# rofuyu/exp-trmf-nips16

Hardware: AMD Instinct MI355X
Metric: als_iterations_per_sec (higher is better)
Workload: dtype f32

## Files before the change

exp-trmf-nips16_amd/csrc/full_kernels.hpp:

```cpp
#pragma once

#include "cg_kernels.hpp"
#include "common.hpp"
#include "gram_kernels.hpp"

namespace trmf {

#if !defined(TRMF_UNIT_BODIES)
template <int NT>
__global__ void spmm_rows_kernel(const uint32_t *__restrict__ ptr,
                                                        const uint32_t *__restrict__ idx,
                                                        const real *__restrict__ val,
                                                        const real *__restrict__ X,
                                                        real *__restrict__ out, uint32_t row_begin,
                                                        uint32_t row_end, uint32_t zero_row, uint32_t long_thresh);
template <int NT>
__global__ void spmm_part_kernel(const uint32_t *__restrict__ idx, const real *__restrict__ val, const real *__restrict__ X,
                                 const uint32_t *__restrict__ items, uint32_t item_begin, uint32_t item_end, real *__restrict__ part,
                                 uint32_t zero_row);
#else
template <int NT, bool ITEM>
__device__ __forceinline__ void spmm_body(const uint32_t *__restrict__ ptr,
                                                        const uint32_t *__restrict__ idx,
                                                        const real *__restrict__ val,
                                                        const real *__restrict__ X,
                                                        real *__restrict__ out, uint32_t row_begin,
                                                        uint32_t row_end, uint32_t zero_row, uint32_t long_thresh) {
    constexpr int KP = kTile * NT;
    const int wave = threadIdx.x >> 6, lane = threadIdx.x & 63;
    const int g = lane >> 4, c = lane & 15;
    const uint32_t row = row_begin + blockIdx.x * 4u + (uint32_t)wave;
    if (row >= row_end) return;
    const uint32_t p0 = (uint32_t)__builtin_amdgcn_readfirstlane((int)ptr[ITEM ? 2 * row : row]);
    const uint32_t p1 = (uint32_t)__builtin_amdgcn_readfirstlane((int)ptr[ITEM ? 2 * row + 1 : row + 1]);
    if (!ITEM && p1 - p0 >= long_thresh) return;
    GramState<NT> st;
    st.clear();
    real nowq[NT];
#pragma unroll
    for (int q = 0; q < NT; q++) nowq[q] = 0;
    if (p1 > p0)
        gram_ring<NT, kRingDepth, false, false>(st, idx, val, X, zero_row, 4u, lane, nowq, GramDesc{p0, p1, 0},
                                                SingleRowStream{4u * kRingDepth}, [](int) {});
#pragma unroll
    for (int q = 0; q < NT; q++) {
        real v = st.b[q];
        v += __shfl_xor(v, 16, kWave);
        v += __shfl_xor(v, 32, kWave);
        if (g == 0) out[(size_t)row * KP + kTile * q + c] = v;
    }
}
template <int NT>
__global__ __launch_bounds__(256) void spmm_rows_kernel(const uint32_t *__restrict__ ptr,
                                                        const uint32_t *__restrict__ idx,
                                                        const real *__restrict__ val,
                                                        const real *__restrict__ X,
                                                        real *__restrict__ out, uint32_t row_begin,
                                                        uint32_t row_end, uint32_t zero_row, uint32_t long_thresh) {
    spmm_body<NT, false>(ptr, idx, val, X, out, row_begin, row_end, zero_row, long_thresh);
}
template <int NT>
__global__ __launch_bounds__(256) void spmm_part_kernel(const uint32_t *__restrict__ idx, const real *__restrict__ val,
                                                        const real *__restrict__ X, const uint32_t *__restrict__ items,
                                                        uint32_t item_begin, uint32_t item_end, real *__restrict__ part, uint32_t zero_row) {
    spmm_body<NT, true>(items, idx, val, X, part, item_begin, item_end, zero_row, 0u);
}
#endif

#if !defined(TRMF_UNIT)
__global__ __launch_bounds__(256) void spmm_reduce_kernel(const uint32_t *__restrict__ rows, const uint32_t *__restrict__ first,
                                                          const real *__restrict__ part, real *__restrict__ out, uint32_t begin,
                                                          uint32_t end, int KP) {
    const size_t e = (size_t)blockIdx.x * 256 + threadIdx.x;
    const uint32_t li = begin + (uint32_t)(e / (size_t)KP);
    if (li >= end) return;
    const int col = (int)(e % (size_t)KP);
    real acc = 0;
    for (uint32_t it = first[li]; it < first[li + 1]; it++) acc += part[(size_t)it * KP + col];
    out[(size_t)rows[li] * KP + col] = acc;
}
#endif

#if !defined(TRMF_UNIT_BODIES)
template <int NT>
__global__ void dense_tn_mfma_kernel(const real *__restrict__ A, int K, int M,
                                                            const real *__restrict__ B,
                                                            double *__restrict__ part);
#else
template <int NT>
__global__ __launch_bounds__(256) void dense_tn_mfma_kernel(const real *__restrict__ A, int K, int M,
                                                            const real *__restrict__ B,
                                                            double *__restrict__ part) {
    constexpr int KP = kTile * NT;
    const int wave = threadIdx.x >> 6, lane = threadIdx.x & 63, g = lane >> 4, c = lane & 15;
    const int m0 = (blockIdx.x * 4 + wave) * kTile;
    if (m0 >= M) return;
    const int nchunk = gridDim.y, ch = blockIdx.y;
    const int j0 = (int)((long long)K * ch / nchunk), j1 = (int)((long long)K * (ch + 1) / nchunk);
    typename Mfma16<real>::acc_t acc[NT];
#pragma unroll
    for (int q = 0; q < NT; q++) acc[q] = typename Mfma16<real>::acc_t{0, 0, 0, 0};
    const int mrow = min(m0 + c, M - 1);
    constexpr int U = 4;
    for (int j = j0; j < j1; j += 4 * U) {
        real a[U];
        RealVec<NT> bv[U];
#pragma unroll
        for (int u = 0; u < U; u++) {
            const int jj = j + 4 * u + g;
            const bool valid = jj < j1;
            const size_t jr = (size_t)(valid ? jj : j0);
            a[u] = A[jr * M + mrow];
            bv[u] = *reinterpret_cast<const RealVec<NT> *>(B + jr * KP + NT * c);
            if (!valid) a[u] = 0;
        }
#pragma unroll
        for (int u = 0; u < U; u++)
#pragma unroll
            for (int q = 0; q < NT; q++) acc[q] = Mfma16<real>::mma(a[u], bv[u].v[q], acc[q]);
    }
#pragma unroll
    for (int q = 0; q < NT; q++)
#pragma unroll
        for (int r = 0; r < 4; r++) {
            const int m = m0 + Mfma16<real>::row(lane, r);
            if (m < M) part[((size_t)ch * M + m) * KP + NT * c + q] = (double)acc[q][r];
        }
}
#endif
#if !defined(TRMF_UNIT)
__global__ __launch_bounds__(256) void dense_tn_reduce_kernel(const double *__restrict__ part, int nchunk,
                                                              int M, int KP, int NT, int k,
                                                              real *__restrict__ out) {
    const size_t e = (size_t)blockIdx.x * 4 + (threadIdx.x >> 6);
    const int lane = threadIdx.x & 63;
    if (e >= (size_t)M * KP) return;
    const int m = (int)(e / KP), tp = (int)(e - (size_t)m * KP);
    double acc = 0;
    for (int ch = lane; ch < nchunk; ch += 64) acc += part[((size_t)ch * M + m) * KP + tp];
    acc = wave_butterfly_sum(acc);
    const int t = collog(tp, NT);
    if (lane == 0) out[(size_t)m * KP + t] = (t < k) ? (real)acc : real(0);
}
#endif

#if !defined(TRMF_UNIT)
__global__ __launch_bounds__(256) void dense_tn_reduce_flat_kernel(const double *__restrict__ part, int nchunk,
                                                                   int M, int KP, int NT, int k,
// ... 258 lines not shown
```

exp-trmf-nips16_amd/csrc/gram_kernels.hpp:

```cpp
#pragma once

#include <type_traits>
#include <utility>

#include "common.hpp"

namespace trmf {

template <typename T> struct Mfma16;
template <> struct Mfma16<float> {
    typedef float acc_t __attribute__((ext_vector_type(4)));
    static __device__ __forceinline__ acc_t mma(float a, float b, acc_t c) {
        return __builtin_amdgcn_mfma_f32_16x16x4f32(a, b, c, 0, 0, 0);
    }
    static __device__ __forceinline__ int row(int lane, int r) { return 4 * (lane >> 4) + r; }
};
template <> struct Mfma16<double> {
    typedef double acc_t __attribute__((ext_vector_type(4)));
    static __device__ __forceinline__ acc_t mma(double a, double b, acc_t c) {
        return __builtin_amdgcn_mfma_f64_16x16x4f64(a, b, c, 0, 0, 0);
    }
    static __device__ __forceinline__ int row(int lane, int r) { return (lane >> 4) + 4 * r; }
};

// ... 25 lines not shown
    v += __shfl_xor(v, 16, kWave);
    v += __shfl_xor(v, 32, kWave);
    return v;
}

template <int... Is, typename Fn>
__device__ __forceinline__ void static_for_impl(std::integer_sequence<int, Is...>, Fn &&f) {
    (f(std::integral_constant<int, Is>{}), ...);
}
template <int N, typename Fn> __device__ __forceinline__ void static_for(Fn &&f) {
    static_for_impl(std::make_integer_sequence<int, N>{}, f);
}
struct GramDesc {
    uint32_t e0;
    uint32_t end;
    int row;
};

template <typename T> __device__ __forceinline__ T row16_sum(T v) { return row16_allsum(v); }
#if defined(TRMF_F32)
template <int CTRL> __device__ __forceinline__ float dpp_mov(float v) {
    return __int_as_float(__builtin_amdgcn_update_dpp(0, __float_as_int(v), CTRL, 0xf, 0xf, true));
}
__device__ __forceinline__ float row16_allsum_dpp(float v) {
    v += dpp_mov<0xB1>(v);
    v += dpp_mov<0x4E>(v);
    v += dpp_mov<0x141>(v);
    v += dpp_mov<0x140>(v);
    return v;
}
template <> __device__ __forceinline__ float row16_sum<float>(float v) { return row16_allsum_dpp(v); }
#endif

template <int NT> struct GramState {
    typename Mfma16<real>::acc_t acc[NT * (NT + 1) / 2];
    real b[NT];
    double loss;
    __device__ __forceinline__ void clear() {
#pragma unroll
        for (int t = 0; t < NT * (NT + 1) / 2; t++) acc[t] = typename Mfma16<real>::acc_t{0, 0, 0, 0};
#pragma unroll
        for (int q = 0; q < NT; q++) b[q] = 0;
        loss = 0;
    }
};

template <int N> struct alignas(sizeof(real)) RealVec { real v[N]; };

template <int SRC> __device__ __forceinline__ uint32_t quad_bcast(uint32_t v) {
    return (uint32_t)__builtin_amdgcn_update_dpp(0, (int)v, 0x55 * SRC, 0xf, 0xf, true);
}
template <int SRC> __device__ __forceinline__ float quad_bcast(float v) {
    return __int_as_float(__builtin_amdgcn_update_dpp(0, __float_as_int(v), 0x55 * SRC, 0xf, 0xf, true));
}
template <int SRC> __device__ __forceinline__ double quad_bcast(double v) {
    const long long b = __double_as_longlong(v);
    const int lo = __builtin_amdgcn_update_dpp(0, (int)(b & 0xffffffffLL), 0x55 * SRC, 0xf, 0xf, true);
    const int hi = __builtin_amdgcn_update_dpp(0, (int)(b >> 32), 0x55 * SRC, 0xf, 0xf, true);
    return __longlong_as_double(((long long)hi << 32) | (unsigned int)lo);
}

template <int SRC> __device__ __forceinline__ float quad_inject(float x, float y) {
    return __int_as_float(__builtin_amdgcn_update_dpp(__float_as_int(x), __float_as_int(y), 0x55 * SRC, 0xf, 0x8, false));
}
template <int SRC> __device__ __forceinline__ double quad_inject(double x, double y) {
    const long long xb = __double_as_longlong(x), yb = __double_as_longlong(y);
    const int lo = __builtin_amdgcn_update_dpp((int)(xb & 0xffffffffLL), (int)(yb & 0xffffffffLL), 0x55 * SRC, 0xf, 0x8, false);
    const int hi = __builtin_amdgcn_update_dpp((int)(xb >> 32), (int)(yb >> 32), 0x55 * SRC, 0xf, 0x8, false);
    return __longlong_as_double(((long long)hi << 32) | (unsigned int)lo);
}
template <int NT> __host__ __device__ constexpr bool rhs_pad_ok(int k) { return k <= kTile * NT - 8; }

template <int NT, typename R>
__device__ __forceinline__ void load_factor_slice(R (&dst)[NT], __amdgpu_buffer_rsrc_t rsrc, uint32_t byte_off) {
#pragma unroll
    for (int q = 0; q < NT; q++) {
        if constexpr (sizeof(R) == 4)
            dst[q] = __builtin_bit_cast(R, __builtin_amdgcn_raw_buffer_load_b32(rsrc, byte_off + 4 * q, 0, 0));
        else
            dst[q] = __builtin_bit_cast(R, __builtin_amdgcn_raw_buffer_load_b64(rsrc, byte_off + 8 * q, 0, 0));
    }
}

template <int NT, int D, bool DO_MMA, bool WITH_LOSS, bool RHS_PAD = false, bool TAIL = false, bool ROWEND = false, typename Next, typename RowDone>
__device__ __forceinline__ void gram_ring(GramState<NT> &st, const uint32_t *__restrict__ idx,
                                          const real *__restrict__ val, const real *__restrict__ X,
                                          uint32_t zero_row, uint32_t estride, int lane,
                                          const real (&wq)[NT], GramDesc d0, Next &&next,
                                          RowDone &&row_done) {
    static_assert(D == 4, "one quad lane per group of the iteration");
    constexpr int KP = kTile * NT;
    const uint32_t g = (uint32_t)(lane >> 4), c = (uint32_t)(lane & 15);
    const __amdgpu_buffer_rsrc_t x_rsrc =
        __builtin_amdgcn_make_buffer_rsrc(const_cast<real *>(X), 0, -1 , 0x00020000);
    const uint32_t lane_bytes = (uint32_t)NT * c * (uint32_t)sizeof(real);
    uint32_t jraw; real yraw; bool vraw;
    uint32_t jsel; real ysel;

    const uint32_t lane_e = (c & 3u) * estride + g;
    auto load_entries = [&](const GramDesc &d) {
        const uint32_t e0u = (uint32_t)__builtin_amdgcn_readfirstlane((int)d.e0), endu = (uint32_t)__builtin_amdgcn_readfirstlane((int)d.end);
        uint32_t left;
        asm("s_max_u32 %0, %1, %2\n\ts_sub_u32 %0, %0, %2" : "=&s"(left) : "s"(endu), "s"(e0u) : "scc");
        vraw = lane_e < left;
        const __amdgpu_buffer_rsrc_t ir = __builtin_amdgcn_make_buffer_rsrc(const_cast<uint32_t *>(idx + e0u), 0, (int)(left * 4u), 0x00020000);
        const __amdgpu_buffer_rsrc_t vr = __builtin_amdgcn_make_buffer_rsrc(const_cast<real *>(val + e0u), 0, (int)(left * (uint32_t)sizeof(real)), 0x00020000);
        jraw = __builtin_amdgcn_raw_buffer_load_b32(ir, lane_e * 4u, 0, 0);
        real yv[1];
        load_factor_slice(yv, vr, lane_e * (uint32_t)sizeof(real));
        yraw = yv[0];
    };
    auto promote_entries = [&]() {
        jsel = __umul24(vraw ? jraw : zero_row, (uint32_t)(KP * sizeof(real)));
        ysel = yraw;
    };
    auto load_slices = [&](auto U, real (&x)[D][NT], real (&yx)[D]) {
        constexpr int u = decltype(U)::value;
        if constexpr (!RHS_PAD) yx[u] = quad_bcast<u>(ysel);
        load_factor_slice(x[u], x_rsrc, quad_bcast<u>(jsel) + lane_bytes);
    };

    GramDesc d1 = d0; next(d1);
    GramDesc d2 = d1; next(d2);
    real x[D][NT], yx[D];
    load_entries(d0);
    promote_entries();
    if (TAIL && d1.row < 0) {
        static_for<D>([&](auto U) { load_slices(U, x, yx); });
    } else {
        load_entries(d1);
        __builtin_amdgcn_sched_barrier(0);
        static_for<D>([&](auto U) { load_slices(U, x, yx); });
        __builtin_amdgcn_sched_barrier(0);
    }
    auto consume = [&](auto U, real ycons) {
        constexpr int u = decltype(U)::value;
        real xt[NT];
#pragma unroll
        for (int q = 0; q < NT; q++) xt[q] = x[u][q];
        if constexpr (RHS_PAD) xt[NT - 1] = quad_inject<u>(x[u][NT - 1], ycons);
        else {
#pragma unroll
            for (int q = 0; q < NT; q++) st.b[q] = fma(yx[u], x[u][q], st.b[q]);
        }
        if (DO_MMA) {
            int t = 0;
#pragma unroll
            for (int ti = 0; ti < NT; ti++)
#pragma unroll
                for (int tj = ti; tj < NT; tj++, t++) st.acc[t] = Mfma16<real>::mma(xt[ti], xt[tj], st.acc[t]);
        }
        if (WITH_LOSS) {
            real d = 0;
#pragma unroll
            for (int q = 0; q < NT; q++) d = fma(wq[q], x[u][q], d);
            d = row16_sum(d);
            const real res = yx[u] - d;
            st.loss += (double)res * (double)res;
        }
    };
    while (TAIL ? d1.row >= 0 : d0.row >= 0) {
        const real ycons = ysel;
        promote_entries();
        load_entries(d2);
        const uint32_t left = ROWEND ? (uint32_t)__builtin_amdgcn_readfirstlane((int)(d0.end - d0.e0)) : 0u;
        static_for<D>([&](auto U) {
            constexpr uint32_t u = (uint32_t)decltype(U)::value;
            if (!ROWEND || u == 0 || left > 4u * u) consume(U, ycons);
            __builtin_amdgcn_sched_barrier(0);
            load_slices(U, x, yx);
            __builtin_amdgcn_sched_barrier(0);
        });
        if (d1.row != d0.row) { row_done(d0.row); }
        d0 = d1; d1 = d2; next(d2);
    }
    if constexpr (TAIL) {
        if (d0.row >= 0) {
            const int ngr = (int)((d0.end - d0.e0 + 3u) >> 2);
            const real ycons = ysel;
            static_for<D>([&](auto U) {
                if (decltype(U)::value < ngr) consume(U, ycons);
            });
            row_done(d0.row);
        }
    }
}

struct SingleRowStream {
    uint32_t step;
    __device__ __forceinline__ void operator()(GramDesc &d) const {
        if (d.row < 0) return;
        d.e0 += step;
        if (d.e0 >= d.end) { d.row = -1; d.end = 0; }
    }
};

constexpr int kRingDepth = 4;

struct SplitRows {
    const uint32_t *rows;
    const uint32_t *first;
    const real *slab;
    uint32_t stride;
    uint32_t begin, end;
};
template <int NT> __host__ __device__ constexpr uint32_t split_part_reals(bool with_b) {
    return (uint32_t)(NT * (NT + 1) / 2) * 4u * kWave + (with_b ? (uint32_t)NT * kWave : 0u);
}
#if !defined(TRMF_UNIT)
__global__ __launch_bounds__(256) void split_reduce_kernel(const uint32_t *__restrict__ first, real *__restrict__ slab, uint32_t stride,
                                                           uint32_t begin, uint32_t end, uint32_t blocks_per_row) {
    typedef real gran_t __attribute__((ext_vector_type(16 / sizeof(real))));
    constexpr uint32_t GR = 16 / sizeof(real);
    const uint32_t li = begin + blockIdx.x / blocks_per_row;
    if (li >= end) return;
    const uint32_t i0 = first[li], i1 = first[li + 1];
    const uint32_t gidx = (blockIdx.x % blocks_per_row) * 256u + threadIdx.x;
    if (i1 - i0 < 2u || gidx * GR >= stride) return;
    real *dst = slab + (size_t)i0 * stride + (size_t)gidx * GR;
    gran_t acc = *reinterpret_cast<const gran_t *>(dst);
    const real *p = dst + stride;
    uint32_t it = i0 + 1;
    for (; it + 8 <= i1; it += 8, p += (size_t)8 * stride) {
        gran_t v[8];
#pragma unroll
        for (int u = 0; u < 8; u++) v[u] = *reinterpret_cast<const gran_t *>(p + (size_t)u * stride);
#pragma unroll
        for (int u = 0; u < 8; u++) acc += v[u];
    }
    for (; it < i1; it++, p += stride) acc += *reinterpret_cast<const gran_t *>(p);
    *reinterpret_cast<gran_t *>(dst) = acc;
}
#endif

template <int NT, bool WITH_B>
__device__ __forceinline__ void load_row_sum(GramState<NT> &st, const SplitRows &sp, uint32_t i0, int lane) {
    typedef typename Mfma16<real>::acc_t acc_t;
    constexpr int NTT = NT * (NT + 1) / 2;
    const real *p = sp.slab + (size_t)i0 * sp.stride;
#pragma unroll
    for (int t = 0; t < NTT; t++) st.acc[t] = *reinterpret_cast<const acc_t *>(p + t * 4 * kWave + 4 * lane);
#pragma unroll
    for (int q = 0; q < NT; q++) st.b[q] = WITH_B ? p[NTT * 4 * kWave + q * kWave + lane] : real(0);
    st.loss = 0;
}

#if !defined(TRMF_F32)
__device__ __forceinline__ void wave_lds_sync() {
    __builtin_amdgcn_fence(__ATOMIC_ACQ_REL, "wavefront");
    __builtin_amdgcn_wave_barrier();
}
#endif



#if !defined(TRMF_F32)
constexpr int kMfmaWaves = 2;
constexpr int kRcpNewton = 2;
__device__ __forceinline__ double recip_pivot(double d) {
    double r = __builtin_amdgcn_rcp(d);
#pragma unroll
    for (int i = 0; i < kRcpNewton; i++) { const double e = fma(-d, r, 1.0); r = fma(r, e, r); }
    return r;
}
__host__ __device__ constexpr int upper_tile_index(int ti, int tj, int NT) { return ti * NT - ti * (ti - 1) / 2 + (tj - ti); }

#if !defined(TRMF_UNIT_BODIES)
template <int NT, int KMAX>
__global__ void fsolve_mfma_kernel(const uint32_t *__restrict__ ptr,
                                                                          const uint32_t *__restrict__ idx,
                                                                          const real *__restrict__ val,
                                                                          const real *__restrict__ X,
                                                                          real *__restrict__ F, uint32_t row_begin,
                                                                          uint32_t row_end, int k, real lambda,
                                                                          uint32_t zero_row, uint32_t long_m1);
template <int NT, int KMAX>
__global__ void fsolve_mfma_long_kernel(SplitRows sp, real *__restrict__ F, int k, real lambda);
#else
template <int NT, int KMAX, bool LONG>
__device__ __forceinline__ void fsolve_mfma_body(const uint32_t *__restrict__ ptr,
                                                                          const uint32_t *__restrict__ idx,
                                                                          const real *__restrict__ val,
                                                                          const real *__restrict__ X,
                                                                          real *__restrict__ F, uint32_t row_begin,
                                                                          uint32_t row_end, int k, real lambda,
                                                                          uint32_t zero_row, uint32_t long_m1, const SplitRows &sp) {
    static_assert(sizeof(real) == 8, "the in-accumulator F-solve is the fp64 path");
    constexpr int KP = kTile * NT, NPAN = KMAX / 4;
    constexpr int CP = 10;
    constexpr int FIN = (KP + 1) * CP;
    constexpr int RP = KP + 2;
    constexpr int SCR = (FIN + 8 > kTile * RP) ? FIN + 8 : kTile * RP;
    __shared__ __attribute__((aligned(16))) real scr_s[4][SCR];
    const int wave = threadIdx.x >> 6, lane = threadIdx.x & 63;
    const int g = lane >> 4, c = lane & 15;
    real *ps = scr_s[wave];
    typedef typename Mfma16<real>::acc_t acc_t;
    typedef VecOf<real, 2> pair_t;
    GramState<NT> st;
    uint32_t row;
    if constexpr (LONG) {
        const uint32_t li = sp.begin + blockIdx.x * 4u + (uint32_t)wave;
        if (li >= sp.end) return;
        row = (uint32_t)__builtin_amdgcn_readfirstlane((int)sp.rows[li]);
        load_row_sum<NT, true>(st, sp, (uint32_t)__builtin_amdgcn_readfirstlane((int)sp.first[li]), lane);
    } else {
        row = row_begin + blockIdx.x * 4u + (uint32_t)wave;
        if (row >= row_end) return;
        const uint32_t p0 = (uint32_t)__builtin_amdgcn_readfirstlane((int)ptr[row]);
        const uint32_t p1 = (uint32_t)__builtin_amdgcn_readfirstlane((int)ptr[row + 1]);
        if (p1 - p0 - 1u >= long_m1) return;
        st.clear();
        real nowq[NT];
#pragma unroll
        for (int q = 0; q < NT; q++) nowq[q] = 0;
        gram_ring<NT, kRingDepth, true, false, false, true>(st, idx, val, X, zero_row, 4u, lane, nowq, GramDesc{p0, p1, 0},
                                                            SingleRowStream{4u * kRingDepth}, [](int) {});
    }
    real y = 0, dinv = 1;
#pragma unroll
    for (int q = 0; q < NT; q++) {
        real v = st.b[q];
        v += __shfl_xor(v, 16, kWave);
        v += __shfl_xor(v, 32, kWave);
        if (g == q) y = v;
    }
#pragma unroll
    for (int ti = 0; ti < NT; ti++)
#pragma unroll
        for (int r = 0; r < 4; r++)
            if (c == g + 4 * r) st.acc[upper_tile_index(ti, ti, NT)][r] += (kTile * ti + c < k) ? lambda : real(1);

    static_for<NPAN>([&](auto Pn) {
        constexpr int pn = decltype(Pn)::value, tp = pn >> 2, r0 = pn & 3, j0 = 4 * pn;
#pragma unroll
        for (int tj = tp; tj < NT; tj++) ps[(kTile * tj + c) * CP + g] = st.acc[upper_tile_index(tp, tj, NT)][r0];
        if ((unsigned)(lane - j0) < 4u) ps[KP * CP + (lane - j0)] = y;
        wave_lds_sync();
        const real *pc = ps + j0 * CP;
        const real P00 = pc[0];
        real P01 = pc[CP], P11 = pc[CP + 1];
        real P02 = pc[2 * CP], P12 = pc[2 * CP + 1], P22 = pc[2 * CP + 2];
        real P03 = pc[3 * CP], P13 = pc[3 * CP + 1], P23 = pc[3 * CP + 2], P33 = pc[3 * CP + 3];
        const real i0 = recip_pivot(P00);
        const real l10 = P01 * i0, l20 = P02 * i0, l30 = P03 * i0;
        P11 = fma(-l10, P01, P11); P12 = fma(-l10, P02, P12); P13 = fma(-l10, P03, P13);
        P22 = fma(-l20, P02, P22); P23 = fma(-l20, P03, P23); P33 = fma(-l30, P03, P33);
        const real i1 = recip_pivot(P11);
        const real l21 = P12 * i1, l31 = P13 * i1;
        P22 = fma(-l21, P12, P22); P23 = fma(-l21, P13, P23); P33 = fma(-l31, P13, P33);
        const real i2 = recip_pivot(P22);
        const real l32 = P23 * i2;
        P33 = fma(-l32, P23, P33);
        const real i3 = recip_pivot(P33);
        const bool has_col = KP == kWave || lane < KP;
        const int col = (lane == j0 || !has_col) ? KP : lane;
        real *rec = ps + col * CP;
        const Quad<real> rin = *reinterpret_cast<const Quad<real> *>(rec);
        const real R0 = rin.v[0];
        const real R1 = fma(-l10, R0, rin.v[1]);
        const real R2 = fma(-l21, R1, fma(-l20, R0, rin.v[2]));
        const real R3 = fma(-l32, R2, fma(-l31, R1, fma(-l30, R0, rin.v[3])));
        const real S0 = -(R0 * i0), S1 = -(R1 * i1), S2 = -(R2 * i2), S3 = -(R3 * i3);
        if (has_col) {
            *reinterpret_cast<Quad<real> *>(rec) = Quad<real>{{R0, R1, R2, R3}};
            *reinterpret_cast<Quad<real> *>(rec + 4) = Quad<real>{{S0, S1, S2, S3}};
        }
        if (lane == j0) {
            *reinterpret_cast<Quad<real> *>(ps + FIN) = Quad<real>{{R0, i0, R1, i1}};
            *reinterpret_cast<Quad<real> *>(ps + FIN + 4) = Quad<real>{{R2, i2, R3, i3}};
        }
        wave_lds_sync();
        {
            const Quad<real> f0 = *reinterpret_cast<const Quad<real> *>(ps + FIN), f1 = *reinterpret_cast<const Quad<real> *>(ps + FIN + 4);
            const real upd = fma(S3, f1.v[2], fma(S2, f1.v[0], fma(S1, f0.v[2], fma(S0, f0.v[0], y))));
            const int q = min(max(lane - j0, 0), 3);
            const pair_t mine = *reinterpret_cast<const pair_t *>(ps + FIN + 2 * q);
            const bool in_panel = (unsigned)(lane - j0) < 4u;
            y = in_panel ? mine.v[0] : (lane > j0 + 3 ? upd : y);
            dinv = in_panel ? mine.v[1] : dinv;
        }
#pragma unroll
        for (int tj = tp; tj < NT; tj++) st.acc[upper_tile_index(tp, tj, NT)][r0] = ps[(kTile * tj + c) * CP + g];
        real aop[NT];
#pragma unroll
        for (int tj = tp; tj < NT; tj++) aop[tj] = ps[(kTile * tj + c) * CP + 4 + g];
        if (c <= 4 * r0 + 3) aop[tp] = 0;
        wave_lds_sync();
#pragma unroll
        for (int ti = tp; ti < NT; ti++)
#pragma unroll
            for (int tj = ti; tj < NT; tj++) {
                acc_t &C = st.acc[upper_tile_index(ti, tj, NT)];
                C = Mfma16<real>::mma(aop[ti], st.acc[upper_tile_index(tp, tj, NT)][r0], C);
            }
    });

    static_for<NT>([&](auto Tr) {
        constexpr int tt = NT - 1 - decltype(Tr)::value;
        if constexpr (kTile * tt < KMAX) {
#pragma unroll
            for (int ti = 0; ti <= tt; ti++)
#pragma unroll
                for (int r = 0; r < 4; r++) {
                    real v = st.acc[upper_tile_index(ti, tt, NT)][r];
                    if (ti == tt && g + 4 * r >= c) v = 0;
                    ps[c * RP + kTile * ti + g + 4 * r] = v;
                }
            if constexpr (tt + 1 < NT) {
#pragma unroll
                for (int r = 0; r < 4; r++) ps[c * RP + kTile * (tt + 1) + g + 4 * r] = 0;
            }
            wave_lds_sync();
            static_for<kTile>([&](auto Nr) {
                constexpr int n = kTile - 1 - decltype(Nr)::value, t = kTile * tt + n;
                if constexpr (t < KMAX && t > 0) {
                    const real xt = lane_bcast(y * dinv, t);
                    const real cv = (KP == kWave || lane < KP) ? ps[n * RP + lane] : real(0);
                    y = fma(-cv, xt, y);
                }
            });
            wave_lds_sync();
        }
    });
    if (lane < k) F[(size_t)row * KP + colpos(lane, NT)] = y * dinv;
}
template <int NT, int KMAX>
__global__ __launch_bounds__(256, kMfmaWaves) void fsolve_mfma_kernel(const uint32_t *__restrict__ ptr,
                                                                          const uint32_t *__restrict__ idx,
                                                                          const real *__restrict__ val,
                                                                          const real *__restrict__ X,
                                                                          real *__restrict__ F, uint32_t row_begin,
                                                                          uint32_t row_end, int k, real lambda,
                                                                          uint32_t zero_row, uint32_t long_m1) {
    fsolve_mfma_body<NT, KMAX, false>(ptr, idx, val, X, F, row_begin, row_end, k, lambda, zero_row, long_m1, SplitRows{});
}
template <int NT, int KMAX>
__global__ __launch_bounds__(256, kMfmaWaves) void fsolve_mfma_long_kernel(SplitRows sp, real *__restrict__ F, int k, real lambda) {
    fsolve_mfma_body<NT, KMAX, true>(nullptr, nullptr, nullptr, nullptr, F, 0u, 0u, k, lambda, 0u, 0u, sp);
}
#endif
#endif

#if defined(TRMF_F32)

template <int SRC> __device__ __forceinline__ float row_bcast(float v) {
    return __int_as_float(__builtin_amdgcn_update_dpp(0, __float_as_int(v), 0x150 + SRC, 0xf, 0xf, true));
}

template <int NT> __device__ __forceinline__ constexpr int quad_slab_floats() {
    int n = 0;
    for (int q = 0; q < NT; q++) n += kTile * (kTile * (q + 1) + 4);
    return n;
}
template <int NT> __device__ __forceinline__ constexpr int quad_slab_col_offset(int q) {
    int n = 0;
    for (int i = 0; i < q; i++) n += kTile * (kTile * (i + 1) + 4);
    return n;
}

typedef float quad_f4 __attribute__((ext_vector_type(4)));

template <int NT, int KMAX, bool RHS_IN>
__device__ __forceinline__ void quad_factor_solve(quad_f4 (&a4)[NT][KMAX / 4], float (&bz)[NT], float (&x)[NT], int c) {
    constexpr int NR = KMAX / 4;
    float dinv[NT];
#pragma unroll
    for (int q = 0; q < NT; q++) dinv[q] = 0;
    static_for<KMAX>([&](auto J) {
        constexpr int j = decltype(J)::value, qj = j >> 4, cj = j & 15, Rj = j >> 2, ij = j & 3;
        {
            const float inv = __builtin_amdgcn_rsqf(row_bcast<cj>(a4[qj][Rj][ij]));
            float u[NT], nu[NT];
#pragma unroll
            for (int q = qj; q < NT; q++) {
                u[q] = a4[q][Rj][ij] * inv;
                if (q == qj && c <= cj) u[q] = 0;
                a4[q][Rj][ij] = u[q];
                nu[q] = -u[q];
            }
            if constexpr (!RHS_IN) {
                const float zj = row_bcast<cj>(bz[qj]) * inv;
#pragma unroll
                for (int q = qj; q < NT; q++) bz[q] = fmaf(-u[q], zj, bz[q]);
                if (c == cj) bz[qj] = zj;
            }
            if (c == cj) dinv[qj] = inv;
            static_for<NR>([&](auto Rx) {
                constexpr int R = decltype(Rx)::value, qs = (4 * R) >> 4;
                if constexpr (4 * R + 3 > j) {
#pragma unroll
                    for (int q = qs; q < NT; q++) a4[q][R] = __builtin_amdgcn_mfma_f32_4x4x1f32(nu[qs], u[q], a4[q][R], 2, R & 3, 0);
                }
            });
            __builtin_amdgcn_sched_barrier(0);
        }
    });
#pragma unroll
    for (int q = 0; q < NT; q++) x[q] = 0;
    if constexpr (RHS_IN) {
        if (c == 15) x[NT - 1] = -1.0f;
#pragma unroll
        for (int q = 0; q < NT; q++) bz[q] = 0;
    }
    static_for<KMAX>([&](auto Jr) {
        constexpr int j = KMAX - 1 - decltype(Jr)::value, qj = j >> 4, cj = j & 15, Rj = j >> 2, ij = j & 3;
        {
            float part = 0;
#pragma unroll
            for (int q = qj; q < NT; q++) part = fmaf(a4[q][Rj][ij], x[q], part);
            const float sum = row16_allsum_dpp(part);
            const float xv = (bz[qj] - sum) * dinv[qj];
            if (c == cj) x[qj] = xv;
        }
    });
}

struct QuadStream {
    uint32_t pr[5];
    uint32_t step;
    uint32_t long_m1;
    __device__ __forceinline__ uint32_t row_ptr_at(int i) const {
        return i == 0 ? pr[0] : i == 1 ? pr[1] : i == 2 ? pr[2] : i == 3 ? pr[3] : pr[4];
    }
    __device__ __forceinline__ bool skips(int r) const { return row_ptr_at(r + 1) - row_ptr_at(r) - 1u >= long_m1; }
    __device__ __forceinline__ GramDesc first() const {
        GramDesc d{0, 0, -1};
        for (int r = 0; r < 4; r++)
            if (!skips(r)) { d = GramDesc{row_ptr_at(r), row_ptr_at(r + 1), r}; break; }
        return d;
    }
    __device__ __forceinline__ void operator()(GramDesc &d) const {
        if (d.row < 0) return;
        d.e0 += step;
        if (d.e0 < d.end) return;
        int r = d.row + 1;
        while (r < 4 && skips(r)) r++;
        if (r < 4) d = GramDesc{row_ptr_at(r), row_ptr_at(r + 1), r};
        else d = GramDesc{0, 0, -1};
    }
};

constexpr int kQuadWaves = 3;
constexpr int quad_waves(int NT) { return NT >= 4 ? 2 : kQuadWaves; }
constexpr bool quad_row_end(int NT, int KMAX) { return (NT == 3 && KMAX == 40) || (NT == 4 && KMAX == 56); }
#if !defined(TRMF_UNIT_BODIES)
template <int NT, int KMAX>
__global__ void fsolve_quad_kernel(const uint32_t *__restrict__ ptr,
                                                          const uint32_t *__restrict__ idx,
                                                          const float *__restrict__ val,
                                                          const float *__restrict__ X,
                                                          float *__restrict__ F, uint32_t row_begin,
                                                          uint32_t row_end, int k, float lambda,
                                                          uint32_t zero_row, uint32_t long_m1);
template <int NT, int KMAX>
__global__ void fsolve_quad_long_kernel(SplitRows sp, float *__restrict__ F, int k, float lambda);
#else
template <int NT, int KMAX, bool LONG>
__device__ __forceinline__ void fsolve_quad_body(const uint32_t *__restrict__ ptr,
                                                          const uint32_t *__restrict__ idx,
                                                          const float *__restrict__ val,
                                                          const float *__restrict__ X,
                                                          float *__restrict__ F, uint32_t row_begin,
                                                          uint32_t row_end, int k, float lambda,
                                                          uint32_t zero_row, uint32_t long_m1, const SplitRows &sp) {
    static_assert(sizeof(real) == 4, "quad F-solve is the fp32 path");
    constexpr int KP = kTile * NT;
    constexpr int SLAB = quad_slab_floats<NT>();
    __shared__ __attribute__((aligned(16))) float lds_slab[4][SLAB];
    const int wave = threadIdx.x >> 6, lane = threadIdx.x & 63;
    const int grp = lane >> 4, c = lane & 15;
    const uint32_t row0 = LONG ? sp.begin + (blockIdx.x * 4u + (uint32_t)wave) * 4u : row_begin + (blockIdx.x * 4u + (uint32_t)wave) * 4u;
    if (row0 >= (LONG ? sp.end : row_end)) return;
    float *S = lds_slab[wave];
    typedef float f4 __attribute__((ext_vector_type(4)));

    quad_f4 a4[NT][KMAX / 4];
    float bz[NT];
#pragma unroll
    for (int q = 0; q < NT; q++) {
        bz[q] = 0;
#pragma unroll
        for (int s = 0; s < KMAX; s++) a4[q][s >> 2][s & 3] = (s == kTile * q + c) ? 1.0f : 0.0f;
    }
    bool mine = false;

    QuadStream stream;
    stream.step = 4u * kRingDepth;
    stream.long_m1 = long_m1;
    {
        const uint32_t rr = row0 + (uint32_t)(lane < 5 ? lane : 4);
        const uint32_t lim = LONG ? sp.end : row_end;
        const uint32_t v = (LONG ? sp.first : ptr)[rr < lim ? rr : lim];
#pragma unroll
        for (int i = 0; i < 5; i++) stream.pr[i] = (uint32_t)__builtin_amdgcn_readlane((int)v, i);
    }

    GramState<NT> st;
    st.clear();
    constexpr bool PAD = KMAX <= kTile * NT - 8;
    auto finalize = [&](int sys) {
        if constexpr (!PAD) {
#pragma unroll
            for (int q = 0; q < NT; q++) {
                st.b[q] += __shfl_xor(st.b[q], 16, kWave);
                st.b[q] += __shfl_xor(st.b[q], 32, kWave);
            }
        }
        int t = 0;
#pragma unroll
        for (int ti = 0; ti < NT; ti++)
#pragma unroll
            for (int tj = ti; tj < NT; tj++, t++) {
                f4 v = st.acc[t];
                if (ti == tj) {
#pragma unroll
                    for (int r = 0; r < 4; r++)
                        if (c == 4 * grp + r) v[r] += (kTile * ti + c < k) ? lambda : 1.0f;
                }
                *reinterpret_cast<f4 *>(&S[quad_slab_col_offset<NT>(tj) + c * (kTile * (tj + 1) + 4) + kTile * ti + 4 * grp]) = v;
            }
        __builtin_amdgcn_fence(__ATOMIC_ACQ_REL, "wavefront");
        __builtin_amdgcn_wave_barrier();
        if (grp == sys) {
            mine = true;
#pragma unroll
            for (int q = 0; q < NT; q++) {
                if constexpr (!PAD) bz[q] = st.b[q];
#pragma unroll
                for (int s4 = 0; s4 < KMAX / 4; s4++) {
                    if (4 * s4 <= kTile * q + 15)
                        a4[q][s4] = *reinterpret_cast<const f4 *>(&S[quad_slab_col_offset<NT>(q) + c * (kTile * (q + 1) + 4) + 4 * s4]);
                }
            }
        }
        __builtin_amdgcn_fence(__ATOMIC_ACQ_REL, "wavefront");
        __builtin_amdgcn_wave_barrier();
        st.clear();
    };

    if constexpr (LONG) {
        for (int sys = 0; sys < 4; sys++) {
            if (stream.row_ptr_at(sys + 1) == stream.row_ptr_at(sys)) continue;
            load_row_sum<NT, !PAD>(st, sp, stream.row_ptr_at(sys), lane);
            finalize(sys);
        }
    } else {
        float nowq[NT];
#pragma unroll
        for (int q = 0; q < NT; q++) nowq[q] = 0;
        gram_ring<NT, kRingDepth, true, false, PAD, false, quad_row_end(NT, KMAX)>(st, idx, val, X, zero_row, 4u, lane, nowq, stream.first(), stream,
                                                    finalize);
    }

    float x[NT];
    quad_factor_solve<NT, KMAX, PAD>(a4, bz, x, c);
    if (mine) {
        RealVec<NT> o;
#pragma unroll
        for (int q = 0; q < NT; q++) o.v[q] = (kTile * q + c < k) ? x[q] : 0.0f;
        const uint32_t orow = LONG ? sp.rows[row0 + (uint32_t)grp] : row0 + (uint32_t)grp;
        *reinterpret_cast<RealVec<NT> *>(F + (size_t)orow * KP + NT * c) = o;
    }
}
template <int NT, int KMAX>
__global__ __launch_bounds__(256, quad_waves(NT)) void fsolve_quad_kernel(const uint32_t *__restrict__ ptr,
                                                          const uint32_t *__restrict__ idx,
                                                          const float *__restrict__ val,
                                                          const float *__restrict__ X,
                                                          float *__restrict__ F, uint32_t row_begin,
                                                          uint32_t row_end, int k, float lambda,
                                                          uint32_t zero_row, uint32_t long_m1) {
    fsolve_quad_body<NT, KMAX, false>(ptr, idx, val, X, F, row_begin, row_end, k, lambda, zero_row, long_m1, SplitRows{});
}
template <int NT, int KMAX>
__global__ __launch_bounds__(256, quad_waves(NT) - 1) void fsolve_quad_long_kernel(SplitRows sp, float *__restrict__ F, int k, float lambda) {
    fsolve_quad_body<NT, KMAX, true>(nullptr, nullptr, nullptr, nullptr, F, 0u, 0u, k, lambda, 0u, 0u, sp);
}
#endif

#endif

#if !defined(TRMF_UNIT_BODIES)
template <int NT, bool RHS_PAD, bool PACKED>
__global__ void gram_x_kernel(const uint32_t *__restrict__ ptr,
                                                     const uint32_t *__restrict__ idx,
                                                     const real *__restrict__ val,
                                                     const real *__restrict__ Hf,
                                                     real *__restrict__ G, real *__restrict__ Bv,
                                                     uint32_t row_begin, uint32_t row_end, int k,
                                                     uint32_t zero_row, size_t gs, uint32_t long_thresh, const uint32_t *__restrict__ order);
template <int NT, bool RHS_PAD, bool PACKED>
__global__ void gram_x_long_kernel(SplitRows sp, real *__restrict__ G, real *__restrict__ Bv, int k, size_t gs);
template <int NT, bool RHS_PAD>
__global__ void gram_part_kernel(const uint32_t *__restrict__ idx, const real *__restrict__ val, const real *__restrict__ X,
                                 const uint32_t *__restrict__ items, uint32_t item_begin, uint32_t item_end,
                                 real *__restrict__ slab, uint32_t stride, uint32_t zero_row);
#else
template <int NT, bool RHS_PAD>
__global__ __launch_bounds__(256) void gram_part_kernel(const uint32_t *__restrict__ idx, const real *__restrict__ val,
                                                        const real *__restrict__ X, const uint32_t *__restrict__ items,
                                                        uint32_t item_begin, uint32_t item_end, real *__restrict__ slab,
                                                        uint32_t stride, uint32_t zero_row) {
    typedef typename Mfma16<real>::acc_t acc_t;
    constexpr int NTT = NT * (NT + 1) / 2;
    const int wave = threadIdx.x >> 6, lane = threadIdx.x & 63;
    const uint32_t item = item_begin + blockIdx.x * 4u + (uint32_t)wave;
    if (item >= item_end) return;
    const uint32_t p0 = (uint32_t)__builtin_amdgcn_readfirstlane((int)items[2 * item]);
    const uint32_t p1 = (uint32_t)__builtin_amdgcn_readfirstlane((int)items[2 * item + 1]);
    GramState<NT> st;
    st.clear();
    real nowq[NT];
#pragma unroll
    for (int q = 0; q < NT; q++) nowq[q] = 0;
    if (p1 > p0)
        gram_ring<NT, kRingDepth, true, false, RHS_PAD>(st, idx, val, X, zero_row, 4u, lane, nowq, GramDesc{p0, p1, 0},
                                                        SingleRowStream{4u * kRingDepth}, [](int) {});
    real *p = slab + (size_t)item * stride;
#pragma unroll
    for (int t = 0; t < NTT; t++) *reinterpret_cast<acc_t *>(p + t * 4 * kWave + 4 * lane) = st.acc[t];
    if constexpr (!RHS_PAD) {
#pragma unroll
        for (int q = 0; q < NT; q++) p[NTT * 4 * kWave + q * kWave + lane] = st.b[q];
    }
}

template <int NT, bool RHS_PAD, bool PACKED, bool LONG>
__device__ __forceinline__ void gram_x_body(const uint32_t *__restrict__ ptr,
                                                     const uint32_t *__restrict__ idx,
                                                     const real *__restrict__ val,
                                                     const real *__restrict__ Hf,
                                                     real *__restrict__ G, real *__restrict__ Bv,
                                                     uint32_t row_begin, uint32_t row_end, int k,
                                                     uint32_t zero_row, size_t gs, uint32_t long_thresh, const SplitRows &sp,
                                                     const uint32_t *__restrict__ order) {
    constexpr int KP = kTile * NT;
    const int wave = threadIdx.x >> 6, lane = threadIdx.x & 63;
    const int g = lane >> 4, c = lane & 15;
    GramState<NT> st;
    uint32_t row;
    if constexpr (LONG) {
        const uint32_t li = sp.begin + blockIdx.x * 4u + (uint32_t)wave;
        if (li >= sp.end) return;
        row = (uint32_t)__builtin_amdgcn_readfirstlane((int)sp.rows[li]);
        load_row_sum<NT, !RHS_PAD>(st, sp, (uint32_t)__builtin_amdgcn_readfirstlane((int)sp.first[li]), lane);
    } else {
    row = row_begin + blockIdx.x * (blockDim.x >> 6) + (uint32_t)wave;
    if (row >= row_end) return;
    if (order) row = (uint32_t)__builtin_amdgcn_readfirstlane((int)order[row]);
    const uint32_t p0 = (uint32_t)__builtin_amdgcn_readfirstlane((int)ptr[row]);
    const uint32_t p1 = (uint32_t)__builtin_amdgcn_readfirstlane((int)ptr[row + 1]);
    if (p1 - p0 >= long_thresh) return;

    st.clear();
    real nowq[NT];
#pragma unroll
    for (int q = 0; q < NT; q++) nowq[q] = 0;
    if (p1 > p0)
        gram_ring<NT, kRingDepth, true, false, RHS_PAD>(st, idx, val, Hf, zero_row, 4u, lane, nowq, GramDesc{p0, p1, 0},
                                                        SingleRowStream{4u * kRingDepth}, [](int) {});
    }
    if constexpr (RHS_PAD) {
        if (c == 15) {
#pragma unroll
            for (int ti = 0; ti < NT; ti++) {
                const int t = ti * NT - ti * (ti - 1) / 2 + (NT - 1 - ti);
#pragma unroll
                for (int r = 0; r < 4; r++) {
                    const int tt = kTile * ti + Mfma16<real>::row(lane, r);
                    Bv[(size_t)row * KP + tt] = (tt < k) ? st.acc[t][r] : real(0);
                }
            }
        }
    } else {
#pragma unroll
        for (int q = 0; q < NT; q++) {
            real v = st.b[q];
            v += __shfl_xor(v, 16, kWave);
            v += __shfl_xor(v, 32, kWave);
            if (g == 0) Bv[(size_t)row * KP + kTile * q + c] = (kTile * q + c < k) ? v : real(0);
        }
    }
    real *Grow = G + (size_t)row * gs;
    int t = 0;
#pragma unroll
    for (int ti = 0; ti < NT; ti++)
#pragma unroll
        for (int tj = ti; tj < NT; tj++, t++)
#pragma unroll
            for (int r = 0; r < 4; r++) {
                const int rw = kTile * ti + Mfma16<real>::row(lane, r), cl = kTile * tj + c;
                if (rw < k && cl < k) {
                    const real a = st.acc[t][r];
                    if constexpr (PACKED) {
                        if (rw <= cl) Grow[rw * k - rw * (rw - 1) / 2 + cl - rw] = a;
                    } else {
                        Grow[rw * k + cl] = a;
                        if (ti != tj) Grow[cl * k + rw] = a;
                    }
                }
            }
}
template <int NT, bool RHS_PAD, bool PACKED>
__global__ __launch_bounds__(256) void gram_x_kernel(const uint32_t *__restrict__ ptr,
                                                     const uint32_t *__restrict__ idx,
                                                     const real *__restrict__ val,
                                                     const real *__restrict__ Hf,
                                                     real *__restrict__ G, real *__restrict__ Bv,
                                                     uint32_t row_begin, uint32_t row_end, int k,
                                                     uint32_t zero_row, size_t gs, uint32_t long_thresh, const uint32_t *__restrict__ order) {
    gram_x_body<NT, RHS_PAD, PACKED, false>(ptr, idx, val, Hf, G, Bv, row_begin, row_end, k, zero_row, gs, long_thresh, SplitRows{}, order);
}
template <int NT, bool RHS_PAD, bool PACKED>
__global__ __launch_bounds__(256) void gram_x_long_kernel(SplitRows sp, real *__restrict__ G, real *__restrict__ Bv, int k, size_t gs) {
    gram_x_body<NT, RHS_PAD, PACKED, true>(nullptr, nullptr, nullptr, nullptr, G, Bv, 0u, 0u, k, 0u, gs, 0u, sp, nullptr);
}
#endif

#if !defined(TRMF_UNIT_BODIES)
template <int NT>
__global__ void loss_kernel(const uint32_t *__restrict__ ptr,
                                                   const uint32_t *__restrict__ idx,
                                                   const real *__restrict__ val,
                                                   const real *__restrict__ Hf,
                                                   const real *__restrict__ W,
                                                   double *__restrict__ lossrow,
                                                   uint32_t row_begin, uint32_t row_end,
                                                   uint32_t zero_row);
#else
template <int NT>
__global__ __launch_bounds__(256) void loss_kernel(const uint32_t *__restrict__ ptr,
                                                   const uint32_t *__restrict__ idx,
                                                   const real *__restrict__ val,
                                                   const real *__restrict__ Hf,
                                                   const real *__restrict__ W,
                                                   double *__restrict__ lossrow,
                                                   uint32_t row_begin, uint32_t row_end,
                                                   uint32_t zero_row) {
    constexpr int KP = kTile * NT;
    __shared__ double Sl[4];
    const int wave = threadIdx.x >> 6, lane = threadIdx.x & 63;
    const int c = lane & 15;
    const uint32_t row = row_begin + blockIdx.x;
    if (row >= row_end) return;
    const uint32_t p0 = ptr[row], p1 = ptr[row + 1];
    GramState<NT> st;
    st.clear();
    real wq[NT];
#pragma unroll
    for (int q = 0; q < NT; q++) wq[q] = W[(size_t)row * KP + NT * c + q];
    {
        const uint32_t e0 = (uint32_t)__builtin_amdgcn_readfirstlane((int)(p0 + 4u * (uint32_t)wave));
        const uint32_t e1 = (uint32_t)__builtin_amdgcn_readfirstlane((int)p1);
        GramDesc d0{e0, e1, e0 < e1 ? 0 : -1};
        gram_ring<NT, kRingDepth, false, true>(st, idx, val, Hf, zero_row, 16u, lane, wq, d0,
                                               SingleRowStream{16u * kRingDepth}, [](int) {});
    }
    double l = (c == 0) ? st.loss : 0.0;
    l = wave_allsum(l);
    if (lane == 0) Sl[wave] = l;
    __syncthreads();
    if (threadIdx.x == 0) lossrow[row] = (Sl[0] + Sl[1]) + (Sl[2] + Sl[3]);
}
#endif

}
```

exp-trmf-nips16_amd/csrc/kernel_units.hpp:

```cpp
#pragma once

#if defined(TRMF_UNIT) || defined(TRMF_SINGLE_UNIT)
#define TRMF_UNIT_BODIES 1
#endif
#if !defined(TRMF_UNIT) || TRMF_UNIT == 1
#include "gram_kernels.hpp"
#endif
#if !defined(TRMF_UNIT) || TRMF_UNIT == 2
#include "cg_kernels.hpp"
#endif
#if defined(TRMF_UNIT) && TRMF_UNIT == 4
#include "cg_kernels.hpp"
#include "gram_kernels.hpp"
#include "full_kernels.hpp"
#endif
#if !defined(TRMF_UNIT) || TRMF_UNIT == 5
#include "heldout_kernels.hpp"
#endif
#if !defined(TRMF_UNIT) || TRMF_UNIT == 6
#include "forecast_kernels.hpp"
#endif
#if !defined(TRMF_UNIT) || TRMF_UNIT == 7
#include "online_kernels.hpp"
#endif
#if !defined(TRMF_UNIT) || TRMF_UNIT == 8
#include "uncertainty_kernels.hpp"
#endif
#if !defined(TRMF_UNIT)
#include "cg_persist_args.hpp"
#elif TRMF_UNIT == 3
#include "cg_persist.hpp"
#endif
#if defined(TRMF_SINGLE_UNIT)
#include "cg_persist.hpp"
#endif

namespace trmf {

#define TRMF_HV_SIG (XParams, XState *, HvVecs, TileShard, int, int, const uint32_t *, const real *, const real *, const double *, double *, const PeerTable *, int, int)
#define TRMF_HV_KQS(X, MODE, SHARD, NTH)                           \
    X void hv_tile_kernel<MODE, 8, SHARD, NTH> TRMF_HV_SIG;        \
    X void hv_tile_kernel<MODE, 16, SHARD, NTH> TRMF_HV_SIG;       \
    X void hv_tile_kernel<MODE, 24, SHARD, NTH> TRMF_HV_SIG;       \
    X void hv_tile_kernel<MODE, 32, SHARD, NTH> TRMF_HV_SIG;       \
    X void hv_tile_kernel<MODE, 40, SHARD, NTH> TRMF_HV_SIG;       \
    X void hv_tile_kernel<MODE, 48, SHARD, NTH> TRMF_HV_SIG;       \
    X void hv_tile_kernel<MODE, 56, SHARD, NTH> TRMF_HV_SIG;       \
    X void hv_tile_kernel<MODE, 64, SHARD, NTH> TRMF_HV_SIG;
#define TRMF_UNIT_HV(X, SHARD, NTH)                                                                                   \
    TRMF_HV_KQS(X, HV_GRAD, SHARD, NTH) TRMF_HV_KQS(X, HV_CG_FIRST, SHARD, NTH) TRMF_HV_KQS(X, HV_CG_STEP, SHARD, NTH) TRMF_HV_KQS(X, HV_PLAIN, SHARD, NTH)

#define TRMF_PERSIST_SIG (XParams, XState *, PersistArgs)
#define TRMF_PERSIST_KQS(X, SHARD, NTH)                                  \
    X void cg_persist_kernel<8, SHARD, NTH> TRMF_PERSIST_SIG;            \
    X void cg_persist_kernel<16, SHARD, NTH> TRMF_PERSIST_SIG;           \
    X void cg_persist_kernel<24, SHARD, NTH> TRMF_PERSIST_SIG;           \
    X void cg_persist_kernel<32, SHARD, NTH> TRMF_PERSIST_SIG;           \
    X void cg_persist_kernel<40, SHARD, NTH> TRMF_PERSIST_SIG;           \
    X void cg_persist_kernel<48, SHARD, NTH> TRMF_PERSIST_SIG;           \
    X void cg_persist_kernel<56, SHARD, NTH> TRMF_PERSIST_SIG;           \
    X void cg_persist_kernel<64, SHARD, NTH> TRMF_PERSIST_SIG;
#define TRMF_UNIT_PERSIST(X) TRMF_PERSIST_KQS(X, false, 256) TRMF_PERSIST_KQS(X, true, 256) TRMF_PERSIST_KQS(X, false, 512)

#define TRMF_FSOLVE_SIG (const uint32_t *, const uint32_t *, const real *, const real *, real *, uint32_t, uint32_t, int, real, uint32_t, uint32_t)
#define TRMF_FSOLVE_LONG_SIG (SplitRows, real *, int, real)
#if defined(TRMF_F32)
#define TRMF_FSOLVE_ONE(X, NT, KMAX) X void fsolve_quad_kernel<NT, KMAX> TRMF_FSOLVE_SIG;
#define TRMF_FSOLVE_LONG_ONE(X, NT, KMAX) X void fsolve_quad_long_kernel<NT, KMAX> TRMF_FSOLVE_LONG_SIG;
#else
#define TRMF_FSOLVE_ONE(X, NT, KMAX) X void fsolve_mfma_kernel<NT, KMAX> TRMF_FSOLVE_SIG;
#define TRMF_FSOLVE_LONG_ONE(X, NT, KMAX) X void fsolve_mfma_long_kernel<NT, KMAX> TRMF_FSOLVE_LONG_SIG;
#endif
#define TRMF_GRAMX_SIG (const uint32_t *, const uint32_t *, const real *, const real *, real *, real *, uint32_t, uint32_t, int, uint32_t, size_t, uint32_t, const uint32_t *)
#define TRMF_GRAMX_LONG_SIG (SplitRows, real *, real *, int, size_t)
#define TRMF_GRAM_PART_SIG (const uint32_t *, const real *, const real *, const uint32_t *, uint32_t, uint32_t, real *, uint32_t, uint32_t)
#define TRMF_SPLIT_NT(X, NT)                                               \
    X void gram_part_kernel<NT, true> TRMF_GRAM_PART_SIG;                  \
    X void gram_part_kernel<NT, false> TRMF_GRAM_PART_SIG;                 \
    X void gram_x_long_kernel<NT, true, true> TRMF_GRAMX_LONG_SIG;         \
    X void gram_x_long_kernel<NT, true, false> TRMF_GRAMX_LONG_SIG;        \
    X void gram_x_long_kernel<NT, false, true> TRMF_GRAMX_LONG_SIG;        \
    X void gram_x_long_kernel<NT, false, false> TRMF_GRAMX_LONG_SIG;
#define TRMF_UNIT_SPLIT(X)                                                                                                   \
    TRMF_FSOLVE_LONG_ONE(X, 1, 8) TRMF_FSOLVE_LONG_ONE(X, 1, 16) TRMF_FSOLVE_LONG_ONE(X, 2, 24) TRMF_FSOLVE_LONG_ONE(X, 2, 32) \
    TRMF_FSOLVE_LONG_ONE(X, 3, 40) TRMF_FSOLVE_LONG_ONE(X, 3, 48) TRMF_FSOLVE_LONG_ONE(X, 4, 56) TRMF_FSOLVE_LONG_ONE(X, 4, 64) \
    TRMF_SPLIT_NT(X, 1) TRMF_SPLIT_NT(X, 2) TRMF_SPLIT_NT(X, 3) TRMF_SPLIT_NT(X, 4)
#define TRMF_GRAMX_NT(X, NT)                                     \
    X void gram_x_kernel<NT, true, true> TRMF_GRAMX_SIG;         \
    X void gram_x_kernel<NT, true, false> TRMF_GRAMX_SIG;        \
    X void gram_x_kernel<NT, false, true> TRMF_GRAMX_SIG;        \
    X void gram_x_kernel<NT, false, false> TRMF_GRAMX_SIG;
#define TRMF_LOSS_SIG (const uint32_t *, const uint32_t *, const real *, const real *, const real *, double *, uint32_t, uint32_t, uint32_t)
#define TRMF_UNIT_GRAM(X)                                                                                                    \
    TRMF_FSOLVE_ONE(X, 1, 8) TRMF_FSOLVE_ONE(X, 1, 16) TRMF_FSOLVE_ONE(X, 2, 24) TRMF_FSOLVE_ONE(X, 2, 32)                   \
    TRMF_FSOLVE_ONE(X, 3, 40) TRMF_FSOLVE_ONE(X, 3, 48) TRMF_FSOLVE_ONE(X, 4, 56) TRMF_FSOLVE_ONE(X, 4, 64)                  \
    TRMF_GRAMX_NT(X, 1) TRMF_GRAMX_NT(X, 2) TRMF_GRAMX_NT(X, 3) TRMF_GRAMX_NT(X, 4)                                         \
    X void loss_kernel<1> TRMF_LOSS_SIG; X void loss_kernel<2> TRMF_LOSS_SIG; X void loss_kernel<3> TRMF_LOSS_SIG; X void loss_kernel<4> TRMF_LOSS_SIG;

#define TRMF_APPLY_SHARED_SIG (XParams, const XState *, int, const real *, const real *, const real *, const real *, const real *, int, real *, int, double *, int, int, int)
#define TRMF_FULL_NT(X, NT)                                                                                                              \
    X void spmm_rows_kernel<NT>(const uint32_t *, const uint32_t *, const real *, const real *, real *, uint32_t, uint32_t, uint32_t, uint32_t);  \
    X void spmm_part_kernel<NT>(const uint32_t *, const real *, const real *, const uint32_t *, uint32_t, uint32_t, real *, uint32_t);  \
    X void dense_tn_mfma_kernel<NT>(const real *, int, int, const real *, double *);                                                    \
    X void small_gram_mfma_kernel<NT>(const real *, int, int, double *);                                                                \
    X void chol_wave_kernel<NT>(const real *, real *, int);                                                                             \
    X void apply_shared_mfma_kernel<NT> TRMF_APPLY_SHARED_SIG;
#define TRMF_UNIT_FULL(X) TRMF_FULL_NT(X, 1) TRMF_FULL_NT(X, 2) TRMF_FULL_NT(X, 3) TRMF_FULL_NT(X, 4)

#define TRMF_UNIT_HELDOUT(X)                                                                                                 \
    X void heldout_eval_kernel<0>(HeldoutArgs); X void heldout_eval_kernel<1>(HeldoutArgs); X void heldout_eval_kernel<2>(HeldoutArgs); \
    X void heldout_eval_kernel<3>(HeldoutArgs); X void heldout_eval_kernel<4>(HeldoutArgs);

#define TRMF_UNIT_FORECAST(X)                                                                                                \
    X void forecast_score_kernel<0>(ScoreArgs); X void forecast_score_kernel<1>(ScoreArgs); X void forecast_score_kernel<2>(ScoreArgs); \
    X void forecast_score_kernel<3>(ScoreArgs); X void forecast_score_kernel<4>(ScoreArgs);

#define TRMF_UNIT_ONLINE(X)                                                                                                  \
    X void assim_factor_kernel<1>(AssimFactorArgs); X void assim_factor_kernel<2>(AssimFactorArgs);                          \
    X void assim_factor_kernel<3>(AssimFactorArgs); X void assim_factor_kernel<4>(AssimFactorArgs);

#define TRMF_UNIT_UNCERTAINTY(X)                                                                                             \
    X void noise_resid_kernel<0>(NoiseResidArgs); X void noise_resid_kernel<1>(NoiseResidArgs); X void noise_resid_kernel<2>(NoiseResidArgs); \
    X void noise_resid_kernel<3>(NoiseResidArgs); X void noise_resid_kernel<4>(NoiseResidArgs);                              \
    X void forecast_dist_kernel<0>(DistArgs); X void forecast_dist_kernel<1>(DistArgs); X void forecast_dist_kernel<2>(DistArgs); \
    X void forecast_dist_kernel<3>(DistArgs); X void forecast_dist_kernel<4>(DistArgs);

#define TRMF_DEFINE_KERNEL template __global__

}
```

exp-trmf-nips16_amd/csrc/session.hpp:

```cpp
#pragma once

#include "session_xphase.hpp"

extern "C" char **environ;

namespace trmf {

struct TrmfSessionImpl : SessionXPhase {
    ~TrmfSessionImpl() {
        if (stream) (void)hipStreamSynchronize(stream);
        if (side) (void)hipStreamSynchronize(side);
        if (aux_theta) (void)hipStreamSynchronize(aux_theta);
        for (auto &e : events) {
            hipEvent_t all[] = {e.f0, e.fk0, e.fk1, e.f1, e.xg1, e.x1, e.lv1};
            for (hipEvent_t ev : all) if (ev) (void)hipEventDestroy(ev);
        }
        for (hipEvent_t ev : {gx0, gx1, gx2, fs0, fs1, fs2, ts0, ts1}) if (ev) (void)hipEventDestroy(ev);
        release_p2p();
        for (hipEvent_t ev : {ov_b, ov_c[0], ov_c[1], ov_c[2], ov_c[3], emu_ready, emu_end}) if (ev) (void)hipEventDestroy(ev);
        if (side) (void)hipStreamDestroy(side);
        for (hipEvent_t ev : {theta_fork, theta_done}) if (ev) (void)hipEventDestroy(ev);
        if (cg_note) (void)hipHostFree(cg_note);
        StreamCache::release(aux_theta);
        StreamCache::release(stream);
    }

    int upload_padded(DevBuf<real> &dst, DevBuf<real> &raw, const real *src, size_t rows) {
        if (raw.upload(src, rows * (size_t)k) || dst.alloc((rows + 1) * (size_t)KP, false)) return kFail;
        const size_t N = (rows + 1) * (size_t)KP;
        hipLaunchKernelGGL(factor_pad_kernel, dim3((unsigned)std::min<size_t>(4096, (N + 255) / 256)), dim3(256), 0, stream,
                           raw.p, rows, k, KP, NT, dst.p);
        TRMF_HIP_CHECK(hipGetLastError());
        return 0;
    }
    int download_padded(const DevBuf<real> &src, real *dst, size_t rows) {
        if (rows == 0) return 0;
        DevBuf<real> raw;
        SyncStreamOnExit drain(stream);
        const size_t N = rows * (size_t)k;
        if (raw.alloc(N, false)) return kFail;
        hipLaunchKernelGGL(factor_unpad_kernel, dim3((unsigned)std::min<size_t>(4096, (N + 255) / 256)), dim3(256), 0, stream,
                           src.p, rows, k, KP, NT, raw.p);
        TRMF_HIP_CHECK(hipGetLastError());
        TRMF_HIP_CHECK(hipStreamSynchronize(stream));
        TRMF_HIP_CHECK(hipMemcpy(dst, raw.p, N * sizeof(real), hipMemcpyDeviceToHost));
        return 0;
    }
    struct StagedFactors {
        unsigned char *base = nullptr;
        std::unique_lock<std::mutex> lease;
        std::vector<unsigned char> fallback;
        size_t bW = 0, bH = 0, bL = 0;
        void commit(void *Wout, void *Hout, void *Lout) const {
            HostStager::parallel_copy(Wout, base, bW);
            HostStager::parallel_copy(Hout, base + bW, bH);
            if (bL) std::memcpy(Lout, base + bW + bH, bL);
        }
    };
    int download_staged(StagedFactors &sf) {
        sf.bW = (size_t)T * k * sizeof(real); sf.bH = (size_t)n * k * sizeof(real); sf.bL = (size_t)nlag * k * sizeof(real);
        const size_t total = sf.bW + sf.bH + sf.bL;
        sf.base = HostStager::current().staging(total, sf.lease);
        if (!sf.base) {
            try { sf.fallback.resize(total); } catch (const std::bad_alloc &) { set_error("host staging of the factors: out of memory"); return kFail; }
            sf.base = sf.fallback.data();
        }
        DevBuf<real> rawW, rawH;
        SyncStreamOnExit drain(stream);
        if (rawW.alloc((size_t)T * k, false) || rawH.alloc((size_t)n * k, false)) return kFail;
        auto unpad = [&](const DevBuf<real> &src, size_t rows, real *dst) {
            const size_t N = rows * (size_t)k;
            if (N) hipLaunchKernelGGL(factor_unpad_kernel, dim3((unsigned)std::min<size_t>(4096, (N + 255) / 256)), dim3(256), 0, stream, src.p, rows, k, KP, NT, dst);
        };
        unpad(W, T, rawW.p); unpad(H, n, rawH.p);
        TRMF_HIP_CHECK(hipGetLastError());
        if (sf.bW) TRMF_HIP_CHECK(hipMemcpyAsync(sf.base, rawW.p, sf.bW, hipMemcpyDeviceToHost, stream));
        if (sf.bH) TRMF_HIP_CHECK(hipMemcpyAsync(sf.base + sf.bW, rawH.p, sf.bH, hipMemcpyDeviceToHost, stream));
        if (sf.bL) TRMF_HIP_CHECK(hipMemcpyAsync(sf.base + sf.bW + sf.bH, theta.p, sf.bL, hipMemcpyDeviceToHost, stream));
        TRMF_HIP_CHECK(hipStreamSynchronize(stream));
        if (test_env("TRMF_FAIL_DOWNLOAD")) { set_error("download failure forced by TRMF_FAIL_DOWNLOAD"); return kFail; }
        return 0;
    }
    int upload_ptr32(DevBuf<uint32_t> &dst, const size_t *src, size_t count) {
        if (dst.alloc(count, false)) return kFail;
        return HostStager::current().h2d_narrow(dst.p, (const uint64_t *)src, count, stream);
    }
    int launch_sum_squares(const real *dv, size_t count) {
        if (sumsq_part.alloc(kSumsqBlocks)) return kFail;
        hipLaunchKernelGGL(sumsq_values_kernel, dim3(kSumsqBlocks), dim3(256), 0, stream, dv, count, sumsq_part.p);
        TRMF_HIP_CHECK(hipGetLastError());
        return 0;
    }
    int finish_sum_squares(double *out) {
        std::vector<double> h(kSumsqBlocks);
        TRMF_HIP_CHECK(hipStreamSynchronize(stream));
        TRMF_HIP_CHECK(hipMemcpy(h.data(), sumsq_part.p, kSumsqBlocks * sizeof(double), hipMemcpyDeviceToHost));
        double acc = 0;
        for (double x : h) acc += x;
        *out = acc;
        return 0;
    }
    int device_sum_squares(const real *dv, size_t count, double *out) { return launch_sum_squares(dv, count) || finish_sum_squares(out) ? kFail : 0; }
    size_t footprint_estimate() const {
        const size_t sz = sizeof(real), NVb = (size_t)(T + 1) * KP * sz, NHb = (size_t)(n + 1) * KP * sz;
        size_t b = dense ? 2 * (size_t)T * n * sz + (full ? (size_t)kGemmChunks * std::max(T, n) * KP * sz : 0)
                         : 2 * (size_t)nnz * (4 + sz) + ((size_t)T + n + 2) * 4;
        b += NVb + NHb + (size_t)(T + n) * k * sz;
        b += 11 * NVb + 4 * NVb;
        if (!full) b += (size_t)T * k * k * sz;
        if (full) b += NHb;
        if (generic) b += (size_t)std::min(kGenBlocks, std::max(n, 1)) * k * k * sz;
        b += (size_t)kLogCap * sizeof(DeviceIterLog) + ((size_t)32 << 20);
        return b + b / 16;
    }
    int create(const PyMatrix *Y, const uint32_t *lags, uint32_t lag_size, const PyMatrix *Wm,
               const PyMatrix *Hm, const PyMatrix *LVm) {
        T = (int)Y->rows; n = (int)Y->cols; k = (int)Wm->cols; nnz = Y->nnz;
        KP = padded_rank(k); NT = KP / kTile; KMAX = ((k + 7) / 8) * 8;
        generic = k > kMaxRank;
        nlag = (int)lag_size; midx = nlag ? (int)lags[nlag - 1] : 0;
        has_lag0 = nlag > 0 && lags[0] == 0;
        comm = active_comm();
        if (StreamCache::acquire(&stream)) return kFail;
        FillStreamScope fill(stream);
        dense = Y->type != TRMF_SPARSE;
        DevicePool::current().reserve(footprint_estimate());

        const double tu0 = now_s();
        if (!dense) {
            host_row_ptr.assign(Y->row_ptr, Y->row_ptr + (size_t)T + 1);
            host_col_ptr.assign(Y->col_ptr, Y->col_ptr + (size_t)n + 1);
            if (upload_ptr32(Yc_ptr, Y->col_ptr, (size_t)n + 1)) return kFail;
            if (Yc_idx.upload(Y->row_idx, nnz)) return kFail;
            if (Yc_val.upload((const real *)Y->val, nnz)) return kFail;
            if (upload_ptr32(Yr_ptr, Y->row_ptr, (size_t)T + 1)) return kFail;
            if (Yr_idx.upload(Y->col_idx, nnz)) return kFail;
            if (Yr_val.upload((const real *)Y->val_t, nnz)) return kFail;
            if (launch_sum_squares(Yr_val.p, nnz)) return kFail;
            bytes_uploaded += 2.0 * (double)nnz * (4 + sizeof(real)) + 8.0 * ((double)T + n + 2);
        } else {
            const size_t N = (size_t)T * n;
            if (Yd_tn.alloc(N, false) || Yd_nt.alloc(N, false)) return kFail;
            if (Y->type == TRMF_DENSE_ROWMAJOR) {
                if (HostStager::current().h2d(Yd_tn.p, Y->val, N * sizeof(real), stream)) return kFail;
                launch_transpose(Yd_tn.p, T, n, Yd_nt.p);
            } else {
                if (HostStager::current().h2d(Yd_nt.p, Y->val, N * sizeof(real), stream)) return kFail;
                launch_transpose(Yd_nt.p, n, T, Yd_tn.p);
            }
            if (launch_sum_squares(Yd_tn.p, N)) return kFail;
            bytes_uploaded += (double)N * sizeof(real);
        }
        if (lag_set.upload(lags, nlag)) return kFail;
        {
            const std::vector<uint32_t> steps = ar_lag_steps(lags, nlag);
            nsteps = (int)steps.size();
            if (lag_steps.upload(steps.data(), steps.size())) return kFail;
        }
        if (upload_padded(W, raw_W, (const real *)Wm->val, T)) return kFail;
        if (upload_padded(H, raw_H, (const real *)Hm->val, n)) return kFail;
        if (theta.upload((const real *)LVm->val, (size_t)nlag * k)) return kFail;
        bytes_uploaded += ((double)T + n + nlag) * k * sizeof(real);
        t_upload_s = now_s() - tu0;

        if (xstate.alloc(1) || log.alloc(kLogCap)) return kFail;
        if (full && (Bf.alloc((size_t)n * KP) || GSf.alloc((size_t)k * k) || Uf.alloc((size_t)k * k) || GSx.alloc((size_t)k * k + kHvGramPad) ||
                     sgram_part.alloc((size_t)kSmallGramBlocks * k * k)))
            return kFail;
        if (comm->world > 1 && count_ranks_per_device()) return kFail;
        if (alloc_time_scratch()) return kFail;

        events.resize(kEventRing);
        for (auto &e : events) {
            hipEvent_t *all[] = {&e.f0, &e.fk0, &e.fk1, &e.f1, &e.xg1, &e.x1, &e.lv1};
            for (hipEvent_t *ev : all) { *ev = nullptr; TRMF_HIP_CHECK(hipEventCreate(ev)); }
        }
        for (hipEvent_t *ev : {&gx0, &gx1, &gx2, &fs0, &fs1, &fs2, &ts0, &ts1}) TRMF_HIP_CHECK(hipEventCreate(ev));
        if (gramx_times.alloc((size_t)8 * comm->world)) return kFail;
        if (comm->world == 1) { gramx_mode = kGramxShard; fs_mode = kShardOn; }
        if (const char *e = test_env("TRMF_GRAMX")) gramx_mode = (e[0] == 'r') ? kGramxReplicate : kGramxShard;
        if (const char *e = test_env("TRMF_FSHARD")) fs_mode = (e[0] == 'r') ? kShardOff : kShardOn;
        if (const char *e = test_env("TRMF_THETA_SOLVE")) theta_force_lds = std::string(e) == "lds";
        if (finish_sum_squares(&ysq_acc)) return kFail;
        set_trYTY();
        raw_W.release(); raw_H.release(); sumsq_part.release();
        if (comm->world > 1) {
            std::vector<uint64_t> off(comm->world + 1);
            for (int r = 0; r <= comm->world; r++) off[r] = (uint64_t)r * 2 * sizeof(double);
            if (comm->allgatherv(gramx_times.p, off.data(), stream)) return kFail;
            TRMF_HIP_CHECK(hipStreamSynchronize(stream));
        }
        if (nlag > 0 && theta_overlap_pays() && !test_env("TRMF_NO_OVERLAP")) (void)ensure_aux();
        created = true;
        return autotune();
    }

    int alloc_time_scratch() {
        const size_t NV = (size_t)T * KP;
        if (full && dense && gemm_part.alloc((size_t)kGemmChunks * (size_t)std::max(T, n) * KP)) return kFail;
        if (Bv.alloc(NV) || g.alloc(NV) || s.alloc(NV) || r.alloc(NV) ||
            d0.alloc(NV) || d1.alloc(NV) || Hd.alloc(NV) || r1.alloc(NV) || Hd1.alloc(NV) || w_new.alloc(NV) ||
            lossrow.alloc(T))
            return kFail;
        const int nchunk = std::max(1, (T - midx + kThetaChunk - 1) / kThetaChunk);
        const int npairs = nlag * (nlag + 1) / 2 + nlag;
        if (theta_part.alloc((size_t)k * nchunk * std::max(npairs, 1))) return kFail;
        if (nlag && allow_dyn_lds(theta_gram_kernel, theta_gram_lds(), "Theta Gram (max lag too large)")) return kFail;
        if (nlag && theta_solve_lds() > kLdsMax) {
            if (theta_scratch.alloc((size_t)k * ((size_t)nlag * nlag + nlag), false)) return kFail;
        } else if (nlag && allow_dyn_lds(theta_solve_kernel, theta_solve_lds(), "Theta solve (too many lags)")) return kFail;
        if (generic) {
            if (gen_scratch.alloc((size_t)std::min(kGenBlocks, std::max(n, 1)) * k * k, false)) return kFail;
            if (allow_dyn_lds(gram_generic_kernel<true>, gram_generic_lds(k), "generic F-solve") ||
                allow_dyn_lds(gram_generic_kernel<false>, gram_generic_lds(k), "generic Gram build")) return kFail;
        }

        nbe = (int)std::min<size_t>(kMaxPartials, (NV + 255) / 256);
        rpb = std::max(1, 256 / k);
        nba = std::min(kMaxPartials, (T + rpb - 1) / rpb);
        if (full && !generic) {
            const int blocks = ((T + kApplyTile - 1) / kApplyTile + 3) / 4, passes = (blocks + 511) / 512;
// ... 75 lines not shown
        fbounds.resize(comm->world + 1); xbounds.resize(comm->world + 1); fcut.clear();
        if (!dense) {
            partition_by_nnz<uint64_t>((uint64_t)n, host_col_ptr.data(), comm->world, fbounds.data());
            partition_by_nnz<uint64_t>((uint64_t)T, host_row_ptr.data(), comm->world, xbounds.data());
        } else {
            for (int r = 0; r <= comm->world; r++) {
                fbounds[r] = (uint64_t)n * r / comm->world;
                xbounds[r] = (uint64_t)T * r / comm->world;
            }
        }
        if (decide_cg_shard()) return kFail;
        init_x_forms();
        return setup_split_rows();
    }
    int setup_split_rows() {
        longF.clear(); longX.clear();
        part_slab.release(); part_stride = 0;
        if (dense || generic) return 0;
        hipDeviceProp_t prop;
        int dev = 0;
        TRMF_HIP_CHECK(hipGetDevice(&dev));
        TRMF_HIP_CHECK(hipGetDeviceProperties(&prop, dev));
        const int waves = std::max(1, prop.multiProcessorCount) * 12;
        if (build_long_rows(longF, host_col_ptr, (size_t)n, (sizeof(real) == 4 && !full) ? 512u : 2048u, waves) ||
            build_long_rows(longX, host_row_ptr, (size_t)T, 2048u, waves, true)) return kFail;
        const uint32_t items = std::max(longF.nitems, longX.nitems);
        if (!items) return 0;
        if (full) {
            part_stride = (uint32_t)KP;
            return part_slab.alloc((size_t)items * part_stride, false);
        }
        if (!with_nt(NT, [&](auto N) { part_stride = split_part_reals<decltype(N)::value>(true); })) return unsupported_rank();
        return part_slab.alloc((size_t)items * part_stride, false);
    }
    int set_series_transform(const real *a, const real *b) {
        if (!dense) { set_error("set_series_transform: needs a dense Y (missing == 0)"); return kFail; }
        FillStreamScope fill(stream);
        TRMF_HIP_CHECK(hipStreamSynchronize(stream));
        if (Yraw.n != (size_t)T * n) {
            if (has_transform) { set_error("set_series_transform: raw matrix lost"); return kFail; }
            if (Yraw.alloc((size_t)T * n, false)) return kFail;
            TRMF_HIP_CHECK(hipMemcpyAsync(Yraw.p, Yd_tn.p, (size_t)T * n * sizeof(real), hipMemcpyDeviceToDevice, stream));
        }
        std::vector<real> one((size_t)n, real(1)), zero((size_t)n, real(0));
        if (tr_a.upload(a ? a : one.data(), n) || tr_b.upload(b ? b : zero.data(), n)) return kFail;
        has_transform = true;
        return apply_series_transform();
    }
    int apply_series_transform() {
        const int nb = 1024;
        if (tr_part.alloc(nb)) return kFail;
        hipLaunchKernelGGL(affine_columns_kernel, dim3(nb), dim3(256), 0, stream, Yraw.p, (size_t)T, n, tr_a.p, tr_b.p, Yd_tn.p, tr_part.p);
        launch_transpose(Yd_tn.p, T, n, Yd_nt.p);
        TRMF_HIP_CHECK(hipGetLastError());
        std::vector<double> part(nb);
        TRMF_HIP_CHECK(hipStreamSynchronize(stream));
        TRMF_HIP_CHECK(hipMemcpy(part.data(), tr_part.p, nb * sizeof(double), hipMemcpyDeviceToHost));
        ysq_acc = 0;
        for (double v : part) ysq_acc += v;
        set_trYTY();
        return 0;
    }

    int append_rows(const PyMatrix *Yn) {
        const int Tn = (int)Yn->rows, T0 = T;
        if ((int)Yn->cols != n) { set_error("append_rows: column count differs from the session's"); return kFail; }
        if ((Yn->type != TRMF_SPARSE) != dense) { set_error("append_rows: storage class (sparse/dense) differs from the session's"); return kFail; }
        if ((uint64_t)(T0 + Tn + 1) >= (1ull << 24) || (uint64_t)(T0 + Tn + 1) * KP * sizeof(real) > 0xffffffffull ||
            nnz + Yn->nnz >= (1ull << 32)) { set_error("append_rows: problem would exceed 32-bit device indices"); return kFail; }
        if (Tn <= 0) return 0;
        FillStreamScope fill(stream);
        TRMF_HIP_CHECK(hipStreamSynchronize(stream));
        const int T1 = T0 + Tn;
        {
            const int Tsave = T; const uint64_t nzsave = nnz;
            T = T1; nnz = dense ? (uint64_t)T1 * n : nnz + Yn->nnz;
            const size_t fp = footprint_estimate();
            T = Tsave; nnz = nzsave;
            DevicePool::current().reserve(fp);
        }
        std::vector<uint64_t> new_row_ptr, new_col_ptr;
        uint64_t new_nnz = nnz;
        double new_ysq = ysq_acc;
        DevBuf<uint32_t> ptr2, idx2, cptr2, cidx2; DevBuf<real> val2, cval2, tn2, nt2, raw2, W2;
        SyncStreamOnExit drain(stream);
        if (!dense) {
            const uint64_t nz0 = nnz, nzn = Yn->nnz, nz1 = nz0 + nzn;
            new_row_ptr = host_row_ptr;
            for (int i = 1; i <= Tn; i++) new_row_ptr.push_back(nz0 + Yn->row_ptr[i]);
            if (upload_ptr32(ptr2, (const size_t *)new_row_ptr.data(), (size_t)T1 + 1) || idx2.alloc(nz1, false) || val2.alloc(nz1, false)) return kFail;
            TRMF_HIP_CHECK(hipMemcpyAsync(idx2.p, Yr_idx.p, nz0 * sizeof(uint32_t), hipMemcpyDeviceToDevice, stream));
            TRMF_HIP_CHECK(hipMemcpyAsync(val2.p, Yr_val.p, nz0 * sizeof(real), hipMemcpyDeviceToDevice, stream));
            if (nzn) {
                TRMF_HIP_CHECK(hipMemcpyAsync(idx2.p + nz0, Yn->col_idx, nzn * sizeof(uint32_t), hipMemcpyHostToDevice, stream));
                TRMF_HIP_CHECK(hipMemcpyAsync(val2.p + nz0, Yn->val_t, nzn * sizeof(real), hipMemcpyHostToDevice, stream));
            }
            new_col_ptr = host_col_ptr;
            std::vector<uint32_t> np32((size_t)n + 1);
            for (int j = 0; j <= n; j++) { new_col_ptr[j] += Yn->col_ptr[j]; np32[j] = (uint32_t)new_col_ptr[j]; }
            DevBuf<uint32_t> wptr, widx; DevBuf<real> wval;
            SyncStreamOnExit drain_block(stream);
            if (cptr2.upload(np32.data(), np32.size()) || cidx2.alloc(nz1, false) || cval2.alloc(nz1, false) ||
                upload_ptr32(wptr, Yn->col_ptr, (size_t)n + 1) || widx.upload(Yn->row_idx, nzn) || wval.upload((const real *)Yn->val, nzn))
                return kFail;
            hipLaunchKernelGGL(csc_append_kernel, dim3((n + 3) / 4), dim3(256), 0, stream, Yc_ptr.p, Yc_idx.p, Yc_val.p, wptr.p, widx.p,
                               wval.p, cptr2.p, cidx2.p, cval2.p, n, (uint32_t)T0);
            TRMF_HIP_CHECK(hipGetLastError());
            TRMF_HIP_CHECK(hipStreamSynchronize(stream));
            new_nnz = nz1;
            if (device_sum_squares(val2.p, new_nnz, &new_ysq)) return kFail;
        } else {
            std::vector<real> blk;
            (void)dense_rows_to_rowmajor(Yn, blk);
            if (tn2.alloc((size_t)T1 * n, false) || nt2.alloc((size_t)T1 * n, false)) return kFail;
            TRMF_HIP_CHECK(hipMemcpyAsync(tn2.p, Yd_tn.p, (size_t)T0 * n * sizeof(real), hipMemcpyDeviceToDevice, stream));
            TRMF_HIP_CHECK(hipMemcpyAsync(tn2.p + (size_t)T0 * n, blk.data(), blk.size() * sizeof(real), hipMemcpyHostToDevice, stream));
            if (has_transform) {
                if (raw2.alloc((size_t)T1 * n, false)) return kFail;
                TRMF_HIP_CHECK(hipMemcpyAsync(raw2.p, Yraw.p, (size_t)T0 * n * sizeof(real), hipMemcpyDeviceToDevice, stream));
                TRMF_HIP_CHECK(hipMemcpyAsync(raw2.p + (size_t)T0 * n, blk.data(), blk.size() * sizeof(real), hipMemcpyHostToDevice, stream));
            }
            launch_transpose(tn2.p, T1, n, nt2.p);
            TRMF_HIP_CHECK(hipGetLastError());
            TRMF_HIP_CHECK(hipStreamSynchronize(stream));
            new_nnz = (uint64_t)T1 * n;
            if (device_sum_squares(tn2.p, new_nnz, &new_ysq)) return kFail;
        }
        {
            if (W2.alloc((size_t)(T1 + 1) * KP)) return kFail;
            TRMF_HIP_CHECK(hipMemcpyAsync(W2.p, W.p, (size_t)T0 * KP * sizeof(real), hipMemcpyDeviceToDevice, stream));
            if (k <= kMaxRank) {
                hipLaunchKernelGGL(latent_forecast_kernel, dim3(1), dim3(64), 0, stream, W2.p, T0, T1, KP, NT, k, lag_set.p, nlag, theta.p);
                TRMF_HIP_CHECK(hipGetLastError());
            } else if (launch_rollout(W.p, T0, Tn, W2.p + (size_t)T0 * KP, nullptr)) return kFail;
            TRMF_HIP_CHECK(hipStreamSynchronize(stream));
        }
        if (!dense) {
            Yr_ptr.swap(ptr2); Yr_idx.swap(idx2); Yr_val.swap(val2);
            Yc_ptr.swap(cptr2); Yc_idx.swap(cidx2); Yc_val.swap(cval2);
            host_row_ptr.swap(new_row_ptr); host_col_ptr.swap(new_col_ptr);
        } else {
            Yd_tn.swap(tn2); Yd_nt.swap(nt2);
            if (has_transform) Yraw.swap(raw2);
        }
        W.swap(W2);
        nnz = new_nnz; ysq_acc = new_ysq;
        T = T1;
        if (dense && has_transform && apply_series_transform()) return kFail;
        set_trYTY();
        iter = 0;
        if (gramx_mode != kGramxReplicate && comm->world > 1 && !test_env("TRMF_GRAMX")) { gramx_mode = kGramxMeasure; gramx_calls = 0; }
        if (alloc_time_scratch()) return kFail;
        TRMF_HIP_CHECK(hipDeviceSynchronize());
        return autotune();
    }
    bool decisions_pending() const {
        if (comm->world <= 1 || full) return false;
        if (fs_mode == kShardMeasure && period_H > 0) return true;
        if (period_W <= 0) return false;
        if (x_form < 0) return true;
        const bool rep_gram = tile_TI > 0 ? x_form == kXRep : (!uts && !cg_shard);
        return rep_gram && !cg_shard && gramx_mode == kGramxMeasure;
    }
    struct TunedDecisions {
        int fs_mode, gramx_mode, x_form, tuned_iters;
        float x_ms[kXForms]; double x_ms_all[kXForms];
        std::vector<int> x_cands;
        std::string persist_note;
    };
    static std::map<std::string, TunedDecisions> &decision_cache() { static std::map<std::string, TunedDecisions> c; return c; }
    static std::mutex &decision_mu() { static std::mutex m; return m; }
    std::string decision_key() const {
        std::string key = std::to_string(T) + "," + std::to_string(n) + "," + std::to_string(k) + "," + std::to_string(nnz) + "," + std::to_string(nlag) + "," +
                          std::to_string(midx) + "," + std::to_string(sizeof(real)) + "," + std::to_string(full) + std::to_string(dense) + "," + std::to_string(comm->id) + "," +
                          std::to_string(comm->world) + "," + std::to_string(period_W > 0) + std::to_string(period_H > 0);
        for (char **e = ::environ; e && *e; e++) if (!strncmp(*e, "TRMF_", 5)) { key += ";"; key += *e; }
        return key;
    }
    int autotune() {
        tuned_iters = 0; decisions_from_cache = false;
        if (const char *e = getenv("TRMF_AUTOTUNE")) if (atoi(e) == 0) return 0;
        if (!decisions_pending()) return 0;
        const std::string key = decision_key();
        {
            std::lock_guard<std::mutex> lk(decision_mu());
            auto it = decision_cache().find(key);
            if (it != decision_cache().end() && it->second.x_cands == x_cands) {
                const TunedDecisions &d = it->second;
                fs_mode = d.fs_mode; gramx_mode = d.gramx_mode; x_form = d.x_form; persist_note = d.persist_note;
                for (int f = 0; f < kXForms; f++) { x_ms[f] = d.x_ms[f]; x_ms_all[f] = d.x_ms_all[f]; }
                x_calls = 2 * (int)x_cands.size();
                decisions_from_cache = true;
                if (!decisions_pending()) {
                    if (verbose && comm->rank == 0) fprintf(stderr, ">> %s\n", describe().c_str());
                    return 0;
                }
                decisions_from_cache = false;
            }
        }
        DevBuf<real> W0, H0, T0;
        SyncStreamOnExit drain(stream);
        const size_t nw = (size_t)(T + 1) * KP, nh = (size_t)(n + 1) * KP, nt = (size_t)nlag * k;
        if (W0.alloc(nw, false) || H0.alloc(nh, false) || T0.alloc(nt, false)) return kFail;
        TRMF_HIP_CHECK(hipMemcpyAsync(W0.p, W.p, nw * sizeof(real), hipMemcpyDeviceToDevice, stream));
        TRMF_HIP_CHECK(hipMemcpyAsync(H0.p, H.p, nh * sizeof(real), hipMemcpyDeviceToDevice, stream));
        if (nt) TRMF_HIP_CHECK(hipMemcpyAsync(T0.p, theta.p, nt * sizeof(real), hipMemcpyDeviceToDevice, stream));
        const int v = verbose, it0 = iter;
        const bool ln = log_norms;
        verbose = 0; log_norms = false;
        int rc = 0;
        for (; tuned_iters < kAutotuneMax && decisions_pending() && rc == 0; tuned_iters++) rc = run(1);
        verbose = v; log_norms = ln; iter = it0;
        if (rc) return kFail;
        TRMF_HIP_CHECK(hipMemcpyAsync(W.p, W0.p, nw * sizeof(real), hipMemcpyDeviceToDevice, stream));
        TRMF_HIP_CHECK(hipMemcpyAsync(H.p, H0.p, nh * sizeof(real), hipMemcpyDeviceToDevice, stream));
        if (nt) TRMF_HIP_CHECK(hipMemcpyAsync(theta.p, T0.p, nt * sizeof(real), hipMemcpyDeviceToDevice, stream));
        TRMF_HIP_CHECK(hipStreamSynchronize(stream));
        if (sync()) return kFail;
        if (!decisions_pending()) {
            TunedDecisions d{fs_mode, gramx_mode, x_form, tuned_iters, {}, {}, x_cands, persist_note};
            for (int f = 0; f < kXForms; f++) { d.x_ms[f] = x_ms[f]; d.x_ms_all[f] = x_ms_all[f]; }
            std::lock_guard<std::mutex> lk(decision_mu());
// ... 192 lines not shown
            TRMF_HIP_CHECK(hipMemcpy(hp.data(), persist_prof.p, hp.size() * sizeof(long long), hipMemcpyDeviceToHost));
            for (int sel = 0; sel < 2; sel++) {
                const long long t0 = hp[(size_t)sel * kProfIters * kProfSlots];
                for (int i = 0; i < kProfIters; i++) {
                    const long long *r = hp.data() + ((size_t)sel * kProfIters + i) * kProfSlots;
                    if (!r[0] && !r[3]) continue;
                    fprintf(stderr, "PERSIST_PROF tile %s row %2d:", sel ? "mid" : "0  ", i);
                    for (int q = 0; q < kProfSlots; q++) fprintf(stderr, " %8.2f", r[q] ? (r[q] - t0) * 0.01 : 0.0);
                    fprintf(stderr, "  us\n");
                }
            }
            {
                const long long *q = hp.data() + (size_t)2 * kProfIters * kProfSlots;
                long long base = 0;
                for (int t = 0; t < nbt; t++) if (q[2 * t] && (!base || q[2 * t] < base)) base = q[2 * t];
                fprintf(stderr, "PERSIST_TILES");
                for (int t = 0; t < nbt; t++) fprintf(stderr, " %.2f/%.2f", (q[2 * t] - base) * 0.01, (q[2 * t + 1] - base) * 0.01);
                fprintf(stderr, "\n");
            }
        }
#endif
        if (persist_state == 1 && comm->world == 1) {
            XState hx;
            TRMF_HIP_CHECK(hipMemcpy(&hx, xstate.p, sizeof hx, hipMemcpyDeviceToHost));
            if (hx.p2p_error && recover) return persist_recover(hx);
            if (hx.p2p_error) { set_error("persistent CG kernel: an exchange between workgroups timed out"); return kFail; }
            if (recover && snap_iter >= 0 && snap_iter != iter && take_snapshot()) return kFail;
        } else if (persist_state == 1 || (persist_shard_state == 1 && x_form == kXTsPersist)) {
            XState hx;
            TRMF_HIP_CHECK(hipMemcpy(&hx, xstate.p, sizeof hx, hipMemcpyDeviceToHost));
            if (hx.p2p_error) { set_error("persistent CG kernel: an exchange between workgroups timed out (is another process using the GPU? TRMF_PERSIST=0 selects the launch-per-step path)"); return kFail; }
        }
        if (p2p.on) {
            XState hx;
            TRMF_HIP_CHECK(hipMemcpy(&hx, xstate.p, sizeof hx, hipMemcpyDeviceToHost));
            if (hx.p2p_error) {
                char msg[256];
                snprintf(msg, sizeof msg, "time-sharded CG: a peer-to-peer exchange timed out (TRMF_CG=p2p): rank %d, message %lld, launch %lld, "
                         "peer %lld: expected epoch %lld, flag %lld", comm->rank, hx.p2p_diag[0] / 1000000, hx.p2p_diag[0] / 1000 % 1000 - 1,
                         hx.p2p_diag[0] % 1000, hx.p2p_diag[1], hx.p2p_diag[2]);
                set_error(msg);
                if (test_env("TRMF_P2P_DEBUG")) {
                    std::vector<double> hp((size_t)P_NSLOTS * xp.pstride);
                    TRMF_HIP_CHECK(hipMemcpy(hp.data(), pbase(), hp.size() * sizeof(double), hipMemcpyDeviceToHost));
                    fprintf(stderr, "[p2p debug] rank %d: %s\n  stop_it %d cg_iter %d rho %.17g %.17g %.17g gnorm %.17g cgtol %.9g\n", comm->rank, msg,
                            hx.stop_it, hx.cg_iter, hx.rho_hist[0], hx.rho_hist[1], hx.rho_hist[2], hx.gnorm, (double)hx.cgtol);
                    for (int a = 0; a < P_NSLOTS; a++) {
                        double t = 0; int nz = 0;
                        for (int q = 0; q < xp.pstride; q++) { t += hp[(size_t)a * xp.pstride + q]; nz += hp[(size_t)a * xp.pstride + q] != 0; }
                        fprintf(stderr, "  partial array %2d: sum %.17g (%d nonzero)\n", a, t, nz);
                    }
                }
                return kFail;
            }
        }
        return 0;
    }

    int stats(TrmfIterStats *out, int cap) {
        if (sync()) return kFail;
        const int avail = std::min(iter, std::min(kLogCap, kEventRing));
        const int cnt = std::min(cap, avail);
        for (int q = 0; q < cnt; q++) {
            const int it0 = iter - cnt + q;
            DeviceIterLog hl;
            TRMF_HIP_CHECK(hipMemcpy(&hl, log.p + (it0 % kLogCap), sizeof hl, hipMemcpyDeviceToHost));
            PhaseEvents &ev = events[it0 % kEventRing];
            TrmfIterStats &o = out[q];
            o.normF = hl.normF; o.normX = hl.normX; o.normLV = hl.normLV;
            o.f = hl.x.f; o.fnew = hl.x.fnew; o.actred = hl.x.actred; o.prered = hl.x.prered;
            o.gnorm = hl.x.gnorm; o.cg_rnorm = hl.x.cg_rnorm; o.cg_iter = hl.x.cg_iter; o.accepted = hl.x.accepted; o.delta = hl.x.delta;
            o.cg_rnorm_direct = hl.x.rho_direct >= 0 ? std::sqrt(hl.x.rho_direct) : -1.0;
            o.ms_F = o.ms_X = o.ms_LV = o.ms_F_kernel = o.ms_X_gram = -1;
            if (ev_valid.size() != (size_t)kEventRing || !ev_valid[it0 % kEventRing]) continue;
            (void)hipEventElapsedTime(&o.ms_X_gram, ev.f1, ev.xg1);
            (void)hipEventElapsedTime(&o.ms_F, ev.f0, ev.f1);
            (void)hipEventElapsedTime(&o.ms_F_kernel, ev.fk0, ev.fk1);
            (void)hipEventElapsedTime(&o.ms_X, ev.f1, ev.x1);
            (void)hipEventElapsedTime(&o.ms_LV, ev.x1, ev.lv1);
        }
        return cnt;
    }

    double objective() {
        if (full) return NAN;
        XState *st = xstate.p;
        if (loss(W.p, true)) return NAN;
        hipLaunchKernelGGL(reduce_rows_kernel, dim3(1), dim3(256), 0, stream, lossrow.p, T, &st->loss1);
        const double l = host_double(&st->loss1);
        {
            ArVecs av{};
            av.v = W.p;
            hipLaunchKernelGGL((ar_tile_kernel<AR_PLAIN>), dim3((T + ar_TI - 1) / ar_TI, KP / kArCols), dim3(kArThreads),
                               ar_tile_lds_bytes(ar_TI, midx, nlag), stream, xp, st, av, 0, 0, 0, lag_set.p, lag_steps.p, nsteps,
                               theta.p, arbase.p, pbase(), ar_TI, 0);
        }
        hipLaunchKernelGGL(reduce_rows_kernel, dim3(1), dim3(256), 0, stream, P(P_AR), nbar, &st->gs);
        const double ar = host_double(&st->gs);
        hipLaunchKernelGGL(reduce_rows_kernel, dim3(1), dim3(256), 0, stream, P(P_VV), nbar, &st->gs);
        const double w2 = host_double(&st->gs);
        log_norm(H.p, (size_t)n * KP, &st->gs);
        const double h2 = host_double(&st->gs);
        return 0.5 * l + 0.5 * lambdaI * (w2 + h2) + 0.5 * lambdaAR * ar;
    }

    int set_heldout(const PyMatrix *Yt, const std::vector<uint32_t> &rows) {
        ho_set = false; ho_m = 0;
        ho_row.release(); ho_col.release(); ho_val.release(); ho_pred.release(); ho_part.release(); ho_sums.release();
        if (!Yt) return 0;
        FillStreamScope fill(stream);
        const uint64_t m = Yt->nnz;
        if (ho_row.upload(rows.data(), m) || ho_col.upload(Yt->col_idx, m) || ho_val.upload((const real *)Yt->val_t, m)) return kFail;
        ho_nb = (int)std::max<uint64_t>(1, std::min<uint64_t>(kHoMaxBlocks, (m + 255) / 256));
        ho_chunk = ((m + ho_nb - 1) / ho_nb + kHoStep - 1) / kHoStep * kHoStep;
        if (ho_chunk == 0) ho_chunk = kHoStep;
        ho_nb = (int)std::max<uint64_t>(1, (m + ho_chunk - 1) / ho_chunk);
        if (ho_part.alloc((size_t)kHoSums * ho_nb, false) || ho_sums.alloc(kHoSums, false)) return kFail;
        TRMF_HIP_CHECK(hipStreamSynchronize(stream));
        ho_m = m; ho_set = true;
        return 0;
    }
    int eval_heldout(TrmfHeldoutSums *out, real *pred) {
        if (!ho_set) { set_error("eval_heldout: no held-out set (trmf_session_set_heldout)"); return kFail; }
        double h[kHoSums] = {0, 0, 0, 0, 0, 0};
        if (ho_m > 0) {
            FillStreamScope fill(stream);
            if (pred && ho_pred.alloc(ho_m, false)) return kFail;
            HeldoutArgs a{ho_row.p, ho_col.p, ho_val.p, W.p, H.p, pred ? ho_pred.p : nullptr, ho_part.p, ho_m, ho_chunk, KP, NT};
            if (!with_nt0(generic ? 0 : NT, [&](auto N) { hipLaunchKernelGGL(heldout_eval_kernel<decltype(N)::value>, dim3(ho_nb), dim3(256), 0, stream, a); }))
                return unsupported_rank();
            hipLaunchKernelGGL(heldout_reduce_kernel, dim3(1), dim3(256), 0, stream, ho_part.p, ho_nb, ho_sums.p);
            TRMF_HIP_CHECK(hipGetLastError());
            TRMF_HIP_CHECK(hipMemcpyAsync(h, ho_sums.p, sizeof h, hipMemcpyDeviceToHost, stream));
            if (pred) TRMF_HIP_CHECK(hipMemcpyAsync(pred, ho_pred.p, ho_m * sizeof(real), hipMemcpyDeviceToHost, stream));
            TRMF_HIP_CHECK(hipStreamSynchronize(stream));
        }
        out->count = (uint64_t)h[0]; out->count_nonzero = (uint64_t)h[1];
        out->sq_err = h[2]; out->abs_err = h[3]; out->abs_truth = h[4]; out->rel_err = h[5];
        return 0;
    }
    int launch_rollout(const real *Wsrc, int T0, int steps, real *roll, real *flat) {
        RolloutArgs a{Wsrc, roll, flat, lag_set.p, theta.p, T0, steps, KP, NT, k, nlag, 0};
        const size_t lds = rollout_lds_bytes(nlag, midx);
        if (midx > 0 && midx <= T0 && lds <= kLdsMax && !test_env("TRMF_FORECAST_GLOBAL")) {
            if (allow_dyn_lds(forecast_rollout_kernel, lds, "forecast roll-out")) return kFail;
            a.reach = midx;
        }
        hipLaunchKernelGGL(forecast_rollout_kernel, dim3((k + 63) / 64), dim3(64), a.reach ? lds : 0, stream, a);
        TRMF_HIP_CHECK(hipGetLastError());
        return 0;
    }
    int forecast(int steps, bool clip, double threshold, const PyMatrix *truth, real *Ynew, real *Wnew) {
        FillStreamScope fill(stream);
        const size_t NY = (size_t)steps * n, NW = (size_t)steps * k, NT6 = (size_t)n * kFcSums;
        const bool score = truth != nullptr;
        DevBuf<real> roll, flat, tru, yd;
        std::vector<real> blk;
        SyncStreamOnExit drain(stream);
        if (roll.alloc((size_t)steps * KP) || (Wnew && flat.alloc(NW, false)) || (Ynew && yd.alloc(NY, false))) return kFail;
        if (score) {
            const real *src = (const real *)truth->val;
            if (truth->type != TRMF_DENSE_ROWMAJOR) { (void)dense_rows_to_rowmajor(truth, blk); src = blk.data(); }
            if (tru.upload(src, NY)) return kFail;
            if (fc_table[0].n != NT6 || fc_table[1].n != NT6 || fc_prev[0].n != (size_t)n || fc_prev[1].n != (size_t)n) {
                if (fc_table[0].alloc(NT6) || fc_table[1].alloc(NT6) || fc_prev[0].alloc(n) || fc_prev[1].alloc(n)) return kFail;
                fc_cur = 0; fc_rows = 0;
// ... 329 lines not shown
```

exp-trmf-nips16_amd/csrc/session_fphase.hpp:

```cpp
#pragma once

#include "session_transport.hpp"

namespace trmf {

struct SessionFPhase : SessionTransport {
    template <int NT_, bool PAD_> void launch_gram_part(const LongRows &L, uint32_t lo, uint32_t hi, const uint32_t *idx, const real *val,
                                                        const real *X, uint32_t zero_row) {
        const uint32_t i0 = L.first[lo], i1 = L.first[hi];
        if (i1 <= i0) return;
        hipLaunchKernelGGL((gram_part_kernel<NT_, PAD_>), dim3((i1 - i0 + 3) / 4), dim3(256), 0, stream, idx, val, X, L.d_items.p, i0, i1,
                           part_slab.p, part_stride, zero_row);
        if (i1 - i0 > hi - lo) {
            const uint32_t bpr = (uint32_t)((part_stride * sizeof(real) / 16 + 255) / 256);
            hipLaunchKernelGGL(split_reduce_kernel, dim3(bpr * (hi - lo)), dim3(256), 0, stream, L.d_first.p, part_slab.p, part_stride, lo, hi, bpr);
        }
    }
    template <int NT_, int KMAX_> int launch_fsolve_mfma(uint32_t rb, uint32_t re) {
        const uint32_t rows = re - rb;
        if (rows == 0) return 0;
#if !defined(TRMF_F32)
        if (longF.any()) {
            uint32_t lo, hi;
            longF.range(rb, re, lo, hi);
            if (hi > lo) {
                launch_gram_part<NT_, false>(longF, lo, hi, Yc_idx.p, Yc_val.p, W.p, (uint32_t)T);
                hipLaunchKernelGGL((fsolve_mfma_long_kernel<NT_, KMAX_>), dim3((hi - lo + 3) / 4), dim3(256), 0, stream, split_view(longF, lo, hi), H.p, k, (real)lambdaI);
            }
        }
        hipLaunchKernelGGL((fsolve_mfma_kernel<NT_, KMAX_>), dim3((rows + 3) / 4), dim3(256), 0, stream,
                           Yc_ptr.p, Yc_idx.p, Yc_val.p, W.p, H.p, rb, re, k, (real)lambdaI, (uint32_t)T, longF.thresh - 1u);
#endif
        return 0;
    }
    template <int NT_, int KMAX_> int launch_fsolve_quad(uint32_t rb, uint32_t re) {
        const uint32_t rows = re - rb;
        if (rows == 0) return 0;
#if defined(TRMF_F32)
        if (longF.any()) {
            uint32_t lo, hi;
            longF.range(rb, re, lo, hi);
            if (hi > lo) {
                launch_gram_part<NT_, (KMAX_ <= kTile * NT_ - 8)>(longF, lo, hi, Yc_idx.p, Yc_val.p, W.p, (uint32_t)T);
                hipLaunchKernelGGL((fsolve_quad_long_kernel<NT_, KMAX_>), dim3((hi - lo + 15) / 16), dim3(256), 0, stream, split_view(longF, lo, hi), H.p, k, (real)lambdaI);
            }
        }
        if (longF.any()) { uint32_t lo, hi; longF.range(rb, re, lo, hi); if (hi - lo == rows) return 0; }
        const dim3 grid((rows + 15) / 16), block(256);
        hipLaunchKernelGGL((fsolve_quad_kernel<NT_, KMAX_>), grid, block, 0, stream, Yc_ptr.p,
                           Yc_idx.p, Yc_val.p, W.p, H.p, rb, re, k, (real)lambdaI, (uint32_t)T, longF.thresh - 1u);
#endif
        return 0;
    }
    int launch_fsolve_rows(uint32_t rb, uint32_t re) {
        if (generic) {
            if (re > rb)
                hipLaunchKernelGGL(gram_generic_kernel<true>, dim3(std::min<uint32_t>(kGenBlocks, re - rb)), dim3(256), gram_generic_lds(k), stream,
                                   Yc_ptr.p, Yc_idx.p, Yc_val.p, W.p, rb, re, k, KP, NT, (real)lambdaI, gen_scratch.p, (size_t)0, H.p);
            return 0;
        }
        return with_kq(KMAX, [&](auto KM) {
            constexpr int KMAX_ = decltype(KM)::value, NT_ = (KMAX_ + kTile - 1) / kTile;
            if (sizeof(real) == 4) launch_fsolve_quad<NT_, KMAX_>(rb, re);
            else launch_fsolve_mfma<NT_, KMAX_>(rb, re);
        }) ? 0 : unsupported_rank();
    }
    int overlap_chunks() {
        if (comm->world <= 1 || full || host_col_ptr.empty()) return 0;
        if (const char *e = test_env("TRMF_FOVERLAP")) { const int c = atoi(e); return c <= 0 ? 0 : std::max(2, std::min(kMaxChunks, c)); }
        uint64_t rows = 0;
        for (int r = 0; r < comm->world; r++) rows = std::max<uint64_t>(rows, fbounds[r + 1] - fbounds[r]);
        uint64_t thresh = kOverlapBytes;
        if (const char *e = test_env("TRMF_FOVERLAP_BYTES")) thresh = std::max<uint64_t>(1, strtoull(e, nullptr, 10));
        const uint64_t bytes = rows * KP * sizeof(real);
        return bytes >= thresh ? (int)std::max<uint64_t>(2, std::min<uint64_t>(kMaxChunks, bytes / thresh)) : 0;
    }
    int fsolve(PhaseEvents &ev) {
        if (fs_mode == kShardMeasure && fs_calls == 2) {
            const int m = decide_shard(fs0, fs1, fs2, "F-solve");
            if (m < 0) return kFail;
            fs_mode = m;
        }
        const bool replicate = fs_mode == kShardOff, measure = fs_mode == kShardMeasure && fs_calls == 1;
        const uint32_t rb = replicate ? 0u : (uint32_t)fbounds[comm->rank];
        const uint32_t re = replicate ? (uint32_t)n : (uint32_t)fbounds[comm->rank + 1];
        const int C = fs_mode == kShardOn ? overlap_chunks() : 0;
        if (C >= 2) {
            const int W_ = comm->world;
            if (!side) {
                TRMF_HIP_CHECK(hipStreamCreateWithFlags(&side, hipStreamNonBlocking));
                TRMF_HIP_CHECK(hipEventCreateWithFlags(&ov_b, hipEventDisableTiming));
                for (hipEvent_t &e : ov_c) TRMF_HIP_CHECK(hipEventCreateWithFlags(&e, hipEventDisableTiming));
            }
            if (fchunks != C || fcut.size() != (size_t)W_ * (C + 1)) {
                fchunks = C; fcut.resize((size_t)W_ * (C + 1));
                for (int r = 0; r < W_; r++) {
                    const uint64_t n0 = host_col_ptr[fbounds[r]], n1 = host_col_ptr[fbounds[r + 1]];
                    fcut[(size_t)r * (C + 1)] = fbounds[r]; fcut[(size_t)r * (C + 1) + C] = fbounds[r + 1];
                    for (int c = 1; c < C; c++)
                        fcut[(size_t)r * (C + 1) + c] = (uint64_t)(std::lower_bound(host_col_ptr.begin() + fbounds[r], host_col_ptr.begin() + fbounds[r + 1],
                                                                                   n0 + (n1 - n0) * c / C) - host_col_ptr.begin());
                }
            }
            const uint64_t rowbytes = (uint64_t)KP * sizeof(real);
            const uint64_t *mine = fcut.data() + (size_t)comm->rank * (C + 1);
            TRMF_EVREC(ev.fk0, stream);
            for (int c = 0; c < C; c++) {
                if (launch_fsolve_rows((uint32_t)mine[c], (uint32_t)mine[c + 1])) return kFail;
                if (c + 1 < C) TRMF_HIP_CHECK(hipEventRecord(ov_c[c], stream));
            }
            TRMF_EVREC(ev.fk1, stream);
            TRMF_HIP_CHECK(hipGetLastError());
            fs_calls++;
            std::vector<uint64_t> gb(W_), ge(W_);
            for (int c = 0; c < C; c++) {
                for (int r = 0; r < W_; r++) { gb[r] = fcut[(size_t)r * (C + 1) + c] * rowbytes; ge[r] = fcut[(size_t)r * (C + 1) + c + 1] * rowbytes; }
                if (c + 1 < C) {
                    TRMF_HIP_CHECK(hipStreamWaitEvent(side, ov_c[c], 0));
                    if (comm->allgatherv_ranges(H.p, gb.data(), ge.data(), side)) return kFail;
                } else {
                    TRMF_HIP_CHECK(hipEventRecord(ov_b, side));
                    if (comm->allgatherv_ranges(H.p, gb.data(), ge.data(), stream)) return kFail;
                    TRMF_HIP_CHECK(hipStreamWaitEvent(stream, ov_b, 0));
                }
            }
            return 0;
        }
        if (measure) TRMF_HIP_CHECK(hipEventRecord(fs0, stream));
        TRMF_EVREC(ev.fk0, stream);
        if (launch_fsolve_rows(rb, re)) return kFail;
        TRMF_EVREC(ev.fk1, stream);
        TRMF_HIP_CHECK(hipGetLastError());
        fs_calls++;
        if (replicate) return 0;
        if (measure) TRMF_HIP_CHECK(hipEventRecord(fs1, stream));
        if (gather_rows(H.p, fbounds, (size_t)KP * sizeof(real))) return kFail;
        if (measure) TRMF_HIP_CHECK(hipEventRecord(fs2, stream));
        return 0;
    }

    template <int NT_> void launch_spmm(const LongRows &L, const uint32_t *ptr, const uint32_t *idx, const real *val, const real *X,
                                        real *out, uint32_t rb, uint32_t re, uint32_t zero_row) {
        if (re <= rb) return;
        if (L.any()) {
            uint32_t lo, hi;
            L.range(rb, re, lo, hi);
            const uint32_t i0 = L.first[lo], i1 = L.first[hi];
            if (i1 > i0) {
                hipLaunchKernelGGL((spmm_part_kernel<NT_>), dim3((i1 - i0 + 3) / 4), dim3(256), 0, stream, idx, val, X, L.d_items.p, i0, i1, part_slab.p, zero_row);
                hipLaunchKernelGGL(spmm_reduce_kernel, dim3((unsigned)(((size_t)(hi - lo) * KP + 255) / 256)), dim3(256), 0, stream, L.d_rows.p, L.d_first.p,
                                   part_slab.p, out, lo, hi, KP);
            }
        }
        hipLaunchKernelGGL((spmm_rows_kernel<NT_>), dim3((re - rb + 3) / 4), dim3(256), 0, stream, ptr, idx, val, X, out, rb, re, zero_row, L.thresh);
    }
    template <int NT_> void launch_dense_tn(const real *A, int K, int M, const real *B, real *out) {
        const int xb = (M + 63) / 64;
        const long long cap = (long long)kGemmChunks * std::max(n, T) / std::max(M, 1);
        const int nchunk = (int)std::max<long long>(1, std::min<long long>({cap, (long long)std::max(1, K / 64), (1024 + xb - 1) / xb}));
        hipLaunchKernelGGL((dense_tn_mfma_kernel<NT_>), dim3(xb, nchunk), dim3(256), 0, stream, A, K, M, B, gemm_part.p);
        if (nchunk <= 16)
            hipLaunchKernelGGL(dense_tn_reduce_flat_kernel, dim3((unsigned)(((size_t)M * KP + 255) / 256)), dim3(256), 0, stream,
                               gemm_part.p, nchunk, M, KP, NT, k, out);
        else
            hipLaunchKernelGGL(dense_tn_reduce_kernel, dim3((unsigned)(((size_t)M * KP + 3) / 4)), dim3(256), 0, stream,
                               gemm_part.p, nchunk, M, KP, NT, k, out);
    }
    int y_times_factor(bool transposed, const real *X, real *out, uint32_t rb, uint32_t re) {
        if (generic) {
            if (!dense) {
                if (re > rb)
                    hipLaunchKernelGGL(spmm_generic_kernel, dim3(std::min<uint32_t>(4096, re - rb)), dim3(256), 0, stream, transposed ? Yc_ptr.p : Yr_ptr.p,
                                       transposed ? Yc_idx.p : Yr_idx.p, transposed ? Yc_val.p : Yr_val.p, X, out, rb, re, k, KP, NT);
            } else {
                const int K = transposed ? T : n, M = transposed ? n : T;
                hipLaunchKernelGGL(dense_tn_generic_kernel, dim3(std::min(4096, std::max(1, M))), dim3(256), 0, stream, transposed ? Yd_tn.p : Yd_nt.p, K, M, X, out, k, KP, NT);
            }
            TRMF_HIP_CHECK(hipGetLastError());
            return 0;
        }
        if (!dense) {
            const uint32_t *ptr = transposed ? Yc_ptr.p : Yr_ptr.p, *idx = transposed ? Yc_idx.p : Yr_idx.p;
            const real *val = transposed ? Yc_val.p : Yr_val.p;
            const uint32_t zr = (uint32_t)(transposed ? T : n);
            if (!with_nt(NT, [&](auto N) { launch_spmm<decltype(N)::value>(transposed ? longF : longX, ptr, idx, val, X, out, rb, re, zr); })) return unsupported_rank();
        } else {
            const real *A = transposed ? Yd_tn.p : Yd_nt.p;
            const int K = transposed ? T : n, M = transposed ? n : T;
            if (!with_nt(NT, [&](auto N) { launch_dense_tn<decltype(N)::value>(A, K, M, X, out); })) return unsupported_rank();
        }
        TRMF_HIP_CHECK(hipGetLastError());
        return 0;
    }
    int small_gram(const real *A, int rows, real lambda, real *GS, hipStream_t stream) {
        if (generic) {
            hipLaunchKernelGGL(small_gram_generic_kernel, dim3(k), dim3(256), 0, stream, A, rows, k, KP, NT, lambda, GS);
            return 0;
        }
        const int nb = std::max(1, std::min(kSmallGramBlocks / 4, rows / 256));
        if (!with_nt(NT, [&](auto N) {
                hipLaunchKernelGGL((small_gram_mfma_kernel<decltype(N)::value>), dim3(nb), dim3(256), 0, stream, A, rows, k, sgram_part.p);
            })) return unsupported_rank();
        hipLaunchKernelGGL(small_gram_reduce_kernel, dim3((k * k + 3) / 4), dim3(256), 0, stream, sgram_part.p, nb * 4, k, lambda, GS);
        return 0;
    }
    int fsolve_full(PhaseEvents &ev) {
        const uint32_t rb = (uint32_t)fbounds[comm->rank], re = (uint32_t)fbounds[comm->rank + 1];
        TRMF_EVREC(ev.fk0, stream);
        hipStream_t gs = stream;
        if (y_times_factor(true, W.p, Bf.p, dense ? 0u : rb, dense ? (uint32_t)n : re)) return kFail;
        if (small_gram(W.p, T, (real)lambdaI, GSf.p, gs)) return kFail;
        if (re > rb && generic) {
            hipLaunchKernelGGL(chol_generic_kernel, dim3(1), dim3(256), 0, stream, GSf.p, Uf.p, k);
            const int nrows = (int)(re - rb);
            hipLaunchKernelGGL(solve_rows_generic_kernel, dim3(std::min(2048, nrows)), dim3(256), (size_t)k * sizeof(real), stream, Uf.p, Bf.p + (size_t)rb * KP,
                               H.p + (size_t)rb * KP, nrows, k, KP, NT);
        } else if (re > rb) {
            const size_t ulds = (size_t)k * k * sizeof(real);
            if (!with_nt(NT, [&](auto N) { hipLaunchKernelGGL(chol_wave_kernel<decltype(N)::value>, dim3(1), dim3(64), 0, gs, GSf.p, Uf.p, k); })) return unsupported_rank();
            const int nrows = (int)(re - rb), nblk = std::max(1, std::min(2048, (nrows + 3) / 4));
            hipLaunchKernelGGL(solve_rows_kernel, dim3(nblk), dim3(256), ulds, stream, Uf.p, Bf.p + (size_t)rb * KP,
                               H.p + (size_t)rb * KP, nrows, k, KP, NT);
        }
        TRMF_EVREC(ev.fk1, stream);
        TRMF_HIP_CHECK(hipGetLastError());
        return gather_rows(H.p, fbounds, (size_t)KP * sizeof(real));
    }

    double fsolve_bytes() const {
        return fs_mode == kShardOff ? bytes_for_rows(0, (uint64_t)n) : bytes_for_rows(fbounds[comm->rank], fbounds[comm->rank + 1]);
    }
    double bytes_for_rows(uint64_t rb, uint64_t re) const {
        const double sz = sizeof(real);
        const double nz = host_col_ptr.empty() ? 0.0 : (double)(host_col_ptr[re] - host_col_ptr[rb]);
        const double rows = (double)(re - rb);
        return nz * (4.0 + sz + k * sz) + (rows + 1) * 8.0 + rows * k * sz;
    }
};

}
```

exp-trmf-nips16_amd/csrc/session_state.hpp:

```cpp
#pragma once

#include <algorithm>
#include <chrono>
#include <cmath>
#include <cstring>
#include <map>
#include <memory>
#include <mutex>
#include <type_traits>
#include <vector>

#include "../../include/trmf_abi.h"
#include "comm.hpp"
#include "dev_buf.hpp"
#include "full_kernels.hpp"
#include "generic_kernels.hpp"
#include "resident_kernels.hpp"
#include "theta_kernels.hpp"

namespace trmf {

std::shared_ptr<Comm> active_comm();

template <int... Vs, class F> bool dispatch_int(int v, F &&f) {
    return ((v == Vs ? (f(std::integral_constant<int, Vs>{}), true) : false) || ...);
}
template <class F> bool with_nt(int nt, F &&f) { return dispatch_int<1, 2, 3, 4>(nt, f); }
template <class F> bool with_nt0(int nt, F &&f) { return dispatch_int<0, 1, 2, 3, 4>(nt, f); }
template <class F> bool with_kq(int kq, F &&f) { return dispatch_int<8, 16, 24, 32, 40, 48, 56, 64>(kq, f); }

struct SessionState {
    int T = 0, n = 0, k = 0, KP = 0, NT = 0, KMAX = 0, nlag = 0, midx = 0;
    uint64_t nnz = 0;
    double lambdaI = 0, lambdaAR = 0, lambdaLag = 0;
    int period_W = 1, period_H = 1, period_Lag = 2, verbose = 0;
    bool log_norms = true;
    int max_cg_iter = 20;
    int max_cg() const { return (int)std::min<long long>(max_cg_iter, (long long)T * k); }
    bool cg_direct = test_env("TRMF_CG_DIRECT") != nullptr && atoi(test_env("TRMF_CG_DIRECT")) != 0;
    double eps_cg = 0.1;
    int iter = 0;
    std::shared_ptr<Comm> comm;
    std::vector<uint64_t> fbounds, xbounds;
    hipStream_t stream = nullptr;
    DevBuf<uint32_t> Yc_ptr, Yc_idx, Yr_ptr, Yr_idx, lag_set, lag_steps;
    int nsteps = 0;
    bool has_lag0 = false;
    DevBuf<real> Yc_val, Yr_val, W, H, theta, G, Bv, g, s, r, r1, d0, d1, Hd, Hd1, w_new;
    DevBuf<double> lossrow, partials, theta_part;
    bool full = false, dense = false;
    DevBuf<real> Yd_tn, Yd_nt;
    DevBuf<real> Bf, GSf, GSx, Uf;
    DevBuf<double> gemm_part, sgram_part;
    double trYTY = 0;
    static constexpr int kGemmChunks = 32, kSmallGramBlocks = 256;
    DevBuf<XState> xstate;
    DevBuf<DeviceIterLog> log;
    static constexpr int kLogCap = 4096;
    std::vector<PhaseEvents> events;
    static constexpr int kEventRing = 64;
    int nbe = 1, nba = 1, rpb = 1;
    bool generic = false;
    DevBuf<real> gen_scratch, theta_scratch;
    bool gpacked = false;
    int tile_TI = 0, nbt = 1;
    int tile_nth = 256;
    DevBuf<double> xmsg_own[3];
    double *xm[3] = {nullptr, nullptr, nullptr};
    TileShard tsh{}, tsh_rank{};
    struct P2p {
        bool on = false;
        bool loopback = false;
        void *arena = nullptr;
        size_t bytes = 0;
        std::vector<void *> peer;
        unsigned long long epoch[3] = {0, 0, 0};
        double *msg[3] = {nullptr, nullptr, nullptr};
        size_t ext_off = 0, ext_bytes = 0;
        size_t ext_ll_bytes = 0;
        std::string note;
    } p2p;
    bool p2p_use = false;
    DevBuf<PeerTable> peer_table;
    std::vector<uint64_t> tbounds;
    bool ts_possible = false;
    enum { kXRep = 0, kXTsComm = 1, kXTsP2p = 2, kXTsPersist = 3, kXForms = 4 };
    int x_form = kXRep;
    std::vector<int> x_cands;
    int x_calls = 0, cg_pred = 4;
    float x_ms[kXForms] = {0, 0, 0, 0};
    double x_ms_all[kXForms] = {0, 0, 0, 0};
    hipEvent_t ts0 = nullptr, ts1 = nullptr;
    int ar_TI = 64, nbar = 1;
    DevBuf<real> arbase;
    XParams xp{};
    static bool test_knobs() { static const bool on = getenv("TRMF_TEST") != nullptr; return on; }
    static int unsupported_rank() { set_error("unsupported rank"); return kFail; }
    static const char *test_env(const char *name) {
        if (test_knobs()) return getenv(name);
        if (getenv(name)) {
            static std::mutex mu; static std::map<std::string, bool> told;
            std::lock_guard<std::mutex> lk(mu);
            if (!told[name]) { told[name] = true; fprintf(stderr, "[trmf] %s is a test knob: ignored unless TRMF_TEST is set\n", name); }
        }
        return nullptr;
    }

    double *pbase_override = nullptr;
    static constexpr int kSumsqBlocks = 1024;
    DevBuf<double> sumsq_part;

    std::vector<uint64_t> host_row_ptr, host_col_ptr;
    double ysq_acc = 0;

    double t_upload_s = 0;
    double bytes_uploaded = 0;
    DevBuf<real> raw_W, raw_H;
    static double now_s() { return std::chrono::duration<double>(std::chrono::steady_clock::now().time_since_epoch()).count(); }
    bool created = false;

    static double sum_squares(const real *v, uint64_t count) {
        double acc = 0;
        for (uint64_t e = 0; e < count; e++) acc += (double)v[e] * (double)v[e];
        return acc;
    }
    static double dense_rows_to_rowmajor(const PyMatrix *Y, std::vector<real> &tn) {
        const size_t R = Y->rows, C = Y->cols;
        const real *v = (const real *)Y->val;
        tn.resize(R * C);
        if (Y->type == TRMF_DENSE_ROWMAJOR) std::memcpy(tn.data(), v, R * C * sizeof(real));
// ... 199 lines not shown
```

exp-trmf-nips16_amd/csrc/session_xphase.hpp:

```cpp
#pragma once

#include "session_fphase.hpp"

namespace trmf {

struct SessionXPhase : SessionFPhase {
    int setup_tile_messages() {
        tsh = TileShard{};
        tsh.rank = 0; tsh.world = 1; tsh.tile0 = 0; tsh.ntiles = nbt; tsh.nbt = nbt; tsh.tpr = std::max(nbt, 1);
        tsh.row_b = 0; tsh.row_e = T; tsh.slot_dbl = (unsigned)nbt * kRecDoubles; tsh.edge_off_dbl = tsh.slot_dbl;
        tsh_rank = tsh;
        ts_possible = false;
        tbounds.assign(comm->world + 1, (uint64_t)T);
        tbounds[0] = 0;
        size_t doubles = (size_t)std::max(nbt, 1) * kRecDoubles;
        const int W_ = comm->world;
        if (tile_TI > 0 && W_ > 1 && !full) {
            const int tpr = (nbt + W_ - 1) / W_;
            const long long last_rows = (long long)T - (long long)(W_ - 1) * tpr * tile_TI;
            if ((long long)(W_ - 1) * tpr < nbt && (long long)tpr * tile_TI >= midx && last_rows >= std::max(midx, 1)) {
                ts_possible = true;
                const size_t edge_bytes = (size_t)2 * kEdgeVecs * midx * KP * sizeof(real);
                tsh_rank.rank = comm->rank; tsh_rank.world = W_; tsh_rank.tpr = tpr;
                tsh_rank.tile0 = comm->rank * tpr; tsh_rank.ntiles = std::min(nbt, (comm->rank + 1) * tpr) - tsh_rank.tile0;
                tsh_rank.row_b = tsh_rank.tile0 * tile_TI; tsh_rank.row_e = std::min(T, (tsh_rank.tile0 + tsh_rank.ntiles) * tile_TI);
                tsh_rank.edge_off_dbl = (unsigned)tpr * kRecDoubles;
                tsh_rank.slot_dbl = tsh_rank.edge_off_dbl + (unsigned)((edge_bytes + 15) / 16 * 2);
                for (int r = 1; r < W_; r++) tbounds[r] = (uint64_t)std::min<long long>(T, (long long)r * tpr * tile_TI);
                doubles = std::max(doubles, (size_t)W_ * tsh_rank.slot_dbl);
            }
        }
        release_p2p();
        for (int m = 0; m < 3; m++) { if (xmsg_own[m].alloc(doubles)) return kFail; xm[m] = xmsg_own[m].p; }
        const char *e = getenv("TRMF_CG");
        const bool ptables = nbt <= kPersistMaxTiles;
        if (ts_possible && ((e && e[0] == 'p') || (!e && !getenv("TRMF_NO_P2P"))) &&
            setup_p2p(doubles, e != nullptr, ptables ? (size_t)2 * nbt * kLLWords * 8 : 0, ptables ? (size_t)2 * T * KP * 2 * sizeof(real) : 0)) return kFail;
        return 0;
    }
    void init_x_forms() {
        x_cands.clear(); x_calls = 0; x_form = kXRep;
        for (int f = 0; f < kXForms; f++) { x_ms[f] = 0; x_ms_all[f] = 0; }
        const char *e = getenv("TRMF_CG");
        const bool fused_ts = tile_TI > 0 && ts_possible;
        if (!fused_ts && !uts) return;
        if (fused_ts && e && e[0] == 'p' && e[1] == 'e') {
            if (!persist_usable_shard()) { x_form = kXTsP2p; persist_note = "TRMF_CG=persist: tiles not co-resident / tables missing, peer-to-peer launches instead"; return; }
            x_form = kXTsPersist; return;
        }
        if (e && e[0] == 'p') { x_form = kXTsP2p; return; }
        if (e && e[0] == 't') { x_form = kXTsComm; return; }
        if (fused_ts && e && e[0] == 'r') { x_form = kXRep; return; }
        if (fused_ts) x_cands.push_back(kXRep);
        x_cands.push_back(kXTsComm);
        if (p2p.on) x_cands.push_back(kXTsP2p);
        const char *at = getenv("TRMF_AUTOTUNE");
        if (fused_ts && p2p.on && !(at && atoi(at) == 0) && persist_usable_shard()) {
            if (max_ranks_per_device == 1) x_cands.push_back(kXTsPersist);
            else persist_note = std::to_string(max_ranks_per_device) + " ranks share one device: the persistent-kernel form is not tried";
        }
        x_form = x_cands.size() == 1 ? x_cands[0] : -1;
    }
    static const char *x_form_name(int f) {
        return f == kXRep ? "replicated" : f == kXTsComm ? "time-sharded (communicator)" : f == kXTsP2p ? "time-sharded (peer to peer)"
             : f == kXTsPersist ? "time-sharded (one persistent kernel per rank, peer to peer)" : "measuring";
    }

    template <int NT_> void launch_gram_x(uint32_t rb, uint32_t re) {
        if (re <= rb) return;
        const uint32_t wpb = longX.skewed ? 1u : 4u;
        const dim3 grid((re - rb + wpb - 1) / wpb), block(64 * wpb), lblock(256);
        uint32_t lo = 0, hi = 0;
        if (longX.any()) longX.range(rb, re, lo, hi);
        const dim3 lgrid((hi - lo + 3) / 4);
        const uint32_t *xorder = (longX.skewed && longX.d_order.p && rb == 0 && re == (uint32_t)T) ? longX.d_order.p : nullptr;
        auto launch = [&](auto Pad, auto Packed) {
            constexpr bool PAD = decltype(Pad)::value, PACKED = decltype(Packed)::value;
            if (hi > lo) {
                launch_gram_part<NT_, PAD>(longX, lo, hi, Yr_idx.p, Yr_val.p, H.p, (uint32_t)n);
                hipLaunchKernelGGL((gram_x_long_kernel<NT_, PAD, PACKED>), lgrid, lblock, 0, stream, split_view(longX, lo, hi), G.p, Bv.p, k, xp.gstride);
            }
            hipLaunchKernelGGL((gram_x_kernel<NT_, PAD, PACKED>), grid, block, 0, stream, Yr_ptr.p, Yr_idx.p, Yr_val.p, H.p, G.p, Bv.p,
                               rb, re, k, (uint32_t)n, xp.gstride, longX.thresh, xorder);
        };
        if (rhs_pad_ok<NT_>(k)) {
            if (gpacked) launch(std::true_type{}, std::true_type{}); else launch(std::true_type{}, std::false_type{});
        } else {
            if (gpacked) launch(std::false_type{}, std::true_type{}); else launch(std::false_type{}, std::false_type{});
        }
    }
    int launch_gram_x_rows(uint32_t rb, uint32_t re) {
        if (generic) {
            if (re > rb)
                hipLaunchKernelGGL(gram_generic_kernel<false>, dim3(std::min<uint32_t>(4096, re - rb)), dim3(256), gram_generic_lds(k), stream,
                                   Yr_ptr.p, Yr_idx.p, Yr_val.p, H.p, rb, re, k, KP, NT, real(0), G.p, xp.gstride, Bv.p);
            return 0;
        }
        return with_nt(NT, [&](auto N) { launch_gram_x<decltype(N)::value>(rb, re); }) ? 0 : unsupported_rank();
    }
    int gram_x(bool timeshard = false) {
        if (timeshard || uts) {
            const uint32_t rb = (uint32_t)(uts ? ush.row_b : tsh_rank.row_b), re = (uint32_t)(uts ? ush.row_e : tsh_rank.row_e);
            if (launch_gram_x_rows(rb, re)) return kFail;
            TRMF_HIP_CHECK(hipGetLastError());
            return 0;
        }
        if (!cg_shard && gramx_mode == kGramxMeasure && gramx_calls == 2 && gramx_decide()) return kFail;
        const bool replicate = gramx_mode == kGramxReplicate && !cg_shard;
        const bool measure = gramx_mode == kGramxMeasure && !cg_shard && gramx_calls == 1;
        const uint32_t rb = replicate ? 0u : (uint32_t)xbounds[comm->rank];
        const uint32_t re = replicate ? (uint32_t)T : (uint32_t)xbounds[comm->rank + 1];
        if (measure) TRMF_HIP_CHECK(hipEventRecord(gx0, stream));
        if (launch_gram_x_rows(rb, re)) return kFail;
        TRMF_HIP_CHECK(hipGetLastError());
        gramx_calls++;
        if (replicate) return 0;
        if (cg_shard) return 0;
        if (measure) TRMF_HIP_CHECK(hipEventRecord(gx1, stream));
        if (gather_rows(G.p, xbounds, xp.gstride * sizeof(real))) return kFail;
        if (gather_rows(Bv.p, xbounds, (size_t)KP * sizeof(real))) return kFail;
        if (measure) TRMF_HIP_CHECK(hipEventRecord(gx2, stream));
        return 0;
    }
    int gramx_decide() {
        const int m = decide_shard(gx0, gx1, gx2, "X-side Gram build");
        if (m < 0) return kFail;
        gramx_mode = m == kShardOff ? kGramxReplicate : kGramxShard;
        return 0;
    }
    int loss(const real *Wv, bool all_rows) {
        const uint32_t rb = all_rows ? 0u : (uint32_t)xbounds[comm->rank];
        const uint32_t re = all_rows ? (uint32_t)T : (uint32_t)xbounds[comm->rank + 1];
        if (generic) {
            if (re > rb) hipLaunchKernelGGL(loss_generic_kernel, dim3(re - rb), dim3(256), 0, stream, Yr_ptr.p, Yr_idx.p, Yr_val.p, H.p, Wv, lossrow.p, rb, re, KP);
        } else if (!with_nt(NT, [&](auto N) {
                       if (re > rb)
                           hipLaunchKernelGGL((loss_kernel<decltype(N)::value>), dim3(re - rb), dim3(256), 0, stream, Yr_ptr.p, Yr_idx.p,
                                              Yr_val.p, H.p, Wv, lossrow.p, rb, re, (uint32_t)n);
                   })) return unsupported_rank();
        TRMF_HIP_CHECK(hipGetLastError());
        return all_rows ? 0 : gather_rows(lossrow.p, xbounds, sizeof(double));
    }
    int xprepare_full() {
        const uint32_t rb = (uint32_t)xbounds[comm->rank], re = (uint32_t)xbounds[comm->rank + 1];
        if (y_times_factor(false, H.p, Bv.p, dense ? 0u : rb, dense ? (uint32_t)T : re)) return kFail;
        if (!dense && gather_rows(Bv.p, xbounds, (size_t)KP * sizeof(real))) return kFail;
        return small_gram(H.p, n, real(0), GSx.p, stream);
    }

    template <class F> void with_tile_form(bool shard, F &&f) const {
        if (shard) f(std::true_type{}, std::integral_constant<int, 256>{});
        else if (tile_nth == 512) f(std::false_type{}, std::integral_constant<int, 512>{});
        else f(std::false_type{}, std::integral_constant<int, 256>{});
    }
    template <int MODE> int launch_hv_tile(bool shard, const HvVecs &a, int it, int last, const double *rec_in, double *rec_out) {
        const size_t lds = hv_tile_lds_bytes(tile_TI, midx, KP, nlag, k);
        const TileShard &sh = shard ? tsh_rank : tsh;
        const PeerTable *pt = (shard && p2p_use) ? peer_table.p : nullptr;
        const int mi = rec_out == xm[0] ? 0 : rec_out == xm[1] ? 1 : 2;
        bool ok = false;
        with_tile_form(shard, [&](auto Shard, auto Nth) {
            constexpr bool SHARD = decltype(Shard)::value;
            constexpr int NTH = decltype(Nth)::value;
            ok = with_kq(hv_kq(k), [&](auto Kq) {
                hipLaunchKernelGGL((hv_tile_kernel<MODE, decltype(Kq)::value, SHARD, NTH>), dim3(sh.ntiles), dim3(NTH), lds, stream, xp, xstate.p, a, sh,
                                   it, last, lag_set.p, theta.p, Gmat(), rec_in, rec_out, pt, mi, tile_TI);
            });
        });
        return ok ? 0 : unsupported_rank();
    }
    int first_stop_check(bool follow, int maxcg) const { return follow ? std::min(maxcg, std::max(1, cg_pred)) : maxcg; }
    int follow_stop(int it, int maxcg, int &upto) {
        if (it == maxcg) cg_pred = maxcg;
        if (it != upto || it == maxcg) return 0;
        int stop = kCgRunning;
        TRMF_HIP_CHECK(hipMemcpyAsync(&stop, &xstate.p->stop_it, sizeof(int), hipMemcpyDeviceToHost, stream));
        TRMF_HIP_CHECK(hipStreamSynchronize(stream));
        if (stop != kCgRunning) { cg_pred = stop; return 1; }
        upto = std::min(maxcg, upto + 2);
        return 0;
    }
    int xsolve_fused(bool shard, int maxcg, XState *log_x, double *log_n) {
        real *dbuf[2] = {d0.p, d1.p}, *rbuf[2] = {r.p, r1.p}, *hbuf[2] = {Hd.p, Hd1.p};
        double *mg = xm[2], *mc[2] = {xm[0], xm[1]};
        HvVecs a{};
        a.v = W.p; a.out = g.p; a.Bv = Bv.p;
        if (launch_hv_tile<HV_GRAD>(shard, a, 0, 0, nullptr, mg)) return kFail;
        if (shard && exchange(2, -1, 1, g.p, nullptr, nullptr)) return kFail;
        a = HvVecs{};
        a.v = g.p; a.s = s.p; a.d_out = dbuf[0]; a.r_out = rbuf[0]; a.out = hbuf[0];
        if (launch_hv_tile<HV_CG_FIRST>(shard, a, 0, 0, mg, mc[0])) return kFail;
        if (shard && exchange(0, 0, 3, dbuf[0], rbuf[0], hbuf[0])) return kFail;
        const bool follow = shard && !p2p_use;
        int upto = first_stop_check(follow, maxcg);
        for (int it = 1; it <= maxcg; it++) {
            a.v = dbuf[(it - 1) & 1]; a.r_in = rbuf[(it - 1) & 1]; a.hd_in = hbuf[(it - 1) & 1];
            a.d_out = dbuf[it & 1]; a.r_out = rbuf[it & 1]; a.out = hbuf[it & 1];
            if (launch_hv_tile<HV_CG_STEP>(shard, a, it, it == maxcg ? 1 : 0, mc[(it - 1) & 1], mc[it & 1])) return kFail;
            if (!shard) continue;
            if (exchange(it & 1, it, 3, dbuf[it & 1], rbuf[it & 1], hbuf[it & 1])) return kFail;
            if (!follow) continue;
            if (const int fs = follow_stop(it, maxcg, upto)) { if (fs == kFail) return kFail; break; }
        }
        const TileShard &sh = shard ? tsh_rank : tsh;
        const PeerTable *pt = (shard && p2p_use) ? peer_table.p : nullptr;
        with_tile_form(shard, [&](auto Shard, auto Nth) {
            constexpr int NTH = decltype(Nth)::value;
            hipLaunchKernelGGL((cg_close_kernel<decltype(Shard)::value, NTH>), dim3(sh.ntiles), dim3(NTH), 0, stream, xp, xstate.p, sh, tile_TI, mc[0],
                               mc[1], dbuf[0], dbuf[1], rbuf[0], rbuf[1], hbuf[0], hbuf[1], s.p, g.p, W.p, w_new.p, mg, pt);
        });
        if (shard && exchange(2, -1, cg_direct ? 1 : 0, cg_direct ? s.p : nullptr, nullptr, nullptr)) return kFail;
        if (cg_direct) {
            a = HvVecs{};
            a.v = s.p; a.out = hbuf[0];
            if (launch_hv_tile<HV_PLAIN>(shard, a, 0, 0, nullptr, mg)) return kFail;
            if (shard && exchange(2, -1, 0, nullptr, nullptr, nullptr)) return kFail;
        }
        const int nb = (int)std::min<size_t>(kMaxPartials, ((size_t)(sh.row_e - sh.row_b) * KP + 255) / 256);
        with_tile_form(shard, [&](auto, auto Nth) {
            constexpr int NTH = decltype(Nth)::value;
            hipLaunchKernelGGL(accept_tile_kernel<NTH>, dim3(std::max(nb, 1)), dim3(NTH), 0, stream, xp, xstate.p, mg, sh, shard ? 1 : 0, w_new.p, W.p,
// ... 394 lines not shown
```

exp-trmf-nips16_amd/csrc/trmf_abi.hip:

```cpp
#include "../../include/trmf_abi.h"

#include <memory>
#include <mutex>
#include <random>

#include "session_group.hpp"

namespace trmf {

static std::string g_last_error = "";
static std::mutex g_err_mu;
static thread_local std::string tl_last_error;
void set_error(const std::string &msg) {
    tl_last_error = msg;
    std::lock_guard<std::mutex> lk(g_err_mu);
    g_last_error = msg;
}

static int g_device = 0;
static std::mutex g_prof_mu;
static TrmfTrainProfile g_last_profile;
static bool g_have_profile = false;
static std::shared_ptr<Comm> g_self = std::make_shared<SelfComm>();
static std::shared_ptr<Comm> g_comm;
// ... 266 lines not shown
                                 const PyMatrix *W, const PyMatrix *H, const PyMatrix *lag_val,
                                 double lambdaI, double lambdaAR, double lambdaLag, int32_t period_W,
                                 int32_t period_H, int32_t period_Lag, int32_t missing, int32_t verbose) {
    DeviceGuard guard;
    return reinterpret_cast<TrmfSession *>(make_session(Y, lag_set, lag_size, W, H, lag_val, lambdaI, lambdaAR,
                                                        lambdaLag, period_W, period_H, period_Lag, missing, verbose));
}
#define HND(s) reinterpret_cast<SessionHandle *>(s)

int32_t trmf_session_run(TrmfSession *s, int32_t iters) {
    if (!s) return kFail;
    DeviceGuard guard;
    return guard.ok ? HND(s)->all([&](TrmfSessionImpl *t) { return t->run(iters); }) : kFail;
}
int32_t trmf_session_log_norms(TrmfSession *s, int32_t on) {
    if (!s) return kFail;
    return HND(s)->all([&](TrmfSessionImpl *t) { t->log_norms = on != 0; return 0; });
}
int32_t trmf_session_set_timing(TrmfSession *s, int32_t period) {
    if (!s || period < 0) return kFail;
    return HND(s)->all([&](TrmfSessionImpl *t) { t->ev_period = period; return 0; });
}
int32_t trmf_session_sync(TrmfSession *s) {
    if (!s) return kFail;
    DeviceGuard guard;
    return guard.ok ? HND(s)->all([&](TrmfSessionImpl *t) { return t->sync(); }) : kFail;
}
int32_t trmf_session_mark(TrmfSession *s) {
    if (!s) return kFail;
    DeviceGuard guard;
    return guard.ok ? HND(s)->all([&](TrmfSessionImpl *t) { return t->mark(); }) : kFail;
}
int32_t trmf_session_rewind(TrmfSession *s) {
    if (!s) return kFail;
    DeviceGuard guard;
    return guard.ok ? HND(s)->all([&](TrmfSessionImpl *t) { return t->rewind(); }) : kFail;
}
int32_t trmf_session_append_rows(TrmfSession *s, const PyMatrix *Ynew) {
    if (!s || !Ynew) { set_error("null session or block"); return kFail; }
    DeviceGuard guard;
    return guard.ok ? HND(s)->all([&](TrmfSessionImpl *t) { return t->append_rows(Ynew); }) : kFail;
}
int32_t trmf_session_rows(TrmfSession *s) { return s ? HND(s)->first()->T : kFail; }
int32_t trmf_session_set_series_transform(TrmfSession *s, const void *a, const void *b) {
    if (!s) { set_error("null session"); return kFail; }
    DeviceGuard guard;
    return guard.ok ? HND(s)->all([&](TrmfSessionImpl *t) { return t->set_series_transform((const real *)a, (const real *)b); }) : kFail;
}

int32_t trmf_session_download(TrmfSession *s, PyMatrix *W, PyMatrix *H, PyMatrix *lag_val) {
    if (!s) return kFail;
    DeviceGuard guard;
    if (!guard.ok) return kFail;
    if (HND(s)->all([&](TrmfSessionImpl *t) { return t->sync(); })) return kFail;
    return HND(s)->rank0([&](TrmfSessionImpl *t) -> int {
        if (W && (W->rows != (uint64_t)t->T || W->cols != (uint64_t)t->k || W->type != TRMF_DENSE_ROWMAJOR)) { set_error("W shape/layout mismatch"); return kFail; }
        if (H && (H->rows != (uint64_t)t->n || H->cols != (uint64_t)t->k || H->type != TRMF_DENSE_ROWMAJOR)) { set_error("H shape/layout mismatch"); return kFail; }
        if (lag_val && (lag_val->rows != (uint64_t)t->nlag || lag_val->cols != (uint64_t)t->k || lag_val->type != TRMF_DENSE_COLMAJOR)) { set_error("lag_val shape/layout mismatch"); return kFail; }
        if (W && t->download_padded(t->W, (real *)W->val, t->T)) return kFail;
        if (H && t->download_padded(t->H, (real *)H->val, t->n)) return kFail;
        if (lag_val && t->nlag)
            TRMF_HIP_CHECK(hipMemcpy(lag_val->val, t->theta.p, sizeof(real) * (size_t)t->nlag * t->k, hipMemcpyDeviceToHost));
        return 0;
    });
}

int32_t trmf_session_stats(TrmfSession *s, TrmfIterStats *out, int32_t cap) {
    if (!(s && out && cap > 0)) return 0;
    DeviceGuard guard;
    if (!guard.ok) return 0;
    if (HND(s)->group && HND(s)->all([&](TrmfSessionImpl *t) { return t->sync(); })) return 0;
    int cnt = 0;
    (void)HND(s)->rank0([&](TrmfSessionImpl *t) { cnt = t->stats(out, cap); return cnt < 0 ? kFail : 0; });
    return cnt < 0 ? 0 : cnt;
}
double trmf_session_objective(TrmfSession *s) {
    if (!s) return NAN;
    DeviceGuard guard;
    if (!guard.ok) return NAN;
    double J = NAN;
    (void)HND(s)->all([&](TrmfSessionImpl *t) { const double v = t->objective(); if (t->comm->rank == 0) J = v; return 0; });
    return J;
}
double trmf_session_fsolve_bytes(TrmfSession *s) { return s ? HND(s)->first()->fsolve_bytes() : 0.0; }
int32_t trmf_session_describe(TrmfSession *s, char *buf, int32_t cap) {
    if (!s) return kFail;
    std::string d = HND(s)->first()->describe();
    if (HND(s)->group) d += "; ranks are threads of this process (TRMF_DEVICES), communicator: " + HND(s)->group->comm_kind;
    if (buf && cap > 0) { std::strncpy(buf, d.c_str(), (size_t)cap - 1); buf[cap - 1] = 0; }
    return (int32_t)d.size();
}
void trmf_session_destroy(TrmfSession *s) {
    if (!s) return;
    DeviceGuard guard;
    delete HND(s);
}

int32_t trmf_session_set_heldout(TrmfSession *s, const PyMatrix *Yt) {
    if (!s) { set_error("null session"); return kFail; }
    const TrmfSessionImpl *f = HND(s)->first();
    std::vector<uint32_t> rows;
    if (Yt) {
        if (Yt->type != TRMF_SPARSE) { set_error("set_heldout: Ytest must be a sparse PyMatrix"); return kFail; }
        if (Yt->cols != (uint64_t)f->n) { set_error("set_heldout: Ytest has " + std::to_string(Yt->cols) + " columns, the session " + std::to_string(f->n)); return kFail; }
        if (Yt->rows > (uint64_t)f->T) { set_error("set_heldout: Ytest has more rows than the session's W (" + std::to_string(f->T) + ")"); return kFail; }
        if (Yt->nnz >= (1ull << 32)) { set_error("set_heldout: Ytest exceeds 32-bit entry indices"); return kFail; }
        if (!Yt->row_ptr || (Yt->nnz && (!Yt->col_idx || !Yt->val_t))) { set_error("set_heldout: Ytest lacks its CSR arrays"); return kFail; }
        if (Yt->row_ptr[0] != 0 || Yt->row_ptr[Yt->rows] != Yt->nnz) { set_error("set_heldout: Ytest row pointers do not span its entries"); return kFail; }
        rows.resize(Yt->nnz);
        for (uint64_t i = 0; i < Yt->rows; i++) {
            const size_t p0 = Yt->row_ptr[i], p1 = Yt->row_ptr[i + 1];
            if (p1 < p0 || p1 > Yt->nnz) { set_error("set_heldout: Ytest row pointers are not ascending"); return kFail; }
            for (size_t e = p0; e < p1; e++) rows[e] = (uint32_t)i;
        }
        for (uint64_t e = 0; e < Yt->nnz; e++)
            if (Yt->col_idx[e] >= (uint32_t)f->n) { set_error("set_heldout: Ytest column index " + std::to_string(Yt->col_idx[e]) + " out of range"); return kFail; }
    }
    DeviceGuard guard;
    return guard.ok ? HND(s)->all([&](TrmfSessionImpl *t) { return t->set_heldout(Yt, rows); }) : kFail;
}
int32_t trmf_session_eval_heldout(TrmfSession *s, TrmfHeldoutSums *out, void *pred) {
    if (!s || !out) { set_error("null session or output"); return kFail; }
    const TrmfSessionImpl *f = HND(s)->first();
    if (!f->ho_set) { set_error("eval_heldout: no held-out set (trmf_session_set_heldout)"); return kFail; }
    if (f->has_transform) { set_error("eval_heldout: the session trains on a series transform; held-out truths would be in another scale"); return kFail; }
    DeviceGuard guard;
    if (!guard.ok) return kFail;
    if (HND(s)->all([&](TrmfSessionImpl *t) { return t->sync(); })) return kFail;
    TrmfHeldoutSums sums{};
    const int rc = HND(s)->rank0([&](TrmfSessionImpl *t) { return t->eval_heldout(&sums, (real *)pred); });
    if (rc == 0) *out = sums;
    return rc;
}
static int check_forecast_args(const TrmfSessionImpl *f, const std::string &what, int32_t steps, int32_t clip, double threshold, const PyMatrix *truth) {
    if (steps < 1) { set_error(what + ": steps must be at least 1"); return kFail; }
    if ((uint64_t)f->T + (uint64_t)steps + 1 >= (1ull << 24) || (uint64_t)steps * (uint64_t)f->n >= (1ull << 32)) {
        set_error(what + ": the window would exceed 32-bit device indices"); return kFail;
    }
    if (clip && !std::isfinite(threshold)) { set_error(what + ": the threshold must be finite"); return kFail; }
    if (truth) {
        if (truth->type != TRMF_DENSE_ROWMAJOR && truth->type != TRMF_DENSE_COLMAJOR) { set_error(what + ": the truth must be a dense PyMatrix"); return kFail; }
        if (truth->rows != (uint64_t)steps || truth->cols != (uint64_t)f->n) {
            set_error(what + ": the truth is " + std::to_string(truth->rows) + " x " + std::to_string(truth->cols) + ", the forecast " + std::to_string(steps) +
                      " x " + std::to_string(f->n));
            return kFail;
        }
        if (!truth->val) { set_error(what + ": the truth lacks its values"); return kFail; }
    }
    return 0;
}
int32_t trmf_session_forecast(TrmfSession *s, int32_t steps, int32_t clip, double threshold, const PyMatrix *truth, void *Ynew, void *Wnew) {
    if (!s) { set_error("null session"); return kFail; }
    if (check_forecast_args(HND(s)->first(), "forecast", steps, clip, threshold, truth)) return kFail;
    DeviceGuard guard;
    if (!guard.ok) return kFail;
    if (HND(s)->all([&](TrmfSessionImpl *t) { return t->sync(); })) return kFail;
    return HND(s)->rank0([&](TrmfSessionImpl *t) { return t->forecast(steps, clip != 0, threshold, truth, (real *)Ynew, (real *)Wnew); });
}
int32_t trmf_session_forecast_scores(TrmfSession *s, uint64_t *rows_scored, TrmfSeriesSums *per_series) {
    if (!s) { set_error("null session"); return kFail; }
    static_assert(sizeof(TrmfSeriesSums) == kFcSums * sizeof(double), "the resident table is an array of TrmfSeriesSums");
    DeviceGuard guard;
    if (!guard.ok) return kFail;
    return HND(s)->rank0([&](TrmfSessionImpl *t) { return t->forecast_scores(rows_scored, reinterpret_cast<double *>(per_series)); });
}
int32_t trmf_session_forecast_reset(TrmfSession *s) {
// ... 180 lines not shown
```

exp-trmf-nips16_amd/trmf/session.py:

```python
import ctypes
from ctypes import POINTER, byref, c_char_p, c_double, c_float, c_int32, c_uint32, c_uint64, c_void_p

import numpy as np
import scipy.sparse as smat

from ._corelib import get_clib
from .rf_util import PyMatrix


class TrmfIterStats(ctypes.Structure):
    _fields_ = [('normF', c_double), ('normX', c_double), ('normLV', c_double),
                ('f', c_double), ('fnew', c_double), ('actred', c_double), ('prered', c_double),
                ('gnorm', c_double), ('cg_rnorm', c_double),
                ('cg_iter', c_int32), ('accepted', c_int32),
                ('ms_F', c_float), ('ms_X', c_float), ('ms_LV', c_float), ('ms_F_kernel', c_float),
                ('delta', c_double), ('cg_rnorm_direct', c_double), ('ms_X_gram', c_float), ('reserved_', c_float)]

    def as_dict(self):
        return {name: getattr(self, name) for name, _ in self._fields_}


class TrmfHeldoutSums(ctypes.Structure):
    _fields_ = [('count', c_uint64), ('count_nonzero', c_uint64), ('sq_err', c_double), ('abs_err', c_double),
                ('abs_truth', c_double), ('rel_err', c_double)]

    def as_dict(self):
        return {name: getattr(self, name) for name, _ in self._fields_}


class TrmfSeriesSums(ctypes.Structure):
    _fields_ = [('abs_err', c_double), ('sq_err', c_double), ('abs_truth', c_double), ('abs_dtruth', c_double),
                ('rel_err', c_double), ('count_nonzero', c_double)]

    def as_dict(self):
        return {name: getattr(self, name) for name, _ in self._fields_}


class TrmfAssimilateSums(ctypes.Structure):
    _fields_ = [('rows', c_uint64), ('entries', c_uint64), ('sq_err_before', c_double), ('sq_err_after', c_double)]

    def as_dict(self):
        return {name: getattr(self, name) for name, _ in self._fields_}


class TrmfNoiseStats(ctypes.Structure):
    _fields_ = [('pooled_sigma2', c_double), ('sigma2_min', c_double), ('sigma2_max', c_double), ('series_pooled', c_uint64),
                ('q_min', c_double), ('q_max', c_double)]

    def as_dict(self):
        return {name: getattr(self, name) for name, _ in self._fields_}


class TrmfIntervalSums(ctypes.Structure):
    _fields_ = [('cells', c_double), ('covered', c_double), ('sd_sum', c_double), ('abs_truth', c_double), ('z2_sum', c_double),
                ('nll_sum', c_double), ('crps_sum', c_double)]

    def as_dict(self):
        return {name: getattr(self, name) for name, _ in self._fields_}


class TrmfTrainProfile(ctypes.Structure):
    _fields_ = [('total_s', c_double), ('setup_s', c_double), ('upload_s', c_double), ('compute_s', c_double),
                ('download_s', c_double), ('teardown_s', c_double), ('bytes_h2d', c_double), ('bytes_d2h', c_double),
                ('iters', c_int32), ('device_mallocs', c_int32), ('pool_reused', c_int32), ('failed', c_int32)]

    def as_dict(self):
        return {name: getattr(self, name) for name, _ in self._fields_}


ALLGATHERV_FN = ctypes.CFUNCTYPE(c_int32, c_void_p, POINTER(c_uint64), c_int32, c_void_p)
_prototyped = set()


def bind(lib):
    if id(lib) in _prototyped:
        return lib
    P = POINTER(PyMatrix)
    lib.trmf_sizeof_real.restype = c_int32
    lib.trmf_device_count.restype = c_int32
    lib.trmf_set_device.argtypes = [c_int32]; lib.trmf_set_device.restype = c_int32
    lib.trmf_last_error.restype = c_char_p
    lib.trmf_device_free_bytes.restype = ctypes.c_int64
    lib.trmf_last_train_profile.argtypes = [POINTER(TrmfTrainProfile)]; lib.trmf_last_train_profile.restype = c_int32
    lib.trmf_release_cached.restype = c_int32
    lib.trmf_session_create.argtypes = [P, POINTER(c_uint32), c_uint32, P, P, P, c_double, c_double, c_double,
                                        c_int32, c_int32, c_int32, c_int32, c_int32]
    lib.trmf_session_create.restype = c_void_p
    lib.trmf_session_run.argtypes = [c_void_p, c_int32]; lib.trmf_session_run.restype = c_int32
    lib.trmf_session_log_norms.argtypes = [c_void_p, c_int32]; lib.trmf_session_log_norms.restype = c_int32
    lib.trmf_session_set_timing.argtypes = [c_void_p, c_int32]; lib.trmf_session_set_timing.restype = c_int32
    lib.trmf_session_sync.argtypes = [c_void_p]; lib.trmf_session_sync.restype = c_int32
    if hasattr(lib, 'trmf_session_mark'):
        lib.trmf_session_mark.argtypes = [c_void_p]; lib.trmf_session_mark.restype = c_int32
        lib.trmf_session_rewind.argtypes = [c_void_p]; lib.trmf_session_rewind.restype = c_int32
    lib.trmf_session_append_rows.argtypes = [c_void_p, P]; lib.trmf_session_append_rows.restype = c_int32
    lib.trmf_session_rows.argtypes = [c_void_p]; lib.trmf_session_rows.restype = c_int32
    lib.trmf_session_set_series_transform.argtypes = [c_void_p, c_void_p, c_void_p]
    lib.trmf_session_set_series_transform.restype = c_int32
    lib.trmf_session_download.argtypes = [c_void_p, P, P, P]; lib.trmf_session_download.restype = c_int32
    lib.trmf_session_stats.argtypes = [c_void_p, POINTER(TrmfIterStats), c_int32]
    lib.trmf_session_stats.restype = c_int32
    lib.trmf_session_objective.argtypes = [c_void_p]; lib.trmf_session_objective.restype = c_double
    lib.trmf_session_fsolve_bytes.argtypes = [c_void_p]; lib.trmf_session_fsolve_bytes.restype = c_double
    lib.trmf_session_describe.argtypes = [c_void_p, ctypes.c_char_p, c_int32]; lib.trmf_session_describe.restype = c_int32
    lib.trmf_session_destroy.argtypes = [c_void_p]; lib.trmf_session_destroy.restype = None
    if hasattr(lib, 'trmf_session_set_heldout'):
        lib.trmf_session_set_heldout.argtypes = [c_void_p, P]; lib.trmf_session_set_heldout.restype = c_int32
        lib.trmf_session_eval_heldout.argtypes = [c_void_p, POINTER(TrmfHeldoutSums), c_void_p]
        lib.trmf_session_eval_heldout.restype = c_int32
        lib.trmf_session_set_lambdas.argtypes = [c_void_p, c_double, c_double, c_double]
        lib.trmf_session_set_lambdas.restype = c_int32
    if hasattr(lib, 'trmf_session_forecast'):
        lib.trmf_session_forecast.argtypes = [c_void_p, c_int32, c_int32, c_double, P, c_void_p, c_void_p]
        lib.trmf_session_forecast.restype = c_int32
        lib.trmf_session_forecast_scores.argtypes = [c_void_p, POINTER(c_uint64), c_void_p]
        lib.trmf_session_forecast_scores.restype = c_int32
        lib.trmf_session_forecast_reset.argtypes = [c_void_p]; lib.trmf_session_forecast_reset.restype = c_int32
    if hasattr(lib, 'trmf_session_set_lag_penalty'):
        lib.trmf_session_set_lag_penalty.argtypes = [c_void_p, c_double, c_int32]; lib.trmf_session_set_lag_penalty.restype = c_int32
        lib.trmf_session_solve_lags.argtypes = [c_void_p]; lib.trmf_session_solve_lags.restype = c_int32
        lib.trmf_session_lag_stats.argtypes = [c_void_p, c_void_p, POINTER(c_int32), POINTER(c_int32)]
        lib.trmf_session_lag_stats.restype = c_int32
    if hasattr(lib, 'trmf_session_assimilate'):
        lib.trmf_session_assimilate.argtypes = [c_void_p, c_int32, POINTER(TrmfAssimilateSums), c_void_p]
        lib.trmf_session_assimilate.restype = c_int32
    if hasattr(lib, 'trmf_session_fit_noise'):
        lib.trmf_session_fit_noise.argtypes = [c_void_p, POINTER(TrmfNoiseStats)]; lib.trmf_session_fit_noise.restype = c_int32
        lib.trmf_session_noise.argtypes = [c_void_p, c_void_p, c_void_p]; lib.trmf_session_noise.restype = c_int32
        lib.trmf_session_set_noise.argtypes = [c_void_p, c_void_p, c_void_p]; lib.trmf_session_set_noise.restype = c_int32
        lib.trmf_session_forecast_dist.argtypes = [c_void_p, c_int32, c_int32, c_double, c_double, P, c_void_p, c_void_p, c_void_p]
        lib.trmf_session_forecast_dist.restype = c_int32
        lib.trmf_session_interval_scores.argtypes = [c_void_p, POINTER(c_uint64), c_void_p]
        lib.trmf_session_interval_scores.restype = c_int32
        lib.trmf_session_interval_reset.argtypes = [c_void_p]; lib.trmf_session_interval_reset.restype = c_int32
    lib.trmf_dist_get_unique_id.argtypes = [c_void_p]; lib.trmf_dist_get_unique_id.restype = c_int32
    lib.trmf_dist_init.argtypes = [c_int32, c_int32, c_void_p]; lib.trmf_dist_init.restype = c_int32
    lib.trmf_dist_init_callback.argtypes = [c_int32, c_int32, ALLGATHERV_FN, c_void_p]
    lib.trmf_dist_init_callback.restype = c_int32
    lib.trmf_dist_init_solo.argtypes = [c_int32, c_int32]; lib.trmf_dist_init_solo.restype = c_int32
    lib.trmf_dist_rank.restype = c_int32
    lib.trmf_dist_world.restype = c_int32
    lib.trmf_dist_finalize.restype = None
    lib.trmf_partition_by_nnz.argtypes = [c_uint64, POINTER(c_uint64), c_int32, POINTER(c_uint64)]
    lib.trmf_partition_by_nnz.restype = c_int32
    _prototyped.add(id(lib))
    return lib


def lib_for(dtype):
    return bind(get_clib().lib_for(dtype))


def train_profile(dtype):
    prof = TrmfTrainProfile()
    return prof.as_dict() if lib_for(dtype).trmf_last_train_profile(byref(prof)) == 0 else None


def check_lag_penalty(lambdaLagL1, lag_refit=False):
    try:
        l1 = float(lambdaLagL1)
    except (TypeError, ValueError):
        raise TypeError('lambdaLagL1 must be a number, not {!r}'.format(lambdaLagL1))
    if not np.isfinite(l1) or l1 < 0:
        raise ValueError('lambdaLagL1 must be finite and not negative, not {!r}'.format(lambdaLagL1))
    return l1, bool(lag_refit)


class Session(object):

    def __init__(self, Y, model, lambdaI=0.1, lambdaAR=0.1, lambdaLag=0.1,
                 period_W=1, period_H=1, period_Lag=2, missing=True, verbose=0, log_norms=True, timing=1,
                 lambdaLagL1=0.0, lag_refit=False):
        lambdaLagL1, lag_refit = check_lag_penalty(lambdaLagL1, lag_refit)
        self.handle = None
        self.model = model
        self.lib = lib_for(model.W.dtype)
        self.pyY = Y if isinstance(Y, PyMatrix) else PyMatrix(Y, dtype=model.W.dtype)
        self.handle = self.lib.trmf_session_create(
            byref(self.pyY), model.lag_set.ctypes.data_as(POINTER(c_uint32)), len(model.lag_set),
            byref(model.pyW), byref(model.pyH), byref(model.pylag_val),
            lambdaI, lambdaAR, lambdaLag, period_W, period_H, period_Lag, int(missing), verbose)
        if not self.handle:
            raise RuntimeError('trmf_session_create failed: ' + self.lib.trmf_last_error().decode())
        if not log_norms:
            self.lib.trmf_session_log_norms(self.handle, 0)
        if timing != 1:
# ... 152 lines not shown
        table = np.zeros((self.model.n, len(TrmfSeriesSums._fields_)), dtype=np.float64)
        self._check(self.lib.trmf_session_forecast_scores(self.handle, byref(rows), table.ctypes.data), 'trmf_session_forecast_scores')
        return int(rows.value), table

    def forecast_scores(self):
        from .metrics import Metrics
        return Metrics.from_series_sums(*self.forecast_series_sums())

    def reset_forecast_scores(self):
        self._check(self.lib.trmf_session_forecast_reset(self.handle), 'trmf_session_forecast_reset')
        return self

    def fit_noise(self):
        stats = TrmfNoiseStats()
        self._check(self.lib.trmf_session_fit_noise(self.handle, byref(stats)), 'trmf_session_fit_noise')
        return stats.as_dict()

    def noise(self):
        sigma2, q = np.zeros(self.model.n, dtype=np.float64), np.zeros(self.model.k, dtype=np.float64)
        self._check(self.lib.trmf_session_noise(self.handle, sigma2.ctypes.data, q.ctypes.data), 'trmf_session_noise')
        return sigma2, q

    def set_noise(self, sigma2, q):
        sigma2 = np.ascontiguousarray(sigma2, dtype=np.float64).ravel()
        q = np.ascontiguousarray(q, dtype=np.float64).ravel()
        if sigma2.shape != (self.model.n,) or q.shape != (self.model.k,):
            raise ValueError('set_noise: sigma2 must have n = {} values and q k = {}'.format(self.model.n, self.model.k))
        self._check(self.lib.trmf_session_set_noise(self.handle, sigma2.ctypes.data, q.ctypes.data), 'trmf_session_set_noise')
        return self

    def forecast_dist(self, steps, level=0.9, threshold=None, truth=None, return_latent=False):
        from .uncertainty import z_of_level
        dt = np.dtype(self.model.W.dtype)
        n, k = self.model.n, self.model.k
        steps = int(steps)
        zq = z_of_level(level)
        pyT = self._truth_matrix(truth, 'forecast_dist')
        Ynew = np.empty((max(steps, 0), n), dtype=dt)
        Ysd = np.empty((max(steps, 0), n), dtype=dt)
        Wnew = np.empty((max(steps, 0), k), dtype=dt) if return_latent else None
        self._check(self.lib.trmf_session_forecast_dist(
            self.handle, steps, int(threshold is not None), float(threshold) if threshold is not None else 0.0, zq,
            byref(pyT) if pyT is not None else None, Ynew.ctypes.data, Ysd.ctypes.data,
            Wnew.ctypes.data if Wnew is not None else None), 'trmf_session_forecast_dist')
        return (Ynew, Ysd, Wnew) if return_latent else (Ynew, Ysd)

    def forecast_interval(self, steps, level=0.9, threshold=None, truth=None):
        from .uncertainty import z_of_level
        Ynew, Ysd = self.forecast_dist(steps, level=level, threshold=threshold, truth=truth)
        half = Ysd * Ynew.dtype.type(z_of_level(level))
        lo, hi = Ynew - half, Ynew + half
        if threshold is not None:
            np.maximum(lo, Ynew.dtype.type(threshold), out=lo)
        return Ynew, lo, hi

    def interval_series_sums(self):
        rows = c_uint64(0)
        table = np.zeros((self.model.n, len(TrmfIntervalSums._fields_)), dtype=np.float64)
        self._check(self.lib.trmf_session_interval_scores(self.handle, byref(rows), table.ctypes.data), 'trmf_session_interval_scores')
        return int(rows.value), table

    def interval_scores(self, level=0.9):
        from .uncertainty import IntervalMetrics
        return IntervalMetrics.from_series_sums(self.interval_series_sums()[1], level)

    def reset_interval_scores(self):
        self._check(self.lib.trmf_session_interval_reset(self.handle), 'trmf_session_interval_reset')
        return self

    def download(self):
        m = self.model
        self._check(self.lib.trmf_session_download(self.handle, byref(m.pyW), byref(m.pyH), byref(m.pylag_val)),
                    'trmf_session_download')
        return m

    def stats(self, last=64):
        buf = (TrmfIterStats * last)()
        cnt = self._check(self.lib.trmf_session_stats(self.handle, buf, last), 'trmf_session_stats')
        return [buf[i].as_dict() for i in range(cnt)]

    def objective(self):
        return self.lib.trmf_session_objective(self.handle)

    def fsolve_bytes(self):
        return self.lib.trmf_session_fsolve_bytes(self.handle)

    def describe(self):
        buf = ctypes.create_string_buffer(1024)
        self._check(self.lib.trmf_session_describe(self.handle, buf, len(buf)), 'trmf_session_describe')
        return buf.value.decode()

    def close(self):
        if getattr(self, 'handle', None):
            self.lib.trmf_session_destroy(self.handle)
            self.handle = None

    __del__ = close

    def __enter__(self):
        return self

    def __exit__(self, *exc):
        self.close()


def partition_by_nnz(ptr, world, dtype=np.float32):
    ptr = np.ascontiguousarray(ptr, dtype=np.uint64)
    bounds = np.zeros(world + 1, dtype=np.uint64)
    lib = lib_for(dtype)
    rc = lib.trmf_partition_by_nnz(len(ptr) - 1, ptr.ctypes.data_as(POINTER(c_uint64)), world,
                                   bounds.ctypes.data_as(POINTER(c_uint64)))
    if rc != 0:
        raise RuntimeError(lib.trmf_last_error().decode())
    return bounds
```

include/trmf_abi.h:

```cpp
#ifndef TRMF_ABI_H
#define TRMF_ABI_H

#include <stddef.h>
#include <stdint.h>

#if defined(__GNUC__) || defined(__clang__)
#define TRMF_API __attribute__((visibility("default")))
#else
#define TRMF_API
#endif

#ifdef __cplusplus
extern "C" {
#endif


enum {
    TRMF_DENSE_ROWMAJOR = 1,
    TRMF_DENSE_COLMAJOR = 2,
    TRMF_SPARSE = 3,
    TRMF_EYE = 4
};

typedef struct {
    uint64_t rows, cols, nnz;
    size_t *row_ptr;
    size_t *col_ptr;
    uint32_t *row_idx;
    uint32_t *col_idx;
    void *val;
    void *val_t;
    int32_t type;
} PyMatrix;

TRMF_API void c_trmf_train(const PyMatrix *pyY, uint32_t *py_lag_set, uint32_t py_lag_size,
                  PyMatrix *pyW, PyMatrix *pyH, PyMatrix *pylag_val, int warm_start,
                  double lambdaI, double lambdaAR, double lambdaLag,
                  int32_t max_iter, int32_t period_W, int32_t period_H, int32_t period_Lag,
                  int32_t threads, int32_t missing, int32_t verbose);


typedef struct {
    double total_s, setup_s, upload_s, compute_s, download_s, teardown_s;
    double bytes_h2d, bytes_d2h;
    int32_t iters, device_mallocs, pool_reused, failed;
} TrmfTrainProfile;
TRMF_API int32_t trmf_last_train_profile(TrmfTrainProfile *out);
TRMF_API int32_t trmf_release_cached(void);

TRMF_API int32_t trmf_sizeof_real(void);
TRMF_API int32_t trmf_device_count(void);
TRMF_API int32_t trmf_set_device(int32_t device);
TRMF_API int64_t trmf_device_free_bytes(void);
TRMF_API const char *trmf_last_error(void);

typedef struct {
    double normF, normX, normLV;
    double f, fnew, actred, prered;
    double gnorm, cg_rnorm;
    int32_t cg_iter, accepted;
    float ms_F, ms_X, ms_LV;
    float ms_F_kernel;
    double delta;
    double cg_rnorm_direct;
    float ms_X_gram;
    float reserved_;
} TrmfIterStats;

typedef struct TrmfSession TrmfSession;

TRMF_API TrmfSession *trmf_session_create(const PyMatrix *Y, const uint32_t *lag_set, uint32_t lag_size,
                                 const PyMatrix *W, const PyMatrix *H, const PyMatrix *lag_val,
                                 double lambdaI, double lambdaAR, double lambdaLag,
                                 int32_t period_W, int32_t period_H, int32_t period_Lag,
                                 int32_t missing, int32_t verbose);
TRMF_API int32_t trmf_session_run(TrmfSession *s, int32_t iters);
TRMF_API int32_t trmf_session_log_norms(TrmfSession *s, int32_t on);
TRMF_API int32_t trmf_session_set_timing(TrmfSession *s, int32_t period);
TRMF_API int32_t trmf_session_append_rows(TrmfSession *s, const PyMatrix *Ynew);
TRMF_API int32_t trmf_session_set_series_transform(TrmfSession *s, const void *a , const void *b );
TRMF_API int32_t trmf_session_mark(TrmfSession *s);
TRMF_API int32_t trmf_session_rewind(TrmfSession *s);
TRMF_API int32_t trmf_session_rows(TrmfSession *s);
TRMF_API int32_t trmf_session_sync(TrmfSession *s);
TRMF_API int32_t trmf_session_download(TrmfSession *s, PyMatrix *W, PyMatrix *H, PyMatrix *lag_val);
TRMF_API int32_t trmf_session_stats(TrmfSession *s, TrmfIterStats *out, int32_t cap);
TRMF_API double trmf_session_objective(TrmfSession *s);
TRMF_API double trmf_session_fsolve_bytes(TrmfSession *s);
TRMF_API int32_t trmf_session_describe(TrmfSession *s, char *buf, int32_t cap);
TRMF_API void trmf_session_destroy(TrmfSession *s);

typedef struct {
    uint64_t count, count_nonzero;
    double sq_err, abs_err, abs_truth, rel_err;
} TrmfHeldoutSums;
TRMF_API int32_t trmf_session_set_heldout(TrmfSession *s, const PyMatrix *Ytest);
TRMF_API int32_t trmf_session_eval_heldout(TrmfSession *s, TrmfHeldoutSums *out, void *pred);
TRMF_API int32_t trmf_session_set_lambdas(TrmfSession *s, double lambdaI, double lambdaAR, double lambdaLag);

TRMF_API int32_t trmf_session_set_lag_penalty(TrmfSession *s, double lambdaLagL1, int32_t refit);
TRMF_API int32_t trmf_session_solve_lags(TrmfSession *s);
TRMF_API int32_t trmf_session_lag_stats(TrmfSession *s, int32_t *per_dim , int32_t *capped, int32_t *refit_skipped);

typedef struct {
    double abs_err, sq_err, abs_truth, abs_dtruth, rel_err, count_nonzero;
} TrmfSeriesSums;
TRMF_API int32_t trmf_session_forecast(TrmfSession *s, int32_t steps, int32_t clip, double threshold, const PyMatrix *truth,
                                       void *Ynew, void *Wnew);
TRMF_API int32_t trmf_session_forecast_scores(TrmfSession *s, uint64_t *rows_scored, TrmfSeriesSums *per_series);
TRMF_API int32_t trmf_session_forecast_reset(TrmfSession *s);

typedef struct {
    uint64_t rows, entries;
    double sq_err_before, sq_err_after;
} TrmfAssimilateSums;
TRMF_API int32_t trmf_session_assimilate(TrmfSession *s, int32_t first_row, TrmfAssimilateSums *out ,
                                         void *Wnew );

typedef struct {
    double pooled_sigma2;
    double sigma2_min, sigma2_max;
    uint64_t series_pooled;
    double q_min, q_max;
} TrmfNoiseStats;
TRMF_API int32_t trmf_session_fit_noise(TrmfSession *s, TrmfNoiseStats *out );
TRMF_API int32_t trmf_session_noise(TrmfSession *s, double *sigma2 , double *q );
TRMF_API int32_t trmf_session_set_noise(TrmfSession *s, const double *sigma2 , const double *q );
typedef struct {
    double cells, covered, sd_sum, abs_truth, z2_sum, nll_sum, crps_sum;
} TrmfIntervalSums;
TRMF_API int32_t trmf_session_forecast_dist(TrmfSession *s, int32_t steps, int32_t clip, double threshold, double zq,
                                            const PyMatrix *truth, void *Ynew, void *Ysd, void *Wnew);
TRMF_API int32_t trmf_session_interval_scores(TrmfSession *s, uint64_t *rows_scored, TrmfIntervalSums *per_series);
TRMF_API int32_t trmf_session_interval_reset(TrmfSession *s);

#define TRMF_UNIQUE_ID_BYTES 128
TRMF_API int32_t trmf_dist_get_unique_id(void *out_id );
TRMF_API int32_t trmf_dist_init(int32_t rank, int32_t world, const void *id );
typedef int32_t (*trmf_allgatherv_fn)(void *buf, const uint64_t *offsets, int32_t world,
                                      void *ctx);
TRMF_API int32_t trmf_dist_init_callback(int32_t rank, int32_t world, trmf_allgatherv_fn allgatherv,
                                void *ctx);
TRMF_API int32_t trmf_dist_init_solo(int32_t rank, int32_t world);
TRMF_API int32_t trmf_dist_rank(void);
TRMF_API int32_t trmf_dist_world(void);
TRMF_API void trmf_dist_finalize(void);
TRMF_API int32_t trmf_partition_by_nnz(uint64_t nrows, const size_t *ptr, int32_t world,
                              uint64_t *bounds );

#ifdef __cplusplus
}
#endif
#endif
```

Measured before the change: 1245.

## Pack sparse entries into interleaved index/value records with pre-scaled offsets

The sparse matrix's separate index and value arrays are replaced by an array-of-structs record per nonzero. Each record holds a byte offset already multiplied by the row pitch plus the value. The gram, fsolve, spmm and loss kernels now load each entry with a single wider buffer load instead of two, and no longer do the per-entry umul24 scaling. This costs extra device memory for the record arrays and a one-time conversion kernel. A gram_x download entry point is also added for debugging or inspection.

```diff
diff --git a/exp-trmf-nips16_amd/csrc/full_kernels.hpp b/exp-trmf-nips16_amd/csrc/full_kernels.hpp
--- a/exp-trmf-nips16_amd/csrc/full_kernels.hpp
+++ b/exp-trmf-nips16_amd/csrc/full_kernels.hpp
@@ -9,20 +9,18 @@
 #if !defined(TRMF_UNIT_BODIES)
 template <int NT>
 __global__ void spmm_rows_kernel(const uint32_t *__restrict__ ptr,
-                                                        const uint32_t *__restrict__ idx,
-                                                        const real *__restrict__ val,
+                                                        const uint32_t *__restrict__ rec,
                                                         const real *__restrict__ X,
                                                         real *__restrict__ out, uint32_t row_begin,
                                                         uint32_t row_end, uint32_t zero_row, uint32_t long_thresh);
 template <int NT>
-__global__ void spmm_part_kernel(const uint32_t *__restrict__ idx, const real *__restrict__ val, const real *__restrict__ X,
+__global__ void spmm_part_kernel(const uint32_t *__restrict__ rec, const real *__restrict__ X,
                                  const uint32_t *__restrict__ items, uint32_t item_begin, uint32_t item_end, real *__restrict__ part,
                                  uint32_t zero_row);
 #else
 template <int NT, bool ITEM>
 __device__ __forceinline__ void spmm_body(const uint32_t *__restrict__ ptr,
-                                                        const uint32_t *__restrict__ idx,
-                                                        const real *__restrict__ val,
+                                                        const uint32_t *__restrict__ rec,
                                                         const real *__restrict__ X,
                                                         real *__restrict__ out, uint32_t row_begin,
                                                         uint32_t row_end, uint32_t zero_row, uint32_t long_thresh) {
@@ -40,7 +38,7 @@
 #pragma unroll
     for (int q = 0; q < NT; q++) nowq[q] = 0;
     if (p1 > p0)
-        gram_ring<NT, kRingDepth, false, false>(st, idx, val, X, zero_row, 4u, lane, nowq, GramDesc{p0, p1, 0},
+        gram_ring<NT, kRingDepth, false, false>(st, rec, X, zero_row, 4u, lane, nowq, GramDesc{p0, p1, 0},
                                                 SingleRowStream{4u * kRingDepth}, [](int) {});
 #pragma unroll
     for (int q = 0; q < NT; q++) {
@@ -52,18 +50,17 @@
 }
 template <int NT>
 __global__ __launch_bounds__(256) void spmm_rows_kernel(const uint32_t *__restrict__ ptr,
-                                                        const uint32_t *__restrict__ idx,
-                                                        const real *__restrict__ val,
+                                                        const uint32_t *__restrict__ rec,
                                                         const real *__restrict__ X,
                                                         real *__restrict__ out, uint32_t row_begin,
                                                         uint32_t row_end, uint32_t zero_row, uint32_t long_thresh) {
-    spmm_body<NT, false>(ptr, idx, val, X, out, row_begin, row_end, zero_row, long_thresh);
-}
-template <int NT>
-__global__ __launch_bounds__(256) void spmm_part_kernel(const uint32_t *__restrict__ idx, const real *__restrict__ val,
+    spmm_body<NT, false>(ptr, rec, X, out, row_begin, row_end, zero_row, long_thresh);
+}
+template <int NT>
+__global__ __launch_bounds__(256) void spmm_part_kernel(const uint32_t *__restrict__ rec,
                                                         const real *__restrict__ X, const uint32_t *__restrict__ items,
                                                         uint32_t item_begin, uint32_t item_end, real *__restrict__ part, uint32_t zero_row) {
-    spmm_body<NT, true>(items, idx, val, X, part, item_begin, item_end, zero_row, 0u);
+    spmm_body<NT, true>(items, rec, X, part, item_begin, item_end, zero_row, 0u);
 }
 #endif
 
diff --git a/exp-trmf-nips16_amd/csrc/gram_kernels.hpp b/exp-trmf-nips16_amd/csrc/gram_kernels.hpp
--- a/exp-trmf-nips16_amd/csrc/gram_kernels.hpp
+++ b/exp-trmf-nips16_amd/csrc/gram_kernels.hpp
@@ -131,9 +131,36 @@
     }
 }
 
+constexpr uint32_t kEntryWords = 1u + (uint32_t)(sizeof(real) / 4u);
+constexpr uint32_t kEntryBytes = 4u * kEntryWords;
+typedef uint32_t EntryWords2 __attribute__((ext_vector_type(2)));
+typedef uint32_t EntryWords3 __attribute__((ext_vector_type(3)));
+__device__ __forceinline__ void load_entry_record(__amdgpu_buffer_rsrc_t rsrc, uint32_t byte_off, uint32_t &off, float &y) {
+    const EntryWords2 w = __builtin_amdgcn_raw_buffer_load_b64(rsrc, byte_off, 0, 0);
+    const uint32_t ybits = w.y;
+    off = w.x; y = __builtin_bit_cast(float, ybits);
+}
+__device__ __forceinline__ void load_entry_record(__amdgpu_buffer_rsrc_t rsrc, uint32_t byte_off, uint32_t &off, double &y) {
+    const EntryWords3 w = __builtin_amdgcn_raw_buffer_load_b96(rsrc, byte_off, 0, 0);
+    const uint32_t lo = w.y, hi = w.z;
+    off = w.x; y = __builtin_bit_cast(double, ((unsigned long long)hi << 32) | lo);
+}
+__device__ __forceinline__ void store_entry_record(uint32_t *r, uint32_t off, float y) { r[0] = off; r[1] = __builtin_bit_cast(uint32_t, y); }
+__device__ __forceinline__ void store_entry_record(uint32_t *r, uint32_t off, double y) {
+    const unsigned long long b = __builtin_bit_cast(unsigned long long, y);
+    r[0] = off; r[1] = (uint32_t)b; r[2] = (uint32_t)(b >> 32);
+}
+#if !defined(TRMF_UNIT)
+__global__ __launch_bounds__(256) void entry_records_kernel(const uint32_t *__restrict__ idx, const real *__restrict__ val,
+                                                            uint32_t *__restrict__ rec, size_t count, uint32_t pitch_bytes) {
+    for (size_t e = (size_t)blockIdx.x * 256 + threadIdx.x; e < count; e += (size_t)gridDim.x * 256) {
+        store_entry_record(rec + e * kEntryWords, idx[e] * pitch_bytes, val[e]);
+    }
+}
+#endif
+
 template <int NT, int D, bool DO_MMA, bool WITH_LOSS, bool RHS_PAD = false, bool TAIL = false, bool ROWEND = false, typename Next, typename RowDone>
-__device__ __forceinline__ void gram_ring(GramState<NT> &st, const uint32_t *__restrict__ idx,
-                                          const real *__restrict__ val, const real *__restrict__ X,
+__device__ __forceinline__ void gram_ring(GramState<NT> &st, const uint32_t *__restrict__ rec, const real *__restrict__ X,
                                           uint32_t zero_row, uint32_t estride, int lane,
                                           const real (&wq)[NT], GramDesc d0, Next &&next,
                                           RowDone &&row_done) {
@@ -145,6 +172,7 @@
     const uint32_t lane_bytes = (uint32_t)NT * c * (uint32_t)sizeof(real);
     uint32_t jraw; real yraw; bool vraw;
     uint32_t jsel; real ysel;
+    const uint32_t zero_off = zero_row * (uint32_t)(KP * sizeof(real));
 
     const uint32_t lane_e = (c & 3u) * estride + g;
     auto load_entries = [&](const GramDesc &d) {
@@ -152,15 +180,12 @@
         uint32_t left;
         asm("s_max_u32 %0, %1, %2\n\ts_sub_u32 %0, %0, %2" : "=&s"(left) : "s"(endu), "s"(e0u) : "scc");
         vraw = lane_e < left;
-        const __amdgpu_buffer_rsrc_t ir = __builtin_amdgcn_make_buffer_rsrc(const_cast<uint32_t *>(idx + e0u), 0, (int)(left * 4u), 0x00020000);
-        const __amdgpu_buffer_rsrc_t vr = __builtin_amdgcn_make_buffer_rsrc(const_cast<real *>(val + e0u), 0, (int)(left * (uint32_t)sizeof(real)), 0x00020000);
-        jraw = __builtin_amdgcn_raw_buffer_load_b32(ir, lane_e * 4u, 0, 0);
-        real yv[1];
-        load_factor_slice(yv, vr, lane_e * (uint32_t)sizeof(real));
-        yraw = yv[0];
+        const __amdgpu_buffer_rsrc_t er = __builtin_amdgcn_make_buffer_rsrc(const_cast<uint32_t *>(rec + (size_t)e0u * kEntryWords), 0,
+                                                                            (int)(left * kEntryBytes), 0x00020000);
+        load_entry_record(er, lane_e * kEntryBytes, jraw, yraw);
     };
     auto promote_entries = [&]() {
-        jsel = __umul24(vraw ? jraw : zero_row, (uint32_t)(KP * sizeof(real)));
+        jsel = vraw ? jraw : zero_off;
         ysel = yraw;
     };
     auto load_slices = [&](auto U, real (&x)[D][NT], real (&yx)[D]) {
@@ -317,8 +342,7 @@
 #if !defined(TRMF_UNIT_BODIES)
 template <int NT, int KMAX>
 __global__ void fsolve_mfma_kernel(const uint32_t *__restrict__ ptr,
-                                                                          const uint32_t *__restrict__ idx,
-                                                                          const real *__restrict__ val,
+                                                                          const uint32_t *__restrict__ rec,
                                                                           const real *__restrict__ X,
                                                                           real *__restrict__ F, uint32_t row_begin,
                                                                           uint32_t row_end, int k, real lambda,
@@ -328,8 +352,7 @@
 #else
 template <int NT, int KMAX, bool LONG>
 __device__ __forceinline__ void fsolve_mfma_body(const uint32_t *__restrict__ ptr,
-                                                                          const uint32_t *__restrict__ idx,
-                                                                          const real *__restrict__ val,
+                                                                          const uint32_t *__restrict__ rec,
                                                                           const real *__restrict__ X,
                                                                           real *__restrict__ F, uint32_t row_begin,
                                                                           uint32_t row_end, int k, real lambda,
@@ -363,7 +386,7 @@
         real nowq[NT];
 #pragma unroll
         for (int q = 0; q < NT; q++) nowq[q] = 0;
-        gram_ring<NT, kRingDepth, true, false, false, true>(st, idx, val, X, zero_row, 4u, lane, nowq, GramDesc{p0, p1, 0},
+        gram_ring<NT, kRingDepth, true, false, false, true>(st, rec, X, zero_row, 4u, lane, nowq, GramDesc{p0, p1, 0},
                                                             SingleRowStream{4u * kRingDepth}, [](int) {});
     }
     real y = 0, dinv = 1;
@@ -476,17 +499,16 @@
 }
 template <int NT, int KMAX>
 __global__ __launch_bounds__(256, kMfmaWaves) void fsolve_mfma_kernel(const uint32_t *__restrict__ ptr,
-                                                                          const uint32_t *__restrict__ idx,
-                                                                          const real *__restrict__ val,
+                                                                          const uint32_t *__restrict__ rec,
                                                                           const real *__restrict__ X,
                                                                           real *__restrict__ F, uint32_t row_begin,
                                                                           uint32_t row_end, int k, real lambda,
                                                                           uint32_t zero_row, uint32_t long_m1) {
-    fsolve_mfma_body<NT, KMAX, false>(ptr, idx, val, X, F, row_begin, row_end, k, lambda, zero_row, long_m1, SplitRows{});
+    fsolve_mfma_body<NT, KMAX, false>(ptr, rec, X, F, row_begin, row_end, k, lambda, zero_row, long_m1, SplitRows{});
 }
 template <int NT, int KMAX>
 __global__ __launch_bounds__(256, kMfmaWaves) void fsolve_mfma_long_kernel(SplitRows sp, real *__restrict__ F, int k, real lambda) {
-    fsolve_mfma_body<NT, KMAX, true>(nullptr, nullptr, nullptr, nullptr, F, 0u, 0u, k, lambda, 0u, 0u, sp);
+    fsolve_mfma_body<NT, KMAX, true>(nullptr, nullptr, nullptr, F, 0u, 0u, k, lambda, 0u, 0u, sp);
 }
 #endif
 #endif
@@ -596,8 +618,7 @@
 #if !defined(TRMF_UNIT_BODIES)
 template <int NT, int KMAX>
 __global__ void fsolve_quad_kernel(const uint32_t *__restrict__ ptr,
-                                                          const uint32_t *__restrict__ idx,
-                                                          const float *__restrict__ val,
+                                                          const uint32_t *__restrict__ rec,
                                                           const float *__restrict__ X,
                                                           float *__restrict__ F, uint32_t row_begin,
                                                           uint32_t row_end, int k, float lambda,
@@ -607,8 +628,7 @@
 #else
 template <int NT, int KMAX, bool LONG>
 __device__ __forceinline__ void fsolve_quad_body(const uint32_t *__restrict__ ptr,
-                                                          const uint32_t *__restrict__ idx,
-                                                          const float *__restrict__ val,
+                                                          const uint32_t *__restrict__ rec,
                                                           const float *__restrict__ X,
                                                           float *__restrict__ F, uint32_t row_begin,
                                                           uint32_t row_end, int k, float lambda,
@@ -698,7 +718,7 @@
         float nowq[NT];
 #pragma unroll
         for (int q = 0; q < NT; q++) nowq[q] = 0;
-        gram_ring<NT, kRingDepth, true, false, PAD, false, quad_row_end(NT, KMAX)>(st, idx, val, X, zero_row, 4u, lane, nowq, stream.first(), stream,
+        gram_ring<NT, kRingDepth, true, false, PAD, false, quad_row_end(NT, KMAX)>(st, rec, X, zero_row, 4u, lane, nowq, stream.first(), stream,
                                                     finalize);
     }
 
@@ -714,17 +734,16 @@
 }
 template <int NT, int KMAX>
 __global__ __launch_bounds__(256, quad_waves(NT)) void fsolve_quad_kernel(const uint32_t *__restrict__ ptr,
-                                                          const uint32_t *__restrict__ idx,
-                                                          const float *__restrict__ val,
+                                                          const uint32_t *__restrict__ rec,
                                                           const float *__restrict__ X,
                                                           float *__restrict__ F, uint32_t row_begin,
                                                           uint32_t row_end, int k, float lambda,
                                                           uint32_t zero_row, uint32_t long_m1) {
-    fsolve_quad_body<NT, KMAX, false>(ptr, idx, val, X, F, row_begin, row_end, k, lambda, zero_row, long_m1, SplitRows{});
+    fsolve_quad_body<NT, KMAX, false>(ptr, rec, X, F, row_begin, row_end, k, lambda, zero_row, long_m1, SplitRows{});
 }
 template <int NT, int KMAX>
 __global__ __launch_bounds__(256, quad_waves(NT) - 1) void fsolve_quad_long_kernel(SplitRows sp, float *__restrict__ F, int k, float lambda) {
-    fsolve_quad_body<NT, KMAX, true>(nullptr, nullptr, nullptr, nullptr, F, 0u, 0u, k, lambda, 0u, 0u, sp);
+    fsolve_quad_body<NT, KMAX, true>(nullptr, nullptr, nullptr, F, 0u, 0u, k, lambda, 0u, 0u, sp);
 }
 #endif
 
@@ -733,8 +752,7 @@
 #if !defined(TRMF_UNIT_BODIES)
 template <int NT, bool RHS_PAD, bool PACKED>
 __global__ void gram_x_kernel(const uint32_t *__restrict__ ptr,
-                                                     const uint32_t *__restrict__ idx,
-                                                     const real *__restrict__ val,
+                                                     const uint32_t *__restrict__ rec,
                                                      const real *__restrict__ Hf,
                                                      real *__restrict__ G, real *__restrict__ Bv,
                                                      uint32_t row_begin, uint32_t row_end, int k,
@@ -742,12 +760,12 @@
 template <int NT, bool RHS_PAD, bool PACKED>
 __global__ void gram_x_long_kernel(SplitRows sp, real *__restrict__ G, real *__restrict__ Bv, int k, size_t gs);
 template <int NT, bool RHS_PAD>
-__global__ void gram_part_kernel(const uint32_t *__restrict__ idx, const real *__restrict__ val, const real *__restrict__ X,
+__global__ void gram_part_kernel(const uint32_t *__restrict__ rec, const real *__restrict__ X,
                                  const uint32_t *__restrict__ items, uint32_t item_begin, uint32_t item_end,
                                  real *__restrict__ slab, uint32_t stride, uint32_t zero_row);
 #else
 template <int NT, bool RHS_PAD>
-__global__ __launch_bounds__(256) void gram_part_kernel(const uint32_t *__restrict__ idx, const real *__restrict__ val,
+__global__ __launch_bounds__(256) void gram_part_kernel(const uint32_t *__restrict__ rec,
                                                         const real *__restrict__ X, const uint32_t *__restrict__ items,
                                                         uint32_t item_begin, uint32_t item_end, real *__restrict__ slab,
                                                         uint32_t stride, uint32_t zero_row) {
@@ -764,7 +782,7 @@
 #pragma unroll
     for (int q = 0; q < NT; q++) nowq[q] = 0;
     if (p1 > p0)
-        gram_ring<NT, kRingDepth, true, false, RHS_PAD>(st, idx, val, X, zero_row, 4u, lane, nowq, GramDesc{p0, p1, 0},
+        gram_ring<NT, kRingDepth, true, false, RHS_PAD>(st, rec, X, zero_row, 4u, lane, nowq, GramDesc{p0, p1, 0},
                                                         SingleRowStream{4u * kRingDepth}, [](int) {});
     real *p = slab + (size_t)item * stride;
 #pragma unroll
@@ -777,8 +795,7 @@
 
 template <int NT, bool RHS_PAD, bool PACKED, bool LONG>
 __device__ __forceinline__ void gram_x_body(const uint32_t *__restrict__ ptr,
-                                                     const uint32_t *__restrict__ idx,
-                                                     const real *__restrict__ val,
+                                                     const uint32_t *__restrict__ rec,
                                                      const real *__restrict__ Hf,
                                                      real *__restrict__ G, real *__restrict__ Bv,
                                                      uint32_t row_begin, uint32_t row_end, int k,
@@ -807,7 +824,7 @@
 #pragma unroll
     for (int q = 0; q < NT; q++) nowq[q] = 0;
     if (p1 > p0)
-        gram_ring<NT, kRingDepth, true, false, RHS_PAD>(st, idx, val, Hf, zero_row, 4u, lane, nowq, GramDesc{p0, p1, 0},
+        gram_ring<NT, kRingDepth, true, false, RHS_PAD>(st, rec, Hf, zero_row, 4u, lane, nowq, GramDesc{p0, p1, 0},
                                                         SingleRowStream{4u * kRingDepth}, [](int) {});
     }
     if constexpr (RHS_PAD) {
@@ -853,25 +870,23 @@
 }
 template <int NT, bool RHS_PAD, bool PACKED>
 __global__ __launch_bounds__(256) void gram_x_kernel(const uint32_t *__restrict__ ptr,
-                                                     const uint32_t *__restrict__ idx,
-                                                     const real *__restrict__ val,
+                                                     const uint32_t *__restrict__ rec,
                                                      const real *__restrict__ Hf,
                                                      real *__restrict__ G, real *__restrict__ Bv,
                                                      uint32_t row_begin, uint32_t row_end, int k,
                                                      uint32_t zero_row, size_t gs, uint32_t long_thresh, const uint32_t *__restrict__ order) {
-    gram_x_body<NT, RHS_PAD, PACKED, false>(ptr, idx, val, Hf, G, Bv, row_begin, row_end, k, zero_row, gs, long_thresh, SplitRows{}, order);
+    gram_x_body<NT, RHS_PAD, PACKED, false>(ptr, rec, Hf, G, Bv, row_begin, row_end, k, zero_row, gs, long_thresh, SplitRows{}, order);
 }
 template <int NT, bool RHS_PAD, bool PACKED>
 __global__ __launch_bounds__(256) void gram_x_long_kernel(SplitRows sp, real *__restrict__ G, real *__restrict__ Bv, int k, size_t gs) {
-    gram_x_body<NT, RHS_PAD, PACKED, true>(nullptr, nullptr, nullptr, nullptr, G, Bv, 0u, 0u, k, 0u, gs, 0u, sp, nullptr);
+    gram_x_body<NT, RHS_PAD, PACKED, true>(nullptr, nullptr, nullptr, G, Bv, 0u, 0u, k, 0u, gs, 0u, sp, nullptr);
 }
 #endif
 
 #if !defined(TRMF_UNIT_BODIES)
 template <int NT>
 __global__ void loss_kernel(const uint32_t *__restrict__ ptr,
-                                                   const uint32_t *__restrict__ idx,
-                                                   const real *__restrict__ val,
+                                                   const uint32_t *__restrict__ rec,
                                                    const real *__restrict__ Hf,
                                                    const real *__restrict__ W,
                                                    double *__restrict__ lossrow,
@@ -880,8 +895,7 @@
 #else
 template <int NT>
 __global__ __launch_bounds__(256) void loss_kernel(const uint32_t *__restrict__ ptr,
-                                                   const uint32_t *__restrict__ idx,
-                                                   const real *__restrict__ val,
+                                                   const uint32_t *__restrict__ rec,
                                                    const real *__restrict__ Hf,
                                                    const real *__restrict__ W,
                                                    double *__restrict__ lossrow,
@@ -903,7 +917,7 @@
         const uint32_t e0 = (uint32_t)__builtin_amdgcn_readfirstlane((int)(p0 + 4u * (uint32_t)wave));
         const uint32_t e1 = (uint32_t)__builtin_amdgcn_readfirstlane((int)p1);
         GramDesc d0{e0, e1, e0 < e1 ? 0 : -1};
-        gram_ring<NT, kRingDepth, false, true>(st, idx, val, Hf, zero_row, 16u, lane, wq, d0,
+        gram_ring<NT, kRingDepth, false, true>(st, rec, Hf, zero_row, 16u, lane, wq, d0,
                                                SingleRowStream{16u * kRingDepth}, [](int) {});
     }
     double l = (c == 0) ? st.loss : 0.0;
diff --git a/exp-trmf-nips16_amd/csrc/kernel_units.hpp b/exp-trmf-nips16_amd/csrc/kernel_units.hpp
--- a/exp-trmf-nips16_amd/csrc/kernel_units.hpp
+++ b/exp-trmf-nips16_amd/csrc/kernel_units.hpp
@@ -62,7 +62,7 @@
     X void cg_persist_kernel<64, SHARD, NTH> TRMF_PERSIST_SIG;
 #define TRMF_UNIT_PERSIST(X) TRMF_PERSIST_KQS(X, false, 256) TRMF_PERSIST_KQS(X, true, 256) TRMF_PERSIST_KQS(X, false, 512)
 
-#define TRMF_FSOLVE_SIG (const uint32_t *, const uint32_t *, const real *, const real *, real *, uint32_t, uint32_t, int, real, uint32_t, uint32_t)
+#define TRMF_FSOLVE_SIG (const uint32_t *, const uint32_t *, const real *, real *, uint32_t, uint32_t, int, real, uint32_t, uint32_t)
 #define TRMF_FSOLVE_LONG_SIG (SplitRows, real *, int, real)
 #if defined(TRMF_F32)
 #define TRMF_FSOLVE_ONE(X, NT, KMAX) X void fsolve_quad_kernel<NT, KMAX> TRMF_FSOLVE_SIG;
@@ -71,9 +71,9 @@
 #define TRMF_FSOLVE_ONE(X, NT, KMAX) X void fsolve_mfma_kernel<NT, KMAX> TRMF_FSOLVE_SIG;
 #define TRMF_FSOLVE_LONG_ONE(X, NT, KMAX) X void fsolve_mfma_long_kernel<NT, KMAX> TRMF_FSOLVE_LONG_SIG;
 #endif
-#define TRMF_GRAMX_SIG (const uint32_t *, const uint32_t *, const real *, const real *, real *, real *, uint32_t, uint32_t, int, uint32_t, size_t, uint32_t, const uint32_t *)
+#define TRMF_GRAMX_SIG (const uint32_t *, const uint32_t *, const real *, real *, real *, uint32_t, uint32_t, int, uint32_t, size_t, uint32_t, const uint32_t *)
 #define TRMF_GRAMX_LONG_SIG (SplitRows, real *, real *, int, size_t)
-#define TRMF_GRAM_PART_SIG (const uint32_t *, const real *, const real *, const uint32_t *, uint32_t, uint32_t, real *, uint32_t, uint32_t)
+#define TRMF_GRAM_PART_SIG (const uint32_t *, const real *, const uint32_t *, uint32_t, uint32_t, real *, uint32_t, uint32_t)
 #define TRMF_SPLIT_NT(X, NT)                                               \
     X void gram_part_kernel<NT, true> TRMF_GRAM_PART_SIG;                  \
     X void gram_part_kernel<NT, false> TRMF_GRAM_PART_SIG;                 \
@@ -90,7 +90,7 @@
     X void gram_x_kernel<NT, true, false> TRMF_GRAMX_SIG;        \
     X void gram_x_kernel<NT, false, true> TRMF_GRAMX_SIG;        \
     X void gram_x_kernel<NT, false, false> TRMF_GRAMX_SIG;
-#define TRMF_LOSS_SIG (const uint32_t *, const uint32_t *, const real *, const real *, const real *, double *, uint32_t, uint32_t, uint32_t)
+#define TRMF_LOSS_SIG (const uint32_t *, const uint32_t *, const real *, const real *, double *, uint32_t, uint32_t, uint32_t)
 #define TRMF_UNIT_GRAM(X)                                                                                                    \
     TRMF_FSOLVE_ONE(X, 1, 8) TRMF_FSOLVE_ONE(X, 1, 16) TRMF_FSOLVE_ONE(X, 2, 24) TRMF_FSOLVE_ONE(X, 2, 32)                   \
     TRMF_FSOLVE_ONE(X, 3, 40) TRMF_FSOLVE_ONE(X, 3, 48) TRMF_FSOLVE_ONE(X, 4, 56) TRMF_FSOLVE_ONE(X, 4, 64)                  \
@@ -99,8 +99,8 @@
 
 #define TRMF_APPLY_SHARED_SIG (XParams, const XState *, int, const real *, const real *, const real *, const real *, const real *, int, real *, int, double *, int, int, int)
 #define TRMF_FULL_NT(X, NT)                                                                                                              \
-    X void spmm_rows_kernel<NT>(const uint32_t *, const uint32_t *, const real *, const real *, real *, uint32_t, uint32_t, uint32_t, uint32_t);  \
-    X void spmm_part_kernel<NT>(const uint32_t *, const real *, const real *, const uint32_t *, uint32_t, uint32_t, real *, uint32_t);  \
+    X void spmm_rows_kernel<NT>(const uint32_t *, const uint32_t *, const real *, real *, uint32_t, uint32_t, uint32_t, uint32_t);  \
+    X void spmm_part_kernel<NT>(const uint32_t *, const real *, const uint32_t *, uint32_t, uint32_t, real *, uint32_t);  \
     X void dense_tn_mfma_kernel<NT>(const real *, int, int, const real *, double *);                                                    \
     X void small_gram_mfma_kernel<NT>(const real *, int, int, double *);                                                                \
     X void chol_wave_kernel<NT>(const real *, real *, int);                                                                             \
diff --git a/exp-trmf-nips16_amd/csrc/session.hpp b/exp-trmf-nips16_amd/csrc/session.hpp
--- a/exp-trmf-nips16_amd/csrc/session.hpp
+++ b/exp-trmf-nips16_amd/csrc/session.hpp
@@ -85,6 +85,15 @@
         if (dst.alloc(count, false)) return kFail;
         return HostStager::current().h2d_narrow(dst.p, (const uint64_t *)src, count, stream);
     }
+    int build_entry_records(const uint32_t *idx, const real *val, DevBuf<uint32_t> &rec, size_t count) {
+        if (generic) return 0;
+        if (rec.alloc(count * kEntryWords, false)) return kFail;
+        if (!count) return 0;
+        const unsigned blocks = (unsigned)std::min<size_t>((count + 255) / 256, 8192);
+        hipLaunchKernelGGL(entry_records_kernel, dim3(blocks), dim3(256), 0, stream, idx, val, rec.p, count, (uint32_t)(KP * sizeof(real)));
+        TRMF_HIP_CHECK(hipGetLastError());
+        return 0;
+    }
     int launch_sum_squares(const real *dv, size_t count) {
         if (sumsq_part.alloc(kSumsqBlocks)) return kFail;
         hipLaunchKernelGGL(sumsq_values_kernel, dim3(kSumsqBlocks), dim3(256), 0, stream, dv, count, sumsq_part.p);
@@ -104,7 +113,7 @@
     size_t footprint_estimate() const {
         const size_t sz = sizeof(real), NVb = (size_t)(T + 1) * KP * sz, NHb = (size_t)(n + 1) * KP * sz;
         size_t b = dense ? 2 * (size_t)T * n * sz + (full ? (size_t)kGemmChunks * std::max(T, n) * KP * sz : 0)
-                         : 2 * (size_t)nnz * (4 + sz) + ((size_t)T + n + 2) * 4;
+                         : 2 * (size_t)nnz * (4 + sz) + ((size_t)T + n + 2) * 4 + (generic ? 0 : 2 * (size_t)nnz * kEntryBytes);
         b += NVb + NHb + (size_t)(T + n) * k * sz;
         b += 11 * NVb + 4 * NVb;
         if (!full) b += (size_t)T * k * k * sz;
@@ -137,6 +146,7 @@
             if (Yr_idx.upload(Y->col_idx, nnz)) return kFail;
             if (Yr_val.upload((const real *)Y->val_t, nnz)) return kFail;
             if (launch_sum_squares(Yr_val.p, nnz)) return kFail;
+            if (build_entry_records(Yc_idx.p, Yc_val.p, Yc_rec, nnz) || build_entry_records(Yr_idx.p, Yr_val.p, Yr_rec, nnz)) return kFail;
             bytes_uploaded += 2.0 * (double)nnz * (4 + sizeof(real)) + 8.0 * ((double)T + n + 2);
         } else {
             const size_t N = (size_t)T * n;
@@ -378,7 +388,7 @@
         std::vector<uint64_t> new_row_ptr, new_col_ptr;
         uint64_t new_nnz = nnz;
         double new_ysq = ysq_acc;
-        DevBuf<uint32_t> ptr2, idx2, cptr2, cidx2; DevBuf<real> val2, cval2, tn2, nt2, raw2, W2;
+        DevBuf<uint32_t> ptr2, idx2, cptr2, cidx2, rec2, crec2; DevBuf<real> val2, cval2, tn2, nt2, raw2, W2;
         SyncStreamOnExit drain(stream);
         if (!dense) {
             const uint64_t nz0 = nnz, nzn = Yn->nnz, nz1 = nz0 + nzn;
@@ -402,6 +412,7 @@
             hipLaunchKernelGGL(csc_append_kernel, dim3((n + 3) / 4), dim3(256), 0, stream, Yc_ptr.p, Yc_idx.p, Yc_val.p, wptr.p, widx.p,
                                wval.p, cptr2.p, cidx2.p, cval2.p, n, (uint32_t)T0);
             TRMF_HIP_CHECK(hipGetLastError());
+            if (build_entry_records(idx2.p, val2.p, rec2, nz1) || build_entry_records(cidx2.p, cval2.p, crec2, nz1)) return kFail;
             TRMF_HIP_CHECK(hipStreamSynchronize(stream));
             new_nnz = nz1;
             if (device_sum_squares(val2.p, new_nnz, &new_ysq)) return kFail;
@@ -434,6 +445,7 @@
         if (!dense) {
             Yr_ptr.swap(ptr2); Yr_idx.swap(idx2); Yr_val.swap(val2);
             Yc_ptr.swap(cptr2); Yc_idx.swap(cidx2); Yc_val.swap(cval2);
+            Yr_rec.swap(rec2); Yc_rec.swap(crec2);
             host_row_ptr.swap(new_row_ptr); host_col_ptr.swap(new_col_ptr);
         } else {
             Yd_tn.swap(tn2); Yd_nt.swap(nt2);
@@ -792,6 +804,27 @@
         return cnt;
     }
 
+    int download_gram_x(real *G_out, real *b_out) {
+        if (full || comm->world > 1) { set_error("gram_x: needs the observed-entries objective (missing = 1) on one rank"); return kFail; }
+        if (launch_gram_x_rows(0u, (uint32_t)T)) return kFail;
+        TRMF_HIP_CHECK(hipGetLastError());
+        TRMF_HIP_CHECK(hipStreamSynchronize(stream));
+        const size_t gs = xp.gstride;
+        std::vector<real> g((size_t)T * gs), b((size_t)T * KP);
+        TRMF_HIP_CHECK(hipMemcpy(g.data(), G.p, g.size() * sizeof(real), hipMemcpyDeviceToHost));
+        TRMF_HIP_CHECK(hipMemcpy(b.data(), Bv.p, b.size() * sizeof(real), hipMemcpyDeviceToHost));
+        for (int i = 0; i < T; i++) {
+            const real *gi = g.data() + (size_t)i * gs;
+            real *go = G_out + (size_t)i * k * k;
+            for (int s = 0; s < k; s++)
+                for (int t = 0; t < k; t++) {
+                    const int lo = std::min(s, t), hi = std::max(s, t);
+                    go[(size_t)s * k + t] = gpacked ? gi[(size_t)lo * k - (size_t)lo * (lo - 1) / 2 + (hi - lo)] : gi[(size_t)s * k + t];
+                }
+            for (int t = 0; t < k; t++) b_out[(size_t)i * k + t] = b[(size_t)i * KP + t];
+        }
+        return 0;
+    }
     double objective() {
         if (full) return NAN;
         XState *st = xstate.p;
diff --git a/exp-trmf-nips16_amd/csrc/session_fphase.hpp b/exp-trmf-nips16_amd/csrc/session_fphase.hpp
--- a/exp-trmf-nips16_amd/csrc/session_fphase.hpp
+++ b/exp-trmf-nips16_amd/csrc/session_fphase.hpp
@@ -5,11 +5,11 @@
 namespace trmf {
 
 struct SessionFPhase : SessionTransport {
-    template <int NT_, bool PAD_> void launch_gram_part(const LongRows &L, uint32_t lo, uint32_t hi, const uint32_t *idx, const real *val,
-                                                        const real *X, uint32_t zero_row) {
+    template <int NT_, bool PAD_> void launch_gram_part(const LongRows &L, uint32_t lo, uint32_t hi, const uint32_t *rec, const real *X,
+                                                        uint32_t zero_row) {
         const uint32_t i0 = L.first[lo], i1 = L.first[hi];
         if (i1 <= i0) return;
-        hipLaunchKernelGGL((gram_part_kernel<NT_, PAD_>), dim3((i1 - i0 + 3) / 4), dim3(256), 0, stream, idx, val, X, L.d_items.p, i0, i1,
+        hipLaunchKernelGGL((gram_part_kernel<NT_, PAD_>), dim3((i1 - i0 + 3) / 4), dim3(256), 0, stream, rec, X, L.d_items.p, i0, i1,
                            part_slab.p, part_stride, zero_row);
         if (i1 - i0 > hi - lo) {
             const uint32_t bpr = (uint32_t)((part_stride * sizeof(real) / 16 + 255) / 256);
@@ -24,12 +24,12 @@
             uint32_t lo, hi;
             longF.range(rb, re, lo, hi);
             if (hi > lo) {
-                launch_gram_part<NT_, false>(longF, lo, hi, Yc_idx.p, Yc_val.p, W.p, (uint32_t)T);
+                launch_gram_part<NT_, false>(longF, lo, hi, Yc_rec.p, W.p, (uint32_t)T);
                 hipLaunchKernelGGL((fsolve_mfma_long_kernel<NT_, KMAX_>), dim3((hi - lo + 3) / 4), dim3(256), 0, stream, split_view(longF, lo, hi), H.p, k, (real)lambdaI);
             }
         }
         hipLaunchKernelGGL((fsolve_mfma_kernel<NT_, KMAX_>), dim3((rows + 3) / 4), dim3(256), 0, stream,
-                           Yc_ptr.p, Yc_idx.p, Yc_val.p, W.p, H.p, rb, re, k, (real)lambdaI, (uint32_t)T, longF.thresh - 1u);
+                           Yc_ptr.p, Yc_rec.p, W.p, H.p, rb, re, k, (real)lambdaI, (uint32_t)T, longF.thresh - 1u);
 #endif
         return 0;
     }
@@ -41,14 +41,14 @@
             uint32_t lo, hi;
             longF.range(rb, re, lo, hi);
             if (hi > lo) {
-                launch_gram_part<NT_, (KMAX_ <= kTile * NT_ - 8)>(longF, lo, hi, Yc_idx.p, Yc_val.p, W.p, (uint32_t)T);
+                launch_gram_part<NT_, (KMAX_ <= kTile * NT_ - 8)>(longF, lo, hi, Yc_rec.p, W.p, (uint32_t)T);
                 hipLaunchKernelGGL((fsolve_quad_long_kernel<NT_, KMAX_>), dim3((hi - lo + 15) / 16), dim3(256), 0, stream, split_view(longF, lo, hi), H.p, k, (real)lambdaI);
             }
         }
         if (longF.any()) { uint32_t lo, hi; longF.range(rb, re, lo, hi); if (hi - lo == rows) return 0; }
         const dim3 grid((rows + 15) / 16), block(256);
         hipLaunchKernelGGL((fsolve_quad_kernel<NT_, KMAX_>), grid, block, 0, stream, Yc_ptr.p,
-                           Yc_idx.p, Yc_val.p, W.p, H.p, rb, re, k, (real)lambdaI, (uint32_t)T, longF.thresh - 1u);
+                           Yc_rec.p, W.p, H.p, rb, re, k, (real)lambdaI, (uint32_t)T, longF.thresh - 1u);
 #endif
         return 0;
     }
@@ -139,7 +139,7 @@
         return 0;
     }
 
-    template <int NT_> void launch_spmm(const LongRows &L, const uint32_t *ptr, const uint32_t *idx, const real *val, const real *X,
+    template <int NT_> void launch_spmm(const LongRows &L, const uint32_t *ptr, const uint32_t *rec, const real *X,
                                         real *out, uint32_t rb, uint32_t re, uint32_t zero_row) {
         if (re <= rb) return;
         if (L.any()) {
@@ -147,12 +147,12 @@
             L.range(rb, re, lo, hi);
             const uint32_t i0 = L.first[lo], i1 = L.first[hi];
             if (i1 > i0) {
-                hipLaunchKernelGGL((spmm_part_kernel<NT_>), dim3((i1 - i0 + 3) / 4), dim3(256), 0, stream, idx, val, X, L.d_items.p, i0, i1, part_slab.p, zero_row);
+                hipLaunchKernelGGL((spmm_part_kernel<NT_>), dim3((i1 - i0 + 3) / 4), dim3(256), 0, stream, rec, X, L.d_items.p, i0, i1, part_slab.p, zero_row);
                 hipLaunchKernelGGL(spmm_reduce_kernel, dim3((unsigned)(((size_t)(hi - lo) * KP + 255) / 256)), dim3(256), 0, stream, L.d_rows.p, L.d_first.p,
                                    part_slab.p, out, lo, hi, KP);
             }
         }
-        hipLaunchKernelGGL((spmm_rows_kernel<NT_>), dim3((re - rb + 3) / 4), dim3(256), 0, stream, ptr, idx, val, X, out, rb, re, zero_row, L.thresh);
+        hipLaunchKernelGGL((spmm_rows_kernel<NT_>), dim3((re - rb + 3) / 4), dim3(256), 0, stream, ptr, rec, X, out, rb, re, zero_row, L.thresh);
     }
     template <int NT_> void launch_dense_tn(const real *A, int K, int M, const real *B, real *out) {
         const int xb = (M + 63) / 64;
@@ -180,10 +180,9 @@
             return 0;
         }
         if (!dense) {
-            const uint32_t *ptr = transposed ? Yc_ptr.p : Yr_ptr.p, *idx = transposed ? Yc_idx.p : Yr_idx.p;
-            const real *val = transposed ? Yc_val.p : Yr_val.p;
+            const uint32_t *ptr = transposed ? Yc_ptr.p : Yr_ptr.p, *rec = transposed ? Yc_rec.p : Yr_rec.p;
             const uint32_t zr = (uint32_t)(transposed ? T : n);
-            if (!with_nt(NT, [&](auto N) { launch_spmm<decltype(N)::value>(transposed ? longF : longX, ptr, idx, val, X, out, rb, re, zr); })) return unsupported_rank();
+            if (!with_nt(NT, [&](auto N) { launch_spmm<decltype(N)::value>(transposed ? longF : longX, ptr, rec, X, out, rb, re, zr); })) return unsupported_rank();
         } else {
             const real *A = transposed ? Yd_tn.p : Yd_nt.p;
             const int K = transposed ? T : n, M = transposed ? n : T;
diff --git a/exp-trmf-nips16_amd/csrc/session_state.hpp b/exp-trmf-nips16_amd/csrc/session_state.hpp
--- a/exp-trmf-nips16_amd/csrc/session_state.hpp
+++ b/exp-trmf-nips16_amd/csrc/session_state.hpp
@@ -46,6 +46,7 @@
     DevBuf<uint32_t> Yc_ptr, Yc_idx, Yr_ptr, Yr_idx, lag_set, lag_steps;
     int nsteps = 0;
     bool has_lag0 = false;
+    DevBuf<uint32_t> Yc_rec, Yr_rec;
     DevBuf<real> Yc_val, Yr_val, W, H, theta, G, Bv, g, s, r, r1, d0, d1, Hd, Hd1, w_new;
     DevBuf<double> lossrow, partials, theta_part;
     bool full = false, dense = false;
diff --git a/exp-trmf-nips16_amd/csrc/session_xphase.hpp b/exp-trmf-nips16_amd/csrc/session_xphase.hpp
--- a/exp-trmf-nips16_amd/csrc/session_xphase.hpp
+++ b/exp-trmf-nips16_amd/csrc/session_xphase.hpp
@@ -77,10 +77,10 @@
         auto launch = [&](auto Pad, auto Packed) {
             constexpr bool PAD = decltype(Pad)::value, PACKED = decltype(Packed)::value;
             if (hi > lo) {
-                launch_gram_part<NT_, PAD>(longX, lo, hi, Yr_idx.p, Yr_val.p, H.p, (uint32_t)n);
+                launch_gram_part<NT_, PAD>(longX, lo, hi, Yr_rec.p, H.p, (uint32_t)n);
                 hipLaunchKernelGGL((gram_x_long_kernel<NT_, PAD, PACKED>), lgrid, lblock, 0, stream, split_view(longX, lo, hi), G.p, Bv.p, k, xp.gstride);
             }
-            hipLaunchKernelGGL((gram_x_kernel<NT_, PAD, PACKED>), grid, block, 0, stream, Yr_ptr.p, Yr_idx.p, Yr_val.p, H.p, G.p, Bv.p,
+            hipLaunchKernelGGL((gram_x_kernel<NT_, PAD, PACKED>), grid, block, 0, stream, Yr_ptr.p, Yr_rec.p, H.p, G.p, Bv.p,
                                rb, re, k, (uint32_t)n, xp.gstride, longX.thresh, xorder);
         };
         if (rhs_pad_ok<NT_>(k)) {
@@ -135,8 +135,8 @@
             if (re > rb) hipLaunchKernelGGL(loss_generic_kernel, dim3(re - rb), dim3(256), 0, stream, Yr_ptr.p, Yr_idx.p, Yr_val.p, H.p, Wv, lossrow.p, rb, re, KP);
         } else if (!with_nt(NT, [&](auto N) {
                        if (re > rb)
-                           hipLaunchKernelGGL((loss_kernel<decltype(N)::value>), dim3(re - rb), dim3(256), 0, stream, Yr_ptr.p, Yr_idx.p,
-                                              Yr_val.p, H.p, Wv, lossrow.p, rb, re, (uint32_t)n);
+                           hipLaunchKernelGGL((loss_kernel<decltype(N)::value>), dim3(re - rb), dim3(256), 0, stream, Yr_ptr.p, Yr_rec.p,
+                                              H.p, Wv, lossrow.p, rb, re, (uint32_t)n);
                    })) return unsupported_rank();
         TRMF_HIP_CHECK(hipGetLastError());
         return all_rows ? 0 : gather_rows(lossrow.p, xbounds, sizeof(double));
diff --git a/exp-trmf-nips16_amd/csrc/trmf_abi.hip b/exp-trmf-nips16_amd/csrc/trmf_abi.hip
--- a/exp-trmf-nips16_amd/csrc/trmf_abi.hip
+++ b/exp-trmf-nips16_amd/csrc/trmf_abi.hip
@@ -372,6 +372,13 @@
     (void)HND(s)->all([&](TrmfSessionImpl *t) { const double v = t->objective(); if (t->comm->rank == 0) J = v; return 0; });
     return J;
 }
+int32_t trmf_session_gram_x(TrmfSession *s, void *G, void *b) {
+    if (!(s && G && b)) return kFail;
+    DeviceGuard guard;
+    if (!guard.ok) return kFail;
+    if (HND(s)->group) { set_error("gram_x: needs a session of one rank"); return kFail; }
+    return HND(s)->first()->download_gram_x((real *)G, (real *)b);
+}
 double trmf_session_fsolve_bytes(TrmfSession *s) { return s ? HND(s)->first()->fsolve_bytes() : 0.0; }
 int32_t trmf_session_describe(TrmfSession *s, char *buf, int32_t cap) {
     if (!s) return kFail;
diff --git a/exp-trmf-nips16_amd/trmf/session.py b/exp-trmf-nips16_amd/trmf/session.py
--- a/exp-trmf-nips16_amd/trmf/session.py
+++ b/exp-trmf-nips16_amd/trmf/session.py
@@ -102,6 +102,8 @@
     lib.trmf_session_stats.restype = c_int32
     lib.trmf_session_objective.argtypes = [c_void_p]; lib.trmf_session_objective.restype = c_double
     lib.trmf_session_fsolve_bytes.argtypes = [c_void_p]; lib.trmf_session_fsolve_bytes.restype = c_double
+    if hasattr(lib, 'trmf_session_gram_x'):
+        lib.trmf_session_gram_x.argtypes = [c_void_p, c_void_p, c_void_p]; lib.trmf_session_gram_x.restype = c_int32
     lib.trmf_session_describe.argtypes = [c_void_p, ctypes.c_char_p, c_int32]; lib.trmf_session_describe.restype = c_int32
     lib.trmf_session_destroy.argtypes = [c_void_p]; lib.trmf_session_destroy.restype = None
     if hasattr(lib, 'trmf_session_set_heldout'):
@@ -420,6 +422,13 @@
     def objective(self):
         return self.lib.trmf_session_objective(self.handle)
 
+    def gram_x(self):
+        T, k = self.rows(), self.model.H.shape[1]
+        dt = self.model.W.dtype
+        G, b = np.empty((T, k, k), dt), np.empty((T, k), dt)
+        self._check(self.lib.trmf_session_gram_x(self.handle, G.ctypes.data_as(c_void_p), b.ctypes.data_as(c_void_p)), 'trmf_session_gram_x')
+        return G, b
+
     def fsolve_bytes(self):
         return self.lib.trmf_session_fsolve_bytes(self.handle)
 
diff --git a/include/trmf_abi.h b/include/trmf_abi.h
--- a/include/trmf_abi.h
+++ b/include/trmf_abi.h
@@ -86,6 +86,7 @@
 TRMF_API int32_t trmf_session_download(TrmfSession *s, PyMatrix *W, PyMatrix *H, PyMatrix *lag_val);
 TRMF_API int32_t trmf_session_stats(TrmfSession *s, TrmfIterStats *out, int32_t cap);
 TRMF_API double trmf_session_objective(TrmfSession *s);
+TRMF_API int32_t trmf_session_gram_x(TrmfSession *s, void *G , void *b );
 TRMF_API double trmf_session_fsolve_bytes(TrmfSession *s);
 TRMF_API int32_t trmf_session_describe(TrmfSession *s, char *buf, int32_t cap);
 TRMF_API void trmf_session_destroy(TrmfSession *s);
```

Result: no change. 1256, median of 6 (+0.9%).
